# shanice-l/UNOPose

Measured on AMD Instinct MI355X. Metric: (query,ref) pairs/sec forward, higher is better.
Workload: dtype bf16; 1 GPU; UNOPose.forward, batch 32 pairs/GPU, 2048 query pts, 5000->2048 reference pts, 196 coarse pts, 518x518 crops, DINOv2 ViT-B/14 reg4, random-init (trained-like) weights

## Files before the change

### include/unopose_hip.h

```cpp
#ifndef UNOPOSE_HIP_H
#define UNOPOSE_HIP_H

#include <stdint.h>

#ifdef __cplusplus
extern "C" {
#endif

#define UNOPOSE_OK 0
#define UNOPOSE_EINVAL 1
#define UNOPOSE_ELAUNCH 2
#define UNOPOSE_ENOMEM 3

typedef void *unopose_stream_t;

int unopose_abi_version(void);
const char *unopose_last_error(void);


int unopose_furthest_point_sampling(const float *xyz, int B, int N, int M,
                                    int32_t *idx, unopose_stream_t stream);

int unopose_gather_points(const float *points, const int32_t *idx, int B, int C,
                          int N, int M, float *out, unopose_stream_t stream);

int unopose_gather_points_grad(const float *grad_out, const int32_t *idx, int B,
                               int C, int N, int M, float *grad_points,
                               unopose_stream_t stream);

int unopose_ball_query(const float *new_xyz, const float *xyz, int B, int N,
                       int M, float radius, int nsample, int32_t *idx,
                       unopose_stream_t stream);

int unopose_group_points(const float *points, const int32_t *idx, int B, int C,
                         int N, int M, int S, float *out,
                         unopose_stream_t stream);

int unopose_group_points_grad(const float *grad_out, const int32_t *idx, int B,
                              int C, int N, int M, int S, float *grad_points,
                              unopose_stream_t stream);

int unopose_three_nn(const float *unknown, const float *known, int B, int n,
                     int m, float *dist2, int32_t *idx, unopose_stream_t stream);

int unopose_three_interpolate(const float *points, const int32_t *idx,
                              const float *weight, int B, int c, int m, int n,
                              float *out, unopose_stream_t stream);

int unopose_three_interpolate_grad(const float *grad_out, const int32_t *idx,
                                   const float *weight, int B, int c, int n,
                                   int m, float *grad_points,
                                   unopose_stream_t stream);


int unopose_lrf_global(const float *pts, int B, int N, int use_ref_rad,
                       float *out, unopose_stream_t stream);

int unopose_query_lrf_group(const float *xyz, int B, int N, float radius,
                            int nsample, float *out, unopose_stream_t stream);

int unopose_lrf_group_idx(const float *xyz, const float *new_xyz, const int *idx,
                          int B, int N, float radius, int nsample, float *out,
                          unopose_stream_t stream);

int unopose_weighted_procrustes(const float *src, const float *ref,
                                const float *w, int M, int N, float thresh,
                                float eps, float *R, float *t,
                                unopose_stream_t stream);

int unopose_pe_image_bytes(void);
int unopose_pe_pack_weights(const float *w1, const float *b1, const float *w2, const float *b2,
                            const float *w3, const float *b3, void *image, unopose_stream_t stream);

int unopose_pe_geometry(const float *xyz, int B, int N, float radius, int nsample, float radius2, int nsample2,
                        const int *cand_in, const int *cand_cnt_in, int cand_stride, void *lists, int *counts,
                        float *frames, int *cand_out, void *lists2, int *counts2, float *frames2,
                        unopose_stream_t stream);
int unopose_pe_mlp_max_packed(const float *xyz, int B, int N, float radius, int nsample, const void *image,
                              const void *lists, const int *counts, const float *frames, void *out, int out_ld,
                              int out_split, unopose_stream_t stream);

int unopose_geo_embedding(const float *points, int B, int n, const void *wd_hi,
                          const void *wd_lo, const void *wa_hi, const void *wa_lo,
                          const float *bias_sum, const float *div_term,
                          float sigma_d, float factor_a, int reduce_mean, int split,
                          int out_bf16, int32_t *knn_ws, void *out,
                          unopose_stream_t stream);

int unopose_geo_embedding_table(const float *points, int B, int n, const float *tab_d, int rows_d, const float *tab_a, int rows_a,
                                const float *bias_sum, const float *w_d, const float *div_term, int hinv, int npoint, float sigma_d,
                                float factor_a, int reduce_mean, int out_bf16, int32_t *knn_ws, void *out,
                                unopose_stream_t stream);

int unopose_geo_embedding_train_workgroups(int B, int n);
int unopose_geo_embedding_train_forward(const float *points, int B, int n, const float *tab_d, int rows_d, const float *tab_a, int rows_a,
                                        const float *bias_sum, const float *w_d, const float *div_term, int hinv, float sigma_d, float factor_a,
                                        int reduce_mean, int32_t *knn, float *out, void *amax, unopose_stream_t stream);
int unopose_geo_embedding_train_backward(const float *points, const int32_t *knn, int B, int n, int rows_d, int rows_a, int hinv, float sigma_d,
                                         float factor_a, int reduce_mean, const float *dE, const void *amax, float *ws, float *full_d,
                                         int *past_table, unopose_stream_t stream);

int unopose_pe_group_mlp_max(const float *xyz, int B, int N, float radius, int nsample,
                             const float *w1, const float *b1, const float *w2,
                             const float *b2, const float *w3, const float *b3,
                             int bf16x3, float *out, unopose_stream_t stream);

int unopose_softmax_stats(const float *x, int B, int R, int C, float *stats_ws, unopose_stream_t stream);
int unopose_infonce_grad(const float *x, int B, int R, int C, const float *stats_ws, const long long *label1,
                         const long long *label2, const float *g, float *grad, unopose_stream_t stream);

int unopose_bn_train_chunk(void);
int unopose_bn_relu_train_forward(const float *x, int B, int C, long L, const float *gamma, const float *beta, float eps, float momentum,
                                  float *running_mean, float *running_var, float *workspace, float *mean, float *rstd, float *y,
                                  unopose_stream_t stream);
int unopose_bn_relu_train_backward(const float *x, const float *dy, int B, int C, long L, const float *gamma, const float *beta,
                                   const float *mean, const float *rstd, float *workspace, float *dgamma, float *dbeta, float *dx,
                                   unopose_stream_t stream);

int unopose_bn_relu_maxpool_train_forward(const float *x, int B, int C, int N, int S, const float *gamma, const float *beta, float eps,
                                          float momentum, float *running_mean, float *running_var, float *workspace, float *mean, float *rstd,
                                          float *out, int32_t *idx, unopose_stream_t stream);
int unopose_bn_relu_maxpool_train_backward(const float *x, const float *g, const int32_t *idx, int B, int C, int N, int S, const float *gamma,
                                           const float *beta, const float *mean, const float *rstd, float *workspace, float *dgamma, float *dbeta,
                                           float *dx, unopose_stream_t stream);

int unopose_saliency_train_forward(const float *atten, const float *s1, const float *s2, int B, int n1, int n2, float *m1, float *m2, float *rmax,
                                   float *rsum, float *cmax, float *csum, unopose_stream_t stream);
int unopose_saliency_train_backward(const float *atten, const float *s1, const float *s2, const float *m1, const float *m2, const float *rmax,
                                    const float *rsum, const float *cmax, const float *csum, const float *g1, const float *g2, int B, int n1, int n2,
                                    float *d_atten, float *ds1, float *ds2, unopose_stream_t stream);

int unopose_nearest_partner(const float *a, const float *b, int B, int n, int m, int over_b, float thr, float *dmin, int32_t *arg,
                            uint8_t *any_close, unopose_stream_t stream);

int unopose_conv1x1_train_wgrad_blocks(void);
int unopose_conv1x1_train_forward(const float *x, int B, int cin, long L, const float *w, int cout, float *y, unopose_stream_t stream);
int unopose_conv1x1_train_wgrad(const float *dy, const float *x, int B, int cout, int cin, long L, float *workspace, float *dw,
                                unopose_stream_t stream);

int unopose_linear_wgrad_f32_splits(long rows, int N, int K);
int unopose_linear_wgrad_f32(const float *g, const float *x, long rows, int N, int K, float *workspace, float *dw, unopose_stream_t stream);
int unopose_assign_labels(const float *atten, int B, int R, int C, const float *score1,
                          const float *score2, float *stats_ws, float *w1, float *w2,
                          unopose_stream_t stream);

int unopose_fine_correspondences(const float *atten, int B, int R, int C, const float *score1,
                                 const float *score2, const float *stats_ws, const float *w1,
                                 const float *w2, const float *pts2, float *weight, float *pred,
                                 unopose_stream_t stream);

int unopose_upproj_plan(const long long *choose, int B2, int Np, int H, int W, int side, int tok_offset, int tok_stride,
                        int cap_rows, int *ws, int *row_list, int *cellmap, int *tile_info, unopose_stream_t stream);

int unopose_linear_bf16_ld(const void *A, int lda, const void *W, int ldw, const float *bias, void *C, int ldc, long M, int N, int K,
                           int epilogue, unopose_stream_t stream);

int unopose_linear_add_layernorm_bf16(const void *A, const void *W, const float *bias, const void *resid, const float *ln_w,
                                      const float *ln_b, float eps, void *C, long M, int K, unopose_stream_t stream);

int unopose_linear_bf16_kv_vt(const void *A, const void *W, const float *bias, void *C, void *vt, long M, int N, int K, int tokens, int key_pad,
                              unopose_stream_t stream);

int unopose_linear_bf16_gather(const void *A, long M, int K, const void *W, int N, const float *bias, const int *row_list,
                               const int *tile_info, int max_tiles, void *C, unopose_stream_t stream);

int unopose_bilinear_sample_compact(const void *Cc, const int *cellmap, const long long *choose, int B2, int side, int Np,
                                    int H, int W, void *out, int out_bf16, unopose_stream_t stream);

int unopose_fine_assign(const void *f1, const void *f2, int B, int R, int C, int D, float shift, const float *score1,
                        const float *score2, const float *pts2, float *ws, float *w1, float *w2, float *weight,
                        float *pred, unopose_stream_t stream);

int unopose_min_dist(const float *p, const float *q, int B, int N, int M, const float *R,
                     const float *t, int cand_per_b, float *out, unopose_stream_t stream);

int unopose_coarse_hypotheses(const float *atten, int B, int R, int C, const float *score1,
                              const float *score2, const float *stats_ws, const float *w1,
                              const float *w2, const float *rand, int nprop, const float *pts1,
                              const float *pts2, float *cdf_ws, float *Rout, float *tout,
                              float *dis, unopose_stream_t stream);

int unopose_coarse_scores(const float *pts1, const float *pts2, int B, int n1, int n2,
                          const float *Rall, const float *tall, int nprop, const int64_t *top,
                          int ncand, const float *w1, float *score, unopose_stream_t stream);

int unopose_topk_smallest(const float *x, int B, int n, int k, int64_t *idx, unopose_stream_t stream);
int unopose_coarse_pick(const float *score, const int64_t *top, int B, int ncand, const float *Rall, const float *tall, int nprop,
                        float *R, float *t, float *best_score, unopose_stream_t stream);

int unopose_token_attention(const void *q, int ldq, const void *k, int ldk, const void *vt,
                            const void *qp, int ldqp, const void *E, int B, int n, int m,
                            float scale, void *out, unopose_stream_t stream);
int unopose_token_attention_key_pad(void);

int unopose_token_attention_f32(const float *q, int ldq, const float *k, int ldk, const float *vt,
                                const float *qp, int ldqp, const float *E, int B, int n, int m,
                                float scale, float *out, unopose_stream_t stream);
int unopose_vit_attention_f32(const float *qkv, int B, int T, int H, float *out, unopose_stream_t stream);
int unopose_token_attention_f32_train(const float *q, int ldq, const float *k, int ldk, const float *vt,
                                      const float *qp, int ldqp, const float *E, int B, int n, int m,
                                      float scale, float *out, float *P, unopose_stream_t stream);
int unopose_token_attention_f32_backward(const float *dout, const float *q, int ldq, const float *v, int ldv,
                                         const float *kt, const float *qp, int ldqp, const float *E, const float *P,
                                         int B, int n, int m, float scale, float *dS, float *dq, float *dk, float *dv,
                                         float *dqp, float *dE, unopose_stream_t stream);
int unopose_vit_attention_f32_split(const float *qkv, int B, int T, int H, void *out_split, unopose_stream_t stream);
int unopose_vit_attention_f32_ss(const void *qkv_split, int B, int T, int H, void *out_split, unopose_stream_t stream);

int unopose_vit_attention(const void *qkv, int B, int T, int H, void *out, unopose_stream_t stream);

int unopose_add_layernorm(const void *a, int a_bf16, const void *b, int b_bf16, const float *w,
                          const float *bias, long rows, int C, float eps, void *out, int out_bf16,
                          unopose_stream_t stream);

int unopose_add_layernorm_strided(const void *a, int a_bf16, const void *b, int b_bf16, const float *w,
                                  const float *bias, long rows, int C, float eps, void *out, int out_bf16,
                                  long ld_out, unopose_stream_t stream);

int unopose_bilinear_sample(const void *z, int z_bf16, const long long *choose, int B, int side, int Np,
                            int H, int W, float *out, unopose_stream_t stream);

int unopose_bilinear_sample_tokens(const void *z, int z_bf16, const long long *choose, int B, int side, int Np,
                                   int H, int W, int tok_offset, int tok_stride, float *out,
                                   unopose_stream_t stream);

int unopose_scale_residual_layernorm(float *x, const void *y_bf16, const float *gamma, const float *w,
                                     const float *bias, long rows, int C, float eps, void *out_bf16,
                                     unopose_stream_t stream);
int unopose_scale_residual_layernorm_f32(float *x, const float *y, const float *gamma, const float *w, const float *bias, long rows,
                                         int C, float eps, void *out_split, long out_ld_bytes, unopose_stream_t stream);

int unopose_scale_residual(float *x, const void *y_bf16, const float *gamma, long rows, int C,
                           unopose_stream_t stream);

int unopose_linear_attention(const void *x, const float *inv_softplus_scale, const void *kvt,
                             const float *ksum, int B, int N, int focus, int mode, void *out,
                             unopose_stream_t stream);
int unopose_linear_attention_kv_state(const void *ykv, const float *inv_softplus_scale, int B, int J, int rows_per_pair,
                                      int first_row, int focus, void *kvt, float *ksum, unopose_stream_t stream);
int unopose_linear_attention_f32(const float *x, const float *inv_softplus_scale, const float *kvt,
                                 const float *ksum, int B, int N, int focus, int mode, float *out,
                                 unopose_stream_t stream);

int unopose_render_depth(const float *verts, int V, const int *faces, int F, const float *Rt, const float *K4, int P, int H, int W,
                         float *depth, unopose_stream_t stream);

int unopose_patchify_bf16(const float *rgb_a, int na, const float *rgb_b, int nb, int S, int Kp, void *out,
                          unopose_stream_t stream);
int unopose_vit_tokens_layernorm(const void *patch, const float *pos, const float *prefix, int npre, int P, int nimg, int C,
                                 const float *ln_w, const float *ln_b, float eps, float *x, void *n1, float *row_mean, unopose_stream_t stream);
int unopose_patchify_split(const float *rgb_a, int na, const float *rgb_b, int nb, int S, int Kp, void *out, unopose_stream_t stream);
int unopose_vit_tokens_layernorm_f32(const float *patch, const float *pos, const float *prefix, int npre, int P, int nimg, int C,
                                     const float *ln_w, const float *ln_b, float eps, float *x, void *n1_split, unopose_stream_t stream);
int unopose_row_dot(const void *x, int x_bf16, const float *w, float b, long rows, int C, void *out, int out_bf16,
                    unopose_stream_t stream);
int unopose_normalize_rows_bf16(const void *x, int x_bf16, long rows, int C, float temp, void *out, int out_f32,
                                unopose_stream_t stream);
int unopose_gather_rows(const void *feats, int B, int N, int row_bytes, const void *idx, int idx_is_i64, int J, int off,
                        const void *alt, long alt_stride_bytes, int prepend, void *out, unopose_stream_t stream);
int unopose_transpose_pad_bf16(const void *v, long ld, int B, int m, int C, int pad, void *vt, unopose_stream_t stream);
int unopose_transpose_pad_f32(const float *v, long ld, int B, int m, int C, int pad, float *vt, unopose_stream_t stream);

int unopose_cloud_radius(const float *pts, int B, int N, float *radius, unopose_stream_t stream);
int unopose_scale_by_radius(const float *x, int B, int n, const float *radius, float eps, int multiply, float *out, unopose_stream_t stream);
int unopose_overlap_scores(const void *scores, int x_bf16, int B, int n_tot, int n1, int halves, float *out, unopose_stream_t stream);
int unopose_nan_to_num_multi(const void *ptrs_dev, const void *sizes_dev, int n_tensors, long max_size, float nan_value, float posinf_value,
                             float neginf_value, unopose_stream_t stream);
int unopose_copy_rows(const void *src, long src_stride_bytes, void *dst, long dst_stride_bytes, int rows, int row_bytes,
                      unopose_stream_t stream);
int unopose_rigid_rows_bf16(const float *p, int B, int N, const float *t, const float *R, void *out, unopose_stream_t stream);
int unopose_token_sum_bf16(const void *x, int B, int J, int C, float *out, unopose_stream_t stream);
int unopose_pose_score(const float *dis, const float *w, int B, int N, float thr, float *out, unopose_stream_t stream);

int unopose_linear_bf16(const void *A, const void *W, const float *bias, void *C, long M, int N, int K,
                        int epilogue, unopose_stream_t stream);
int unopose_gemm_bf16_tile(void);

int unopose_linear_bf16_residual(const void *A, const void *W, const float *bias, float *xres, void *xb, float *stats, const float *prev,
                                 int prev_nparts, long M, int N, int K, unopose_stream_t stream);
int unopose_linear_bf16_lnfold(const void *A, const void *W, const float *dvec, const float *cvec, const float *stats, int nparts, float eps,
                               void *C, long M, int N, int K, int gelu, unopose_stream_t stream);
int unopose_gemm_fold_stagger(int eighth_ticks_per_ktile);

int unopose_bmm_f32(const float *A, long sab, long sah, long sai, long sak, const float *Bm, long sbb, long sbh, long sbj, long sbk,
                    float *C, int bo, int bi, int n, int m, int K, float alpha, unopose_stream_t stream);

int unopose_split_bf16x2(const float *X, long M, int K, void *Xs, unopose_stream_t stream);
int unopose_linear_f32x3(const void *As, const void *Ws, const float *bias, float *C, void *Cs, long M, int N, int K,
                         int epilogue, unopose_stream_t stream);
int unopose_linear_f32x3_bf16(const void *As, const void *Ws, const float *bias, const void *resid, void *Cb, long M, int N, int K,
                              unopose_stream_t stream);

int unopose_prep_desc_ints(void);
int unopose_prep_crop_resize(const void *img, int H, int W, int C, const int *desc, const int *taps, const void *masks, const float *lut,
                             int D, int S, int bgr, int use_mask, float *out, unopose_stream_t stream);
int unopose_prep_compact_lift(const double *depth, int H, int W, const int *desc, const void *masks, const int *row_base, double fx,
                              double fy, double cx, double cy, int D, int max_h, int *pix, double *cloud, double *row_sums,
                              unopose_stream_t stream);
int unopose_prep_distances(const int *desc, const double *cloud, const double *row_sums, int D, int max_n, double *dist,
                           unopose_stream_t stream);
int unopose_prep_gather(const int *sel, const int *index, const int *pix, const double *cloud, int P, int n, int S, float *pts, void *choose,
                        unopose_stream_t stream);

int unopose_vsd_count_ints(void);
int unopose_vsd_counts(const float *test, int n_test, const float *gt, int n_gt, const float *est, int n_est, const int *index,
                       const double *pairs, const double *taus, int T, int P, int H, int W, int *counts, unopose_stream_t stream);
int unopose_pose_errors(const double *pts, int n, const double *syms, int S, const double *est, const double *gt, const double *K, int P,
                        double *mssd, double *mspd, unopose_stream_t stream);

int unopose_adi_tile_points(void);
int unopose_adi_slab_points(void);
int unopose_pose_metrics(const double *pts, int n, const double *syms, int S, const double *est, const double *gt, const double *K, int P,
                         int proj_sym, double *out, unopose_stream_t stream);
int unopose_adi(const double *pts, int n, const double *est, const double *gt, int P, double *workspace, double *adi,
                unopose_stream_t stream);

int unopose_gt_visibility_ints(void);
int unopose_gt_visibility(const float *canvas, int n_canvas, const float *test, int n_test, const int *index, const double *params, int G,
                          int H, int W, int *out, void *mask, void *mask_visib, unopose_stream_t stream);

int unopose_pts_extent_tile_points(void);
int unopose_pts_extent_doubles(void);
int unopose_pts_extent(const double *pts, const long long *offsets, const long long *offsets_dev, int M, int prune, double *kept,
                       long long *kept_count, double *out, unopose_stream_t stream);

#ifdef __cplusplus
}
#endif
#endif
```

### unopose_amd/_lib.py

```python
import ctypes
import os

import torch

_HERE = os.path.dirname(os.path.abspath(__file__))
SO_PATH = os.environ.get("UNOPOSE_LIB") or os.path.join(_HERE, "libunopose_hip.so")

_lib = None

_P = ctypes.c_void_p
_I = ctypes.c_int
_F = ctypes.c_float
_L = ctypes.c_long
_D = ctypes.c_double

SIGNATURES = {
    "unopose_furthest_point_sampling": [_P, _I, _I, _I, _P, _P],
    "unopose_gather_points": [_P, _P, _I, _I, _I, _I, _P, _P],
    "unopose_gather_points_grad": [_P, _P, _I, _I, _I, _I, _P, _P],
    "unopose_ball_query": [_P, _P, _I, _I, _I, _F, _I, _P, _P],
    "unopose_group_points": [_P, _P, _I, _I, _I, _I, _I, _P, _P],
    "unopose_group_points_grad": [_P, _P, _I, _I, _I, _I, _I, _P, _P],
    "unopose_three_nn": [_P, _P, _I, _I, _I, _P, _P, _P],
    "unopose_three_interpolate": [_P, _P, _P, _I, _I, _I, _I, _P, _P],
    "unopose_three_interpolate_grad": [_P, _P, _P, _I, _I, _I, _I, _P, _P],
    "unopose_lrf_global": [_P, _I, _I, _I, _P, _P],
    "unopose_query_lrf_group": [_P, _I, _I, _F, _I, _P, _P],
    "unopose_lrf_group_idx": [_P, _P, _P, _I, _I, _F, _I, _P, _P],
    "unopose_weighted_procrustes": [_P, _P, _P, _I, _I, _F, _F, _P, _P, _P],
    "unopose_assign_labels": [_P, _I, _I, _I, _P, _P, _P, _P, _P, _P],
    "unopose_linear_bf16_ld": [_P, _I, _P, _I, _P, _P, _I, ctypes.c_long, _I, _I, _I, _P],
    "unopose_scale_residual_layernorm_f32": [_P, _P, _P, _P, _P, ctypes.c_long, _I, _F, _P, _L, _P],
    "unopose_gather_rows": [_P, _I, _I, _I, _P, _I, _I, _I, _P, _L, _I, _P, _P],
    "unopose_softmax_stats": [_P, _I, _I, _I, _P, _P],
    "unopose_infonce_grad": [_P, _I, _I, _I, _P, _P, _P, _P, _P, _P],
    "unopose_fine_correspondences": [_P, _I, _I, _I, _P, _P, _P, _P, _P, _P, _P, _P, _P],
    "unopose_upproj_plan": [_P, _I, _I, _I, _I, _I, _I, _I, _I, _P, _P, _P, _P, _P],
    "unopose_linear_add_layernorm_bf16": [_P, _P, _P, _P, _P, _P, _F, _P, ctypes.c_long, _I, _P],
    "unopose_linear_bf16_kv_vt": [_P, _P, _P, _P, _P, ctypes.c_long, _I, _I, _I, _I, _P],
    "unopose_linear_bf16_gather": [_P, ctypes.c_long, _I, _P, _I, _P, _P, _P, _I, _P, _P],
    "unopose_bilinear_sample_compact": [_P, _P, _P, _I, _I, _I, _I, _I, _P, _I, _P],
    "unopose_fine_assign": [_P, _P, _I, _I, _I, _I, _F, _P, _P, _P, _P, _P, _P, _P, _P, _P],
    "unopose_min_dist": [_P, _P, _I, _I, _I, _P, _P, _I, _P, _P],
    "unopose_coarse_hypotheses": [_P, _I, _I, _I, _P, _P, _P, _P, _P, _P, _I, _P, _P, _P, _P, _P, _P, _P],
    "unopose_coarse_scores": [_P, _P, _I, _I, _I, _P, _P, _I, _P, _I, _P, _P, _P],
    "unopose_topk_smallest": [_P, _I, _I, _I, _P, _P],
    "unopose_coarse_pick": [_P, _P, _I, _I, _P, _P, _I, _P, _P, _P, _P],
    "unopose_token_attention": [_P, _I, _P, _I, _P, _P, _I, _P, _I, _I, _I, _F, _P, _P],
    "unopose_token_attention_key_pad": [],
    "unopose_token_attention_f32": [_P, _I, _P, _I, _P, _P, _I, _P, _I, _I, _I, _F, _P, _P],
    "unopose_token_attention_f32_train": [_P, _I, _P, _I, _P, _P, _I, _P, _I, _I, _I, _F, _P, _P, _P],
    "unopose_token_attention_f32_backward": [_P, _P, _I, _P, _I, _P, _P, _I, _P, _P, _I, _I, _I, _F, _P, _P, _P, _P, _P, _P, _P],
    "unopose_vit_attention_f32": [_P, _I, _I, _I, _P, _P],
    "unopose_vit_attention_f32_split": [_P, _I, _I, _I, _P, _P],
    "unopose_vit_attention_f32_ss": [_P, _I, _I, _I, _P, _P],
    "unopose_bn_train_chunk": [],
    "unopose_bn_relu_train_forward": [_P, _I, _I, ctypes.c_long, _P, _P, _F, _F, _P, _P, _P, _P, _P, _P, _P],
    "unopose_bn_relu_train_backward": [_P, _P, _I, _I, ctypes.c_long, _P, _P, _P, _P, _P, _P, _P, _P, _P],
    "unopose_bn_relu_maxpool_train_forward": [_P, _I, _I, _I, _I, _P, _P, _F, _F, _P, _P, _P, _P, _P, _P, _P, _P],
    "unopose_bn_relu_maxpool_train_backward": [_P, _P, _P, _I, _I, _I, _I, _P, _P, _P, _P, _P, _P, _P, _P, _P],
    "unopose_nearest_partner": [_P, _P, _I, _I, _I, _I, _F, _P, _P, _P, _P],
    "unopose_saliency_train_forward": [_P, _P, _P, _I, _I, _I, _P, _P, _P, _P, _P, _P, _P],
    "unopose_saliency_train_backward": [_P, _P, _P, _P, _P, _P, _P, _P, _P, _P, _P, _I, _I, _I, _P, _P, _P, _P],
    "unopose_conv1x1_train_wgrad_blocks": [],
    "unopose_conv1x1_train_forward": [_P, _I, _I, ctypes.c_long, _P, _I, _P, _P],
    "unopose_conv1x1_train_wgrad": [_P, _P, _I, _I, _I, ctypes.c_long, _P, _P, _P],
    "unopose_linear_wgrad_f32_splits": [ctypes.c_long, _I, _I],
    "unopose_linear_wgrad_f32": [_P, _P, ctypes.c_long, _I, _I, _P, _P, _P],
    "unopose_vit_attention": [_P, _I, _I, _I, _P, _P],
    "unopose_add_layernorm": [_P, _I, _P, _I, _P, _P, ctypes.c_long, _I, _F, _P, _I, _P],
    "unopose_add_layernorm_strided": [_P, _I, _P, _I, _P, _P, ctypes.c_long, _I, _F, _P, _I, ctypes.c_long, _P],
    "unopose_bilinear_sample": [_P, _I, _P, _I, _I, _I, _I, _I, _P, _P],
    "unopose_bilinear_sample_tokens": [_P, _I, _P, _I, _I, _I, _I, _I, _I, _I, _P, _P],
    "unopose_scale_residual_layernorm": [_P, _P, _P, _P, _P, ctypes.c_long, _I, _F, _P, _P],
    "unopose_scale_residual": [_P, _P, _P, ctypes.c_long, _I, _P],
    "unopose_linear_attention": [_P, _P, _P, _P, _I, _I, _I, _I, _P, _P],
    "unopose_linear_attention_f32": [_P, _P, _P, _P, _I, _I, _I, _I, _P, _P],
    "unopose_linear_attention_kv_state": [_P, _P, _I, _I, _I, _I, _I, _P, _P, _P],
    "unopose_linear_bf16": [_P, _P, _P, _P, ctypes.c_long, _I, _I, _I, _P],
    "unopose_gemm_bf16_tile": [],
    "unopose_gemm_fold_stagger": [_I],
    "unopose_linear_bf16_residual": [_P, _P, _P, _P, _P, _P, _P, _I, ctypes.c_long, _I, _I, _P],
    "unopose_linear_bf16_lnfold": [_P, _P, _P, _P, _P, _I, _F, _P, ctypes.c_long, _I, _I, _I, _P],
    "unopose_patchify_bf16": [_P, _I, _P, _I, _I, _I, _P, _P],
    "unopose_patchify_split": [_P, _I, _P, _I, _I, _I, _P, _P],
    "unopose_vit_tokens_layernorm": [_P, _P, _P, _I, _I, _I, _I, _P, _P, _F, _P, _P, _P, _P],
    "unopose_vit_tokens_layernorm_f32": [_P, _P, _P, _I, _I, _I, _I, _P, _P, _F, _P, _P, _P],
    "unopose_row_dot": [_P, _I, _P, _F, ctypes.c_long, _I, _P, _I, _P],
    "unopose_normalize_rows_bf16": [_P, _I, ctypes.c_long, _I, _F, _P, _I, _P],
    "unopose_transpose_pad_bf16": [_P, ctypes.c_long, _I, _I, _I, _I, _P, _P],
    "unopose_transpose_pad_f32": [_P, _L, _I, _I, _I, _I, _P, _P],
    "unopose_cloud_radius": [_P, _I, _I, _P, _P],
    "unopose_scale_by_radius": [_P, _I, _I, _P, _F, _I, _P, _P],
    "unopose_overlap_scores": [_P, _I, _I, _I, _I, _I, _P, _P],
    "unopose_copy_rows": [_P, _L, _P, _L, _I, _I, _P],
    "unopose_nan_to_num_multi": [_P, _P, _I, _L, _F, _F, _F, _P],
    "unopose_rigid_rows_bf16": [_P, _I, _I, _P, _P, _P, _P],
    "unopose_token_sum_bf16": [_P, _I, _I, _I, _P, _P],
    "unopose_pose_score": [_P, _P, _I, _I, _F, _P, _P],
    "unopose_render_depth": [_P, _I, _P, _I, _P, _P, _I, _I, _I, _P, _P],
    "unopose_bmm_f32": [_P, ctypes.c_long, ctypes.c_long, ctypes.c_long, ctypes.c_long, _P, ctypes.c_long, ctypes.c_long, ctypes.c_long, ctypes.c_long, _P, _I, _I, _I, _I, _I, _F, _P],
    "unopose_split_bf16x2": [_P, ctypes.c_long, _I, _P, _P],
    "unopose_linear_f32x3": [_P, _P, _P, _P, _P, ctypes.c_long, _I, _I, _I, _P],
    "unopose_pe_image_bytes": [],
    "unopose_pe_pack_weights": [_P, _P, _P, _P, _P, _P, _P, _P],
    "unopose_pe_geometry": [_P, _I, _I, _F, _I, _F, _I, _P, _P, _I, _P, _P, _P, _P, _P, _P, _P, _P],
    "unopose_pe_mlp_max_packed": [_P, _I, _I, _F, _I, _P, _P, _P, _P, _P, _I, _I, _P],
    "unopose_linear_f32x3_bf16": [_P, _P, _P, _P, _P, ctypes.c_long, _I, _I, _P],
    "unopose_pe_group_mlp_max": [_P, _I, _I, _F, _I, _P, _P, _P, _P, _P, _P, _I, _P, _P],
    "unopose_geo_embedding": [_P, _I, _I, _P, _P, _P, _P, _P, _P, _F, _F, _I, _I, _I, _P, _P, _P],
    "unopose_geo_embedding_train_workgroups": [_I, _I],
    "unopose_geo_embedding_train_forward": [_P, _I, _I, _P, _I, _P, _I, _P, _P, _P, _I, _F, _F, _I, _P, _P, _P, _P],
    "unopose_geo_embedding_train_backward": [_P, _P, _I, _I, _I, _I, _I, _F, _F, _I, _P, _P, _P, _P, _P, _P],
    "unopose_geo_embedding_table": [_P, _I, _I, _P, _I, _P, _I, _P, _P, _P, _I, _I, _F, _F, _I, _I, _P, _P, _P],
    "unopose_prep_desc_ints": [],
    "unopose_prep_crop_resize": [_P, _I, _I, _I, _P, _P, _P, _P, _I, _I, _I, _I, _P, _P],
    "unopose_prep_compact_lift": [_P, _I, _I, _P, _P, _P, _D, _D, _D, _D, _I, _I, _P, _P, _P, _P],
    "unopose_prep_distances": [_P, _P, _P, _I, _I, _P, _P],
    "unopose_prep_gather": [_P, _P, _P, _P, _I, _I, _I, _P, _P, _P],
    "unopose_vsd_count_ints": [],
    "unopose_vsd_counts": [_P, _I, _P, _I, _P, _I, _P, _P, _P, _I, _I, _I, _I, _P, _P],
    "unopose_pose_errors": [_P, _I, _P, _I, _P, _P, _P, _I, _P, _P, _P],
    "unopose_adi_tile_points": [],
    "unopose_adi_slab_points": [],
    "unopose_pose_metrics": [_P, _I, _P, _I, _P, _P, _P, _I, _I, _P, _P],
    "unopose_adi": [_P, _I, _P, _P, _I, _P, _P, _P],
    "unopose_gt_visibility_ints": [],
    "unopose_gt_visibility": [_P, _I, _P, _I, _P, _P, _I, _I, _I, _P, _P, _P, _P],
    "unopose_pts_extent_tile_points": [],
    "unopose_pts_extent_doubles": [],
    "unopose_pts_extent": [_P, _P, _P, _I, _I, _P, _P, _P, _P],
}


def lib():
    global _lib
    if _lib is None:
        if not os.path.exists(SO_PATH):
            raise RuntimeError(
                f"{SO_PATH} is missing: the HIP extension has not been built "
                "(run `python -m unopose_amd.build`). There is no CPU fallback."
            )
        L = ctypes.CDLL(SO_PATH)
        L.unopose_abi_version.restype = _I
        L.unopose_last_error.restype = ctypes.c_char_p
        for name, argtypes in SIGNATURES.items():
            fn = getattr(L, name)
            fn.argtypes = argtypes
            fn.restype = _I
        _lib = L
    return _lib


def stream_ptr(device=None):
    if device is None:
        idx = torch._C._cuda_getDevice()
    else:
        idx = device if isinstance(device, int) else torch.device(device).index
        if idx is None:
            idx = torch._C._cuda_getDevice()
    return ctypes.c_void_p(torch._C._cuda_getCurrentRawStream(idx))


class _NullContext:
    def __enter__(self):
        return None

    def __exit__(self, *a):
        return False


_NULL_CONTEXT = _NullContext()


def on_device(dev):
    idx = dev.index if isinstance(dev, torch.device) else dev
    if idx is None or idx == torch._C._cuda_getDevice():
        return _NULL_CONTEXT
    return torch.cuda.device(idx)


def call(name, *args):
    L = lib()
    rc = getattr(L, name)(*args)
    if rc != 0:
        raise RuntimeError(f"{name} failed (code {rc}): {L.unopose_last_error().decode()}")


def ptr(t):
    return ctypes.c_void_p(t.data_ptr())


def check_f32(x, name):
    if not x.is_cuda:
        raise RuntimeError(f"{name}: CPU not supported")
    if not x.is_contiguous():
        raise RuntimeError(f"{name} must be a contiguous tensor")
    if x.dtype != torch.float32:
        raise RuntimeError(f"{name} must be a float tensor")


def check_i32(x, name):
    if not x.is_cuda:
        raise RuntimeError(f"{name} must be a CUDA tensor")
    if not x.is_contiguous():
        raise RuntimeError(f"{name} must be a contiguous tensor")
    if x.dtype != torch.int32:
        raise RuntimeError(f"{name} must be an int tensor")
```

### unopose_amd/csrc/gemm.hip

```cpp
#include <mutex>

#include "gemm_kernel.h"

using namespace unopose;

static inline int use_nt_store(long M, int N) { return (size_t)M * N * 2 > (32u << 20) ? 1 : 0; }

namespace unopose {
int gemm_small_tiles_limit() {
  return gemm_cu_count() * 5 / 8;
}
}
static int small_tiles_limit() { return unopose::gemm_small_tiles_limit(); }

namespace unopose {
int *gemm_sched_slot(hipStream_t stream) {
  hipStreamCaptureStatus cap = hipStreamCaptureStatusNone;
  if (hipStreamIsCapturing(stream, &cap) != hipSuccess || cap != hipStreamCaptureStatusNone) return nullptr;
  static std::mutex mu;
  static int *ring[64] = {nullptr};
  static unsigned next_slot[64] = {0};
  int dev = 0;
  if (hipGetDevice(&dev) != hipSuccess || dev < 0 || dev >= 64) return nullptr;
  std::lock_guard<std::mutex> lock(mu);
  if (!ring[dev]) {
    int *p = nullptr;
    if (hipMalloc(&p, 1024 * 16 * sizeof(int)) != hipSuccess || hipMemset(p, 0, 1024 * 16 * sizeof(int)) != hipSuccess) return nullptr;
    ring[dev] = p;
  }
  return ring[dev] + (size_t)(next_slot[dev]++ & 1023u) * 16;
}
}

static int linear_bf16_dispatch(const void *A, int lda, const void *W, int ldw, const float *bias, void *C, int ldc, long M, int N, int K,
                                int epilogue, hipStream_t s, const char *what) {
  const int tiles_n = N / GEMM_BN;
  const int tiles = cdiv(M, GEMM_BM) * tiles_n;
  if (tiles < small_tiles_limit()) return gemm_small_linear(A, W, bias, C, M, N, K, lda, ldw, ldc, epilogue, s);
  const int n_cu = gemm_cu_count();
  const int grid = tiles >= n_cu ? n_cu : ((tiles + 7) & ~7);
  const int nt = use_nt_store(M, N);
#define UNOPOSE_LD_LAUNCH(E)                                                                                                                \
  hipLaunchKernelGGL(gemm256_kernel<E>, dim3(grid), dim3(512), 0, s, (const u16 *)A, (const u16 *)W, bias, (u16 *)C, (int)M, N, K, tiles_n, \
                     tiles, nt, (const int *)nullptr, (const int *)nullptr, (const u16 *)nullptr, (const float *)nullptr,                     \
                     (const float *)nullptr, 0.f, lda, ldw, ldc, sched)
  int *const sched = tiles > grid ? gemm_sched_slot(s) : nullptr;
  if (epilogue == 1)
    UNOPOSE_LD_LAUNCH(1);
  else if (epilogue == 2)
    UNOPOSE_LD_LAUNCH(2);
  else
    UNOPOSE_LD_LAUNCH(0);
#undef UNOPOSE_LD_LAUNCH
  return check_launch(what);
}

extern "C" {

int unopose_gemm_bf16_tile(void) { return GEMM_BM; }

int unopose_linear_bf16(const void *A, const void *W, const float *bias, void *C, long M, int N, int K, int epilogue,
                        unopose_stream_t stream) {
  UNOPOSE_REQUIRE(A && W && bias && C, "linear_bf16: null pointer");
  UNOPOSE_REQUIRE(M >= 1 && M < (1L << 31) && N >= GEMM_BN && N % GEMM_BN == 0 && K >= GEMM_BK && K % GEMM_BK == 0,
                  "linear_bf16: needs N %% 256 == 0 and K %% 64 == 0 (got M=%ld N=%d K=%d)", M, N, K);
  UNOPOSE_REQUIRE((size_t)M * K * 2 < (1UL << 32) && (size_t)N * K * 2 < (1UL << 32) && (size_t)M * N * 2 < (1UL << 32), "linear_bf16: operand larger than 4 GiB");
  UNOPOSE_REQUIRE(epilogue >= 0 && epilogue <= 2, "linear_bf16: epilogue must be 0 (bias), 1 (bias + GELU) or 2 (bias + ReLU)");
  return linear_bf16_dispatch(A, K, W, K, bias, C, N, M, N, K, epilogue, (hipStream_t)stream, "linear_bf16");
}

int unopose_linear_bf16_ld(const void *A, int lda, const void *W, int ldw, const float *bias, void *C, int ldc, long M, int N, int K,
                           int epilogue, unopose_stream_t stream) {
  UNOPOSE_REQUIRE(A && W && bias && C, "linear_bf16_ld: null pointer");
  UNOPOSE_REQUIRE(M >= 1 && M < (1L << 31) && N >= GEMM_BN && N % GEMM_BN == 0 && K >= GEMM_BK && K % GEMM_BK == 0,
                  "linear_bf16_ld: needs N %% 256 == 0 and K %% 64 == 0 (got M=%ld N=%d K=%d)", M, N, K);
  UNOPOSE_REQUIRE(lda >= K && ldw >= K && ldc >= N && lda % 8 == 0 && ldw % 8 == 0 && ldc % 8 == 0,
                  "linear_bf16_ld: row strides must cover the rows and be multiples of 8 elements (lda=%d ldw=%d ldc=%d)", lda, ldw, ldc);
  UNOPOSE_REQUIRE((size_t)M * lda * 2 < (1UL << 32) && (size_t)N * ldw * 2 < (1UL << 32) && (size_t)M * ldc * 2 < (1UL << 32), "linear_bf16_ld: operand larger than 4 GiB");
  UNOPOSE_REQUIRE(epilogue >= 0 && epilogue <= 2, "linear_bf16_ld: epilogue must be 0 (bias), 1 (bias + GELU) or 2 (bias + ReLU)");
  return linear_bf16_dispatch(A, lda, W, ldw, bias, C, ldc, M, N, K, epilogue, (hipStream_t)stream, "linear_bf16_ld");
}

int unopose_linear_add_layernorm_bf16(const void *A, const void *W, const float *bias, const void *resid, const float *ln_w,
                                      const float *ln_b, float eps, void *C, long M, int K, unopose_stream_t stream) {
  UNOPOSE_REQUIRE(A && W && bias && resid && ln_w && ln_b && C, "linear_add_layernorm_bf16: null pointer");
  UNOPOSE_REQUIRE(M >= 1 && M < (1L << 31) && K >= GEMM_BK && K % GEMM_BK == 0, "linear_add_layernorm_bf16: needs K %% 64 == 0 (got M=%ld K=%d)", M, K);
  UNOPOSE_REQUIRE((size_t)M * K * 2 < (1UL << 32), "linear_add_layernorm_bf16: operand larger than 4 GiB");
  const int tiles = cdiv(M, GEMM_BM);
  if (tiles < small_tiles_limit()) return gemm_small_linear_ln(A, W, bias, resid, ln_w, ln_b, eps, C, M, K, (hipStream_t)stream);
  const int n_cu = gemm_cu_count();
  const int grid = tiles >= n_cu ? n_cu : ((tiles + 7) & ~7);
  hipLaunchKernelGGL((gemm256_kernel<3, false>), dim3(grid), dim3(512), 0, (hipStream_t)stream, (const u16 *)A, (const u16 *)W, bias,
                     (u16 *)C, (int)M, GEMM_BN, K, 1, tiles, use_nt_store(M, GEMM_BN), (const int *)nullptr, (const int *)nullptr,
                     (const u16 *)resid, ln_w, ln_b, eps);
  return check_launch("linear_add_layernorm_bf16");
}

int unopose_linear_bf16_kv_vt(const void *A, const void *W, const float *bias, void *C, void *vt, long M, int N, int K, int tokens, int key_pad,
                               unopose_stream_t stream) {
  UNOPOSE_REQUIRE(A && W && bias && C && vt, "linear_bf16_kv_vt: null pointer");
  UNOPOSE_REQUIRE(M >= 1 && M < (1L << 31) && N >= 256 && N % 128 == 0 && K >= GEMM_BK && K % GEMM_BK == 0,
                  "linear_bf16_kv_vt: needs N %% 128 == 0 (>= 256) and K %% 64 == 0 (got M=%ld N=%d K=%d)", M, N, K);
  UNOPOSE_REQUIRE(tokens >= 1 && key_pad >= tokens && M % tokens == 0 && key_pad - tokens <= 64, "linear_bf16_kv_vt: M must be whole clouds of `tokens` rows, key_pad in [tokens, tokens + 64] (got %ld, %d, %d)", M, tokens, key_pad);
  UNOPOSE_REQUIRE((size_t)M * K * 2 < (1UL << 32) && (size_t)N * K * 2 < (1UL << 32) && (size_t)M * N * 2 < (1UL << 32), "linear_bf16_kv_vt: operand larger than 4 GiB");
  return gemm_small_linear_vt(A, W, bias, C, vt, M, N, K, tokens, key_pad, (hipStream_t)stream);
}

int unopose_linear_bf16_gather(const void *A, long M, int K, const void *W, int N, const float *bias, const int *row_list,
                               const int *tile_info, int max_tiles, void *C, unopose_stream_t stream) {
  UNOPOSE_REQUIRE(A && W && bias && C && row_list && tile_info, "linear_bf16_gather: null pointer");
  UNOPOSE_REQUIRE(M >= 1 && M < (1L << 31) && N >= GEMM_BN && N % GEMM_BN == 0 && N / GEMM_BN <= 64 && K >= GEMM_BK && K % GEMM_BK == 0,
                  "linear_bf16_gather: needs N %% 256 == 0 and K %% 64 == 0 (got M=%ld N=%d K=%d)", M, N, K);
  UNOPOSE_REQUIRE((size_t)M * K * 2 < (1UL << 32) && (size_t)N * K * 2 < (1UL << 32), "linear_bf16_gather: operand larger than 4 GiB");
  UNOPOSE_REQUIRE(max_tiles >= 0, "linear_bf16_gather: bad tile capacity");
  if (max_tiles == 0) return UNOPOSE_OK;
  const int n_cu = gemm_cu_count();
  const int grid = max_tiles >= n_cu ? n_cu : ((max_tiles + 7) & ~7);
  hipLaunchKernelGGL((gemm256_kernel<0, true>), dim3(grid), dim3(512), 0, (hipStream_t)stream, (const u16 *)A, (const u16 *)W, bias,
                     (u16 *)C, (int)M, N, K, 1, 0, 0, row_list, tile_info);
  return check_launch("linear_bf16_gather");
}

static int fold_launch_shape(long M, int N, int *grid, int *tiles, int *tiles_n) {
  *tiles_n = N / GEMM_BN;
  *tiles = cdiv(M, GEMM_BM) * *tiles_n;
  const int n_cu = gemm_cu_count();
  *grid = *tiles >= n_cu ? n_cu : ((*tiles + 7) & ~7);
  return use_nt_store(M, N);
}

static int g_fold_stagger = 8 * 105;
int unopose_gemm_fold_stagger(int eighth_ticks_per_ktile) {
  const int was = g_fold_stagger;
  if (eighth_ticks_per_ktile >= 0) g_fold_stagger = eighth_ticks_per_ktile;
  return was;
}

int unopose_linear_bf16_residual(const void *A, const void *W, const float *bias, float *xres, void *xb, float *stats, const float *prev,
                                 int prev_nparts, long M, int N, int K, unopose_stream_t stream) {
  UNOPOSE_REQUIRE(A && W && bias && xres && xb && stats, "linear_bf16_residual: null pointer");
  UNOPOSE_REQUIRE(prev != stats && (prev_nparts == 0 || (prev && prev_nparts * GEMM_BN == N && prev_nparts <= GEMM_LNF_MAXPARTS)),
                  "linear_bf16_residual: prev must be another buffer with 0 or N / 256 <= %d partials per row (got prev_nparts=%d N=%d)",
                  GEMM_LNF_MAXPARTS, prev_nparts, N);
  UNOPOSE_REQUIRE(M >= 1 && M < (1L << 31) && N >= GEMM_BN && N % GEMM_BN == 0 && K >= GEMM_BK && K % GEMM_BK == 0,
                  "linear_bf16_residual: needs N %% 256 == 0 and K %% 64 == 0 (got M=%ld N=%d K=%d)", M, N, K);
  UNOPOSE_REQUIRE((size_t)M * K * 2 < (1UL << 32) && (size_t)N * K * 2 < (1UL << 32) && (size_t)M * N * 4 < (1UL << 31), "linear_bf16_residual: operand too large for 32-bit buffer offsets");
  int grid, tiles, tiles_n;
  const int nt = fold_launch_shape(M, N, &grid, &tiles, &tiles_n);
  hipStream_t s = (hipStream_t)stream;
  int *const sched = tiles > grid ? gemm_sched_slot(s) : nullptr;
  hipLaunchKernelGGL((gemm256_kernel<5>), dim3(grid), dim3(512), 0, s, (const u16 *)A, (const u16 *)W, bias, (u16 *)xb, (int)M, N, K, tiles_n, tiles, nt,
                     (const int *)nullptr, (const int *)nullptr, (const u16 *)nullptr, (const float *)nullptr, (const float *)nullptr, 0.f, 0, 0, 0, sched,
                     (void *)xres, (const float *)nullptr, (float2 *)stats, prev_nparts, tiles > grid ? g_fold_stagger * (K / GEMM_BK) / 8 : 0, prev);
  return check_launch("linear_bf16_residual");
}

int unopose_linear_bf16_lnfold(const void *A, const void *W, const float *dvec, const float *cvec, const float *stats, int nparts, float eps, void *C,
                               long M, int N, int K, int gelu, unopose_stream_t stream) {
  UNOPOSE_REQUIRE(A && W && dvec && cvec && stats && C, "linear_bf16_lnfold: null pointer");
  UNOPOSE_REQUIRE(M >= 1 && M < (1L << 31) && N >= GEMM_BN && N % GEMM_BN == 0 && K >= GEMM_BK && K % GEMM_BK == 0,
                  "linear_bf16_lnfold: needs N %% 256 == 0 and K %% 64 == 0 (got M=%ld N=%d K=%d)", M, N, K);
  UNOPOSE_REQUIRE(nparts >= 1 && nparts <= GEMM_LNF_MAXPARTS && nparts * GEMM_BN == K, "linear_bf16_lnfold: needs nparts = K / 256 <= %d (got nparts=%d K=%d)", GEMM_LNF_MAXPARTS, nparts, K);
  UNOPOSE_REQUIRE((size_t)M * K * 2 < (1UL << 32) && (size_t)N * K * 2 < (1UL << 32) && (size_t)M * N * 2 < (1UL << 32), "linear_bf16_lnfold: operand larger than 4 GiB");
  int grid, tiles, tiles_n;
  const int nt = fold_launch_shape(M, N, &grid, &tiles, &tiles_n);
  hipStream_t s = (hipStream_t)stream;
  int *const sched = tiles > grid ? gemm_sched_slot(s) : nullptr;
#define UNOPOSE_LNF_LAUNCH(E)                                                                                                                      \
  hipLaunchKernelGGL((gemm256_kernel<E>), dim3(grid), dim3(512), 0, s, (const u16 *)A, (const u16 *)W, dvec, (u16 *)C, (int)M, N, K, tiles_n, tiles, nt, \
                     (const int *)nullptr, (const int *)nullptr, (const u16 *)nullptr, (const float *)nullptr, (const float *)nullptr, eps, 0, 0, 0, sched, \
                     (void *)nullptr, cvec, (float2 *)stats, nparts)
  if (gelu)
    UNOPOSE_LNF_LAUNCH(7);
  else
    UNOPOSE_LNF_LAUNCH(6);
#undef UNOPOSE_LNF_LAUNCH
  return check_launch("linear_bf16_lnfold");
}

}
```

### unopose_amd/csrc/gemm_kernel.h

```cpp
#pragma once
#include "gemm_common.h"

namespace unopose {

constexpr int GEMM_XPOL = 2;
#define GEMM_BK 64
constexpr int GEMM_ROTX = 5, GEMM_ROTS = 3;

#define GEMM_WAIT_VM(n) asm volatile("s_waitcnt vmcnt(" #n ")" ::: "memory")
#define GEMM_WAIT_VM_(n) GEMM_WAIT_VM(n)

#define GEMM_LDS_BIAS (2 * GEMM_BUFBYTES)
#define GEMM_LDS_MBOX (GEMM_LDS_BIAS + 2048)
#define GEMM_LDS_LNW (GEMM_LDS_MBOX + 16)
#define GEMM_LDS_LNB (GEMM_LDS_LNW + 1024)
#define GEMM_LDS_LNPART (GEMM_LDS_LNB + 1024)
#define GEMM_LDS_STATS GEMM_LDS_LNPART
#define GEMM_LNF_MAXPARTS 4
#define GEMM_LDS_SHIFT (GEMM_LDS_LNPART + 8192)

template <int EPI, bool GATHER = false, bool F32 = false>
__global__ __launch_bounds__(512, 1) __attribute__((amdgpu_num_vgpr(127))) void gemm256_kernel(const void *__restrict__ Av, const void *__restrict__ Wv,
                                                           const float *__restrict__ bias, void *__restrict__ Cv, int M,
                                                           int N, int K, int tiles_n, int tiles_arg, int nt_store,
                                                           const int *__restrict__ row_list = nullptr,
                                                           const int *__restrict__ tile_info = nullptr,
                                                           const u16 *__restrict__ resid = nullptr, const float *__restrict__ ln_w = nullptr,
                                                           const float *__restrict__ ln_b = nullptr, float ln_eps = 0.f, int lda = 0,
                                                           int ldw = 0, int ldc = 0, int *__restrict__ sched = nullptr,
                                                           void *__restrict__ C2v = nullptr, const float *__restrict__ aux_vec = nullptr,
                                                           float2 *__restrict__ stats = nullptr, int nparts = 0, int stagger = 0,
                                                           const float *__restrict__ fold_prev = nullptr) {
  static_assert(!(F32 && (EPI == 3 || GATHER)), "the fp32-class form has no LayerNorm epilogue / gathered rows");
  static_assert(!((F32 || GATHER) && EPI >= 5), "the residual / LayerNorm-fold epilogues belong to the dense bf16 form");
  constexpr bool LNF = EPI == 6 || EPI == 7;
  static_assert(F32 || EPI != 4, "EPI 4 (bf16 + residual out of fp32-class operands) is an F32 epilogue");
  constexpr int ESZ = F32 ? 4 : 2;
  constexpr int KT = F32 ? 32 : 64;
  const char *A = reinterpret_cast<const char *>(Av), *W = reinterpret_cast<const char *>(Wv);
  const int LDA = lda ? lda : K, LDW = ldw ? ldw : K, LDC = ldc ? ldc : N;
  const int tiles = GATHER ? __builtin_amdgcn_readfirstlane(tile_info[0]) : tiles_arg;
  __shared__ __attribute__((aligned(1024))) char smem[GEMM_LDS_BIAS + 2048 + 16 + (EPI == 3 ? 2048 + 8192 : EPI == 5 ? 2048 + 8192 + 4096 : LNF ? 2048 + 2 * 8192 : 0)];
  float *const lnw_lds = reinterpret_cast<float *>(smem + GEMM_LDS_LNW), *const lnb_lds = reinterpret_cast<float *>(smem + GEMM_LDS_LNB);
  float2 *const ln_part = reinterpret_cast<float2 *>(smem + GEMM_LDS_LNPART);
  if (EPI == 3 && threadIdx.x < GEMM_BN) {
    lnw_lds[threadIdx.x] = ln_w[threadIdx.x];
    lnb_lds[threadIdx.x] = ln_b[threadIdx.x];
  }
  const int tid = threadIdx.x, lane = tid & 63, wave = __builtin_amdgcn_readfirstlane(tid >> 6);
  const int wm = wave >> 2, wn = wave & 3;
  const int l31 = lane & 31, hi = lane >> 5;
  const int l31_ = l31, hi_ = hi, lane_ = lane;
  const int xcd = blockIdx.x & 7, slot = blockIdx.x >> 3, nslots = gridDim.x >> 3;
  const int tiles_m = tiles / tiles_n, per_group = GEMM_GM * tiles_n;
  int cw = (size_t)N * K * ESZ > (size_t)(4u << 20) ? (2400 * 1024) / (GEMM_BN * K * ESZ) : 0;
  if (cw < 3) cw = 0;
  const bool colwalk = cw > 0 && !GATHER && tiles_n > cw && ((tiles_m & 7) == 0 || tiles_m >= 512);
  const int rq = tiles_m >> 3, rr = tiles_m & 7;
  const int rows_x = rq + (xcd < rr ? 1 : 0), row_base = xcd < rr ? xcd * (rq + 1) : rr * (rq + 1) + (xcd - rr) * rq;
  const int cq = tiles >> 3, cr = tiles & 7;
  const int chunk_base = xcd < cr ? xcd * (cq + 1) : cr * (cq + 1) + (xcd - cr) * cq;
  const int chunk_len = colwalk ? rows_x * tiles_n : cq + (xcd < cr ? 1 : 0);
  const __amdgpu_buffer_rsrc_t a_rs = __builtin_amdgcn_make_buffer_rsrc((void *)A, 0, (int)((size_t)M * LDA * ESZ), 0x00020000);
  const __amdgpu_buffer_rsrc_t w_rs = __builtin_amdgcn_make_buffer_rsrc((void *)W, 0, (int)((size_t)N * LDW * ESZ), 0x00020000);
  const __amdgpu_buffer_rsrc_t c_rs = __builtin_amdgcn_make_buffer_rsrc(Cv, 0, GATHER ? 0x7fffffff : (int)((size_t)M * LDC * 2), 0x00020000);
  const __amdgpu_buffer_rsrc_t b_rs = __builtin_amdgcn_make_buffer_rsrc((void *)bias, 0, N * 4, 0x00020000);
  const int nk = K / KT;

  const int fx = (l31 >> 1) & 7;
  uint32_t fr_off[4];
#pragma unroll
  for (int ks = 0; ks < 4; ++ks) fr_off[ks] = (uint32_t)((l31 >> 3) * 1024 + (l31 & 7) * 128 + ((((ks << 1) | hi) ^ fx) << 4));
  const uint32_t a_base = (uint32_t)(wm * 16384);
  const uint32_t w_base = (uint32_t)(GEMM_OPBYTES + wn * 8192);
  const uint32_t a_dst = (uint32_t)((wave >> 2) * 16384 + (wave & 3) * 2048);
  const uint32_t w_dst = (uint32_t)(GEMM_OPBYTES + (wave >> 1) * 8192 + (wave & 1) * 2048);

  struct TileP {
    int m0, n0, rot;
    uint32_t a_off[4], w_off[2];
  };
  auto tile_params = [&](int ti, int step, TileP &p) {
    const int t = chunk_base + ti;
    int tn, tm;
    if (GATHER) {
      tm = t;
      tn = 0;
      const int ng = N / GEMM_BN;
      for (int g = 1; g < ng; ++g) tn += t >= tile_info[1 + g] ? 1 : 0;
      tn = __builtin_amdgcn_readfirstlane(tn);
    } else if (colwalk) {
      const int per_block = rows_x * cw;
      const int cb = ti / per_block, v = ti - cb * per_block;
      const int cwb = min(cw, tiles_n - cb * cw);
      const int g = v / (GEMM_GM * cwb), w = v - g * GEMM_GM * cwb;
      const int gm = min(GEMM_GM, rows_x - g * GEMM_GM);
      const int tl = w / gm;
      tn = cb * cw + tl;
      tm = row_base + g * GEMM_GM + (w - tl * gm);
    } else {
      const int mg = t / per_group, rr = t - mg * per_group;
      const int gm = min(GEMM_GM, tiles_m - mg * GEMM_GM);
      tn = rr / gm;
      tm = mg * GEMM_GM + (rr - tn * gm);
    }
    p.m0 = __builtin_amdgcn_readfirstlane(tm * GEMM_BM);
    p.n0 = __builtin_amdgcn_readfirstlane(tn * GEMM_BN);
#pragma unroll
    for (int j = 0; j < 4; ++j) {
      const int row = (wave >> 2) * 128 + (j >> 1) * 64 + (wave & 3) * 16 + (j & 1) * 8 + (lane >> 3);
      const int c = (lane & 7) ^ ((row >> 1) & 7);
      int arow = p.m0 + row;
      if (GATHER) arow = max(row_list[p.m0 + row], 0);
      p.a_off[j] = (uint32_t)((size_t)arow * LDA * ESZ + c * 16);
    }
#pragma unroll
    for (int i = 0; i < 2; ++i) {
      const int row = (wave >> 1) * 64 + (wave & 1) * 16 + i * 8 + (lane >> 3);
      const int c = (lane & 7) ^ ((row >> 1) & 7);
      p.w_off[i] = (uint32_t)((size_t)(p.n0 + row) * LDW * ESZ + c * 16);
    }
    const int skew = ((tm & 3) + tn) % GEMM_SKEW;
    p.rot = __builtin_amdgcn_readfirstlane((xcd * GEMM_ROTX + step * GEMM_ROTS + skew) % nk);
  };
  const uint32_t lds0 = (uint32_t)(uintptr_t)(__attribute__((address_space(3))) char *)smem;
  enum { H_A0 = 0, H_B0 = 1, H_B1 = 2, H_A1 = 3 };
  auto stage_half = [&](const TileP &p, int kind, int kt, uint32_t bufoff) {
    kt += __builtin_amdgcn_readfirstlane(p.rot);
    if (kt >= nk) kt -= nk;
    const int so = kt * GEMM_ROWB;
    if (kind == H_A0 || kind == H_A1) {
      const int ah = kind == H_A1 ? 1 : 0;
      const uint32_t la = lds0 + bufoff + a_dst + ah * 8192;
      gemm_dma16(la, p.a_off[2 * ah], a_rs, so);
      gemm_dma16(la + 1024, p.a_off[2 * ah + 1], a_rs, so);
    } else {
      const int bh = kind == H_B1 ? 1 : 0;
      const uint32_t lw = lds0 + bufoff + w_dst + bh * 4096;
      const int sob = so + bh * (32 * ESZ) * LDW;
      gemm_dma16(lw, p.w_off[0], w_rs, sob);
      gemm_dma16(lw + 1024, p.w_off[1], w_rs, sob);
    }
  };
  const __amdgpu_buffer_rsrc_t cv_rs = __builtin_amdgcn_make_buffer_rsrc((void *)(LNF ? aux_vec : bias), 0, N * 4, 0x00020000);
  const __amdgpu_buffer_rsrc_t st_rs = __builtin_amdgcn_make_buffer_rsrc((void *)stats, 0, LNF ? (int)((size_t)((M + GEMM_BM - 1) / GEMM_BM) * GEMM_BM * nparts * 8) : 0, 0x00020000);
  auto stage_bias = [&](const TileP &p, int bsel) {
    if (!LNF) {
      gemm_dma16(lds0 + GEMM_LDS_BIAS + bsel * 1024, (uint32_t)(lane * 16), b_rs, __builtin_amdgcn_readfirstlane(p.n0 * 4));
      return;
    }
    const int total = 2 + 2 * nparts;
#pragma unroll
    for (int rep = 0; rep < (2 + 2 * GEMM_LNF_MAXPARTS + 7) / 8; ++rep) {
      if (rep * 8 >= total) break;
      int pc = rep * 8 + wave;
      if (pc >= total) pc = 0;
      if (pc == 0)
        gemm_dma16(lds0 + GEMM_LDS_BIAS + bsel * 1024, (uint32_t)(lane * 16), b_rs, __builtin_amdgcn_readfirstlane(p.n0 * 4));
      else if (pc == 1)
        gemm_dma16(lds0 + GEMM_LDS_LNW + bsel * 1024, (uint32_t)(lane * 16), cv_rs, __builtin_amdgcn_readfirstlane(p.n0 * 4));
      else
        gemm_dma16(lds0 + GEMM_LDS_STATS + bsel * 8192 + (pc - 2) * 1024, (uint32_t)(lane * 16), st_rs,
                   __builtin_amdgcn_readfirstlane(p.m0 * nparts * 8 + (pc - 2) * 1024));
    }
  };
  const bool can_stream = EPI != 3 && nk >= 2;
  const bool dyn = sched != nullptr && !GATHER && can_stream && nk >= 5;
  int *const mbox = reinterpret_cast<int *>(smem + GEMM_LDS_MBOX);
  TileP cur;
  bool have = false;
  uint32_t par = 0;
  int bsel = 0;
  int ti = slot;
  if (dyn) {
    if (tid == 0) mbox[0] = atomicAdd(sched + xcd, 1);
    __syncthreads();
    ti = __builtin_amdgcn_readfirstlane(mbox[0]);
  }
  if (EPI == 5 && stagger > 0 && ((slot / tiles_n) & 1)) {
    const uint64_t t0 = __builtin_amdgcn_s_memrealtime();
    while ((int64_t)(__builtin_amdgcn_s_memrealtime() - t0) < (int64_t)stagger) __builtin_amdgcn_s_sleep(8);
  }
  for (; ti < chunk_len;) {
    const int step = dyn ? ti / nslots : (ti - slot) / nslots;
    if (!have) {
      tile_params(ti, step, cur);
      stage_bias(cur, bsel);
      stage_half(cur, H_A0, 0, par);
      stage_half(cur, H_B0, 0, par);
      stage_half(cur, H_B1, 0, par);
      stage_half(cur, H_A1, 0, par);
      if (nk >= 2) {
        stage_half(cur, H_A0, 1, par ^ GEMM_BUFBYTES);
        stage_half(cur, H_B0, 1, par ^ GEMM_BUFBYTES);
        GEMM_WAIT_VM(6);
      } else {
        GEMM_WAIT_VM(2);
      }
      asm volatile("s_waitcnt lgkmcnt(0)" ::: "memory");
      __builtin_amdgcn_s_barrier();
    }
    const int m0 = __builtin_amdgcn_readfirstlane(cur.m0), n0 = __builtin_amdgcn_readfirstlane(cur.n0);
    cur.rot = __builtin_amdgcn_readfirstlane(cur.rot);
    bool more = can_stream && ti + nslots < chunk_len;
    int ti_next = ti + nslots;
    TileP nxt;

    const float *bias_lds = reinterpret_cast<const float *>(smem + GEMM_LDS_BIAS + bsel * 1024);
    f32x16 acc[2][4];
#pragma unroll
    for (int nb = 0; nb < 2; ++nb)
#pragma unroll
      for (int g = 0; g < 4; ++g) {
        const float4 bv = EPI == 3 || LNF ? make_float4(0.f, 0.f, 0.f, 0.f) : *reinterpret_cast<const float4 *>(bias_lds + wn * 64 + nb * 32 + 8 * g + 4 * hi);
#pragma unroll
        for (int mb = 0; mb < 4; ++mb) {
          acc[nb][mb][4 * g + 0] = bv.x;
          acc[nb][mb][4 * g + 1] = bv.y;
          acc[nb][mb][4 * g + 2] = bv.z;
          acc[nb][mb][4 * g + 3] = bv.w;
        }
      }

    bf16x8 af[2][4], wf0[4], wf1[4];
    auto read_a = [&](const char *lb, int ah) {
#pragma unroll
      for (int mbl = 0; mbl < 2; ++mbl)
#pragma unroll
        for (int ks = 0; ks < 4; ++ks) af[mbl][ks] = *reinterpret_cast<const bf16x8 *>(lb + a_base + ah * 8192 + mbl * 4096 + fr_off[ks]);
    };
    auto read_b = [&](const char *lb, int bh, bf16x8(&wf)[4]) {
#pragma unroll
      for (int ks = 0; ks < 4; ++ks) wf[ks] = *reinterpret_cast<const bf16x8 *>(lb + w_base + bh * 4096 + fr_off[ks]);
    };
    auto mfma_q = [&](int ah, int bh, const bf16x8(&wf)[4]) {
      if (F32) {
#pragma unroll
        for (int b = 0; b < 2; ++b)
#pragma unroll
          for (int mbl = 0; mbl < 2; ++mbl) {
            f32x16 &a = acc[bh][2 * ah + mbl];
            a = __builtin_amdgcn_mfma_f32_32x32x16_bf16(wf[2 + b], af[mbl][b], a, 0, 0, 0);
            a = __builtin_amdgcn_mfma_f32_32x32x16_bf16(wf[b], af[mbl][2 + b], a, 0, 0, 0);
            a = __builtin_amdgcn_mfma_f32_32x32x16_bf16(wf[b], af[mbl][b], a, 0, 0, 0);
          }
        return;
      }
#pragma unroll
      for (int ks = 0; ks < 4; ++ks)
#pragma unroll
        for (int mbl = 0; mbl < 2; ++mbl)
          acc[bh][2 * ah + mbl] = __builtin_amdgcn_mfma_f32_32x32x16_bf16(wf[ks], af[mbl][ks], acc[bh][2 * ah + mbl], 0, 0, 0);
    };
    if (wm == 1) __builtin_amdgcn_s_barrier();
    auto phase = [&](auto compute) {
      asm volatile("s_waitcnt lgkmcnt(0)" ::: "memory");
      __builtin_amdgcn_sched_barrier(0);
      __builtin_amdgcn_s_barrier();
      __builtin_amdgcn_sched_barrier(0);
      compute();
      __builtin_amdgcn_sched_barrier(0);
      __builtin_amdgcn_s_barrier();
      asm volatile("" ::: "memory");
      __builtin_amdgcn_sched_barrier(0);
    };
    for (int t = 0; t < nk; ++t) {
      const bool last = t + 1 == nk, last2 = t + 2 >= nk;
      if (dyn) {
        if (t == 2 && wave == 0) {
          int tk;
          asm volatile("v_readfirstlane_b32 %0, v255" : "=s"(tk)::"memory");
          if (lane == 0) mbox[0] = tk;
        }
        if (t + 2 == nk) {
          ti_next = __builtin_amdgcn_readfirstlane(*reinterpret_cast<volatile int *>(mbox));
          more = ti_next < chunk_len;
        }
      }
      if (more && t + 2 == nk) tile_params(ti_next, dyn ? ti_next / nslots : step + 1, nxt);
      const char *lb = smem + par;
      const uint32_t bnext = par ^ GEMM_BUFBYTES;
      read_b(lb, 0, wf0);
      read_b(lb, 1, wf1);
      read_a(lb, 0);
      __builtin_amdgcn_sched_barrier(0);
      if (t == 0 && !last) stage_half(cur, H_B1, 1, bnext);
      if (!last)
        stage_half(cur, H_A1, t + 1, bnext);
      else if (more)
        stage_half(nxt, H_A1, 0, bnext);
      if (last && !more)
        GEMM_WAIT_VM(0);
      else
        GEMM_WAIT_VM(8);
      phase([&] {
        mfma_q(0, 0, wf0);
        mfma_q(0, 1, wf1);
      });
      read_a(lb, 1);
      __builtin_amdgcn_sched_barrier(0);
      if (dyn && t == 0 && wave == 0) {
        unsigned long long keep;
        const uint32_t zero = 0, one = 1;
#pragma clang diagnostic push
#pragma clang diagnostic ignored "-Winline-asm"
        asm volatile("s_mov_b64 %0, exec\n\ts_mov_b64 exec, 1\n\ts_nop 1\n\tglobal_atomic_add v255, %2, %3, %1 sc0\n\ts_mov_b64 exec, %0\n\ts_nop 1"
                     : "=&s"(keep)
                     : "s"(sched + xcd), "v"(zero), "v"(one)
                     : "memory", "v255");
#pragma clang diagnostic pop
      }
      if (!last2) {
        stage_half(cur, H_A0, t + 2, par);
        stage_half(cur, H_B0, t + 2, par);
        stage_half(cur, H_B1, t + 2, par);
        GEMM_WAIT_VM(8);
      } else if (more) {
        if (!last) {
          stage_bias(nxt, bsel ^ 1);
          stage_half(nxt, H_A0, 0, par);
          stage_half(nxt, H_B0, 0, par);
          stage_half(nxt, H_B1, 0, par);
          if (LNF) {
            if (nparts <= 3) GEMM_WAIT_VM(9);
            else GEMM_WAIT_VM(10);
          } else
            GEMM_WAIT_VM(8);
        } else if (F32) {
          GEMM_WAIT_VM(2);
        } else {
          stage_half(nxt, H_A0, 1, par);
          stage_half(nxt, H_B0, 1, par);
          GEMM_WAIT_VM(6);
        }
      } else if (!last) {
        GEMM_WAIT_VM(2);
      }
      phase([&] {
        mfma_q(1, 1, wf1);
        mfma_q(1, 0, wf0);
      });
      par ^= GEMM_BUFBYTES;
    }
    if (wm == 0) __builtin_amdgcn_s_barrier();
    par ^= GEMM_BUFBYTES;
    if (EPI == 3) {
#pragma unroll
      for (int mb = 0; mb < 4; ++mb) {
        const int m = min(m0 + wm * 128 + mb * 32 + l31, M - 1);
        const u16 *rp = resid + (size_t)m * GEMM_BN + wn * 64 + 4 * hi;
        float a1 = 0.f, a2 = 0.f;
#pragma unroll
        for (int nb = 0; nb < 2; ++nb)
#pragma unroll
          for (int g = 0; g < 4; ++g) {
            const int nl = nb * 32 + 8 * g + 4 * hi;
            const float4 bv = *reinterpret_cast<const float4 *>(bias_lds + wn * 64 + nl);
            const uint2 r = *reinterpret_cast<const uint2 *>(rp + nb * 32 + 8 * g);
            const float v0 = acc[nb][mb][4 * g + 0] + bv.x + __uint_as_float(r.x << 16);
            const float v1 = acc[nb][mb][4 * g + 1] + bv.y + __uint_as_float(r.x & 0xffff0000u);
            const float v2 = acc[nb][mb][4 * g + 2] + bv.z + __uint_as_float(r.y << 16);
            const float v3 = acc[nb][mb][4 * g + 3] + bv.w + __uint_as_float(r.y & 0xffff0000u);
            acc[nb][mb][4 * g + 0] = v0;
            acc[nb][mb][4 * g + 1] = v1;
            acc[nb][mb][4 * g + 2] = v2;
            acc[nb][mb][4 * g + 3] = v3;
            a1 += (v0 + v1) + (v2 + v3);
            a2 += (v0 * v0 + v1 * v1) + (v2 * v2 + v3 * v3);
          }
        a1 += __shfl_xor(a1, 32);
        a2 += __shfl_xor(a2, 32);
        if (hi == 0) ln_part[((wm * 4 + mb) * 32 + l31) * 4 + wn] = make_float2(a1, a2);
      }
      __syncthreads();
#pragma unroll
      for (int mb = 0; mb < 4; ++mb) {
        const float2 *pp = ln_part + ((wm * 4 + mb) * 32 + l31) * 4;
        const float t1 = (pp[0].x + pp[1].x) + (pp[2].x + pp[3].x), t2 = (pp[0].y + pp[1].y) + (pp[2].y + pp[3].y);
        const float mean = t1 * (1.f / GEMM_BN);
        const float rstd = rsqrtf(fmaxf(t2 * (1.f / GEMM_BN) - mean * mean, 0.f) + ln_eps);
#pragma unroll
        for (int nb = 0; nb < 2; ++nb)
#pragma unroll
          for (int g = 0; g < 4; ++g) {
            const int nl = wn * 64 + nb * 32 + 8 * g + 4 * hi;
            const float4 gw = *reinterpret_cast<const float4 *>(lnw_lds + nl), gb = *reinterpret_cast<const float4 *>(lnb_lds + nl);
            acc[nb][mb][4 * g + 0] = (acc[nb][mb][4 * g + 0] - mean) * rstd * gw.x + gb.x;
            acc[nb][mb][4 * g + 1] = (acc[nb][mb][4 * g + 1] - mean) * rstd * gw.y + gb.y;
            acc[nb][mb][4 * g + 2] = (acc[nb][mb][4 * g + 2] - mean) * rstd * gw.z + gb.z;
            acc[nb][mb][4 * g + 3] = (acc[nb][mb][4 * g + 3] - mean) * rstd * gw.w + gb.w;
          }
      }
    }
    if constexpr (LNF) {
      int l31 = l31_, hi = hi_;
      asm volatile("" : "+v"(l31), "+v"(hi));
      const float *c_lds = reinterpret_cast<const float *>(smem + GEMM_LDS_LNW + bsel * 1024);
      const float inv_k = 1.f / (float)K;
      float rs[4], nm[4];
#pragma unroll
      for (int mb = 0; mb < 4; ++mb) {
        const float2 *sp = reinterpret_cast<const float2 *>(smem + GEMM_LDS_STATS + bsel * 8192) + (wm * 128 + mb * 32 + l31) * nparts;
        float t1 = 0.f, t2 = 0.f;
#pragma unroll
        for (int i = 0; i < GEMM_LNF_MAXPARTS; ++i)
          if (i < nparts) {
            const float2 q = sp[i];
            t1 += q.x;
            t2 += q.y;
          }
        const float mean = t1 * inv_k;
        rs[mb] = rsqrtf(fmaxf(t2 * inv_k - mean * mean, 0.f) + ln_eps);
        nm[mb] = -mean * rs[mb];
      }
#pragma unroll
      for (int nb = 0; nb < 2; ++nb)
#pragma unroll
        for (int g = 0; g < 4; ++g) {
          const int nl = wn * 64 + nb * 32 + 8 * g + 4 * hi;
          const float4 cv = *reinterpret_cast<const float4 *>(c_lds + nl), dv = *reinterpret_cast<const float4 *>(bias_lds + nl);
#pragma unroll
          for (int mb = 0; mb < 4; ++mb) {
            acc[nb][mb][4 * g + 0] = fmaf(rs[mb], acc[nb][mb][4 * g + 0], fmaf(nm[mb], cv.x, dv.x));
            acc[nb][mb][4 * g + 1] = fmaf(rs[mb], acc[nb][mb][4 * g + 1], fmaf(nm[mb], cv.y, dv.y));
            acc[nb][mb][4 * g + 2] = fmaf(rs[mb], acc[nb][mb][4 * g + 2], fmaf(nm[mb], cv.z, dv.z));
            acc[nb][mb][4 * g + 3] = fmaf(rs[mb], acc[nb][mb][4 * g + 3], fmaf(nm[mb], cv.w, dv.w));
          }
        }
    }
    if constexpr (EPI == 5) {
      int l31 = l31_, hi = hi_, lane = lane_;
      asm volatile("" : "+v"(l31), "+v"(hi), "+v"(lane));
      char *cw = smem + par + (wave < 4 ? 8192 + (wave & 1) * 4096 + (wave >> 1) * 16384 : GEMM_OPBYTES + 4096 + (wave - 4) * 8192);
      const __amdgpu_buffer_rsrc_t x_rs = __builtin_amdgcn_make_buffer_rsrc(C2v, 0, (int)((size_t)M * N * 4), 0x00020000);
      const int r4 = lane >> 4, q = lane & 15;
      const uint32_t x_v0 = (uint32_t)((((size_t)m0 + wm * 128 + r4) * N + n0 + wn * 64 + q * 4) * 4);
      const uint32_t c_v0 = (uint32_t)((((size_t)m0 + wm * 128 + r4) * LDC + n0 + wn * 64 + q * 4) * 2);
      const uint32_t x_rowb = (uint32_t)(N * 4), c_rowb = (uint32_t)(LDC * 2);
      const int rows_p = tiles_m * GEMM_BM;
      float sv[2] = {0.f, 0.f};
      if (fold_prev != nullptr) {
        float pv[2][GEMM_LNF_MAXPARTS + 1];
#pragma unroll
        for (int j = 0; j < 2; ++j) {
          const size_t m = (size_t)m0 + wm * 128 + j * 64 + lane, sh_at = (size_t)rows_p * 2 * nparts + m;
#pragma unroll
          for (int i = 0; i < GEMM_LNF_MAXPARTS; ++i) pv[j][i] = fold_prev[i < nparts ? m * 2 * nparts + 2 * i : sh_at];
          pv[j][GEMM_LNF_MAXPARTS] = fold_prev[sh_at];
        }
#pragma unroll
        for (int j = 0; j < 2; ++j) {
          float t = 0.f;
#pragma unroll
          for (int i = 0; i < GEMM_LNF_MAXPARTS; ++i) t += i < nparts ? pv[j][i] : 0.f;
          sv[j] = m0 + wm * 128 + j * 64 + lane < M ? pv[j][GEMM_LNF_MAXPARTS] + t * (1.f / (float)N) : 0.f;
        }
      }
      constexpr int PF = 3;
      f32x4 rv[PF][4];
      auto load_round = [&](int r, f32x4(&dst)[4]) {
#pragma unroll
        for (int it = 0; it < 4; ++it) {
          dst[it] = __builtin_bit_cast(f32x4, __builtin_amdgcn_raw_buffer_load_b128(x_rs, x_v0 + (uint32_t)(r * 16 + it * 4) * x_rowb, 0, GEMM_XPOL));
        }
      };
#pragma unroll
      for (int r = 0; r < PF; ++r) load_round(r, rv[r]);
      float *const sh_lds = reinterpret_cast<float *>(smem + GEMM_LDS_SHIFT + wave * 512);
#pragma unroll
      for (int r = 0; r < 8; ++r) {
        const int mb = r >> 1, h = r & 1;
        if ((l31 >> 4) == h) {
#pragma unroll
          for (int nb = 0; nb < 2; ++nb)
#pragma unroll
            for (int g = 0; g < 4; ++g) {
              const int s16 = (nb * 8 + 2 * g + hi) ^ (l31 & 15);
              *reinterpret_cast<float4 *>(cw + (l31 & 15) * 256 + s16 * 16) =
                  make_float4(acc[nb][mb][4 * g + 0], acc[nb][mb][4 * g + 1], acc[nb][mb][4 * g + 2], acc[nb][mb][4 * g + 3]);
            }
        }
        if (r == 0) {
#pragma unroll
          for (int j = 0; j < 2; ++j) {
            sh_lds[j * 64 + lane] = sv[j];
            if (wn == 0) reinterpret_cast<float *>(stats)[(size_t)rows_p * 2 * tiles_n + m0 + wm * 128 + j * 64 + lane] = sv[j];
          }
        }
        __builtin_amdgcn_fence(__ATOMIC_RELEASE, "wavefront");
        __builtin_amdgcn_wave_barrier();
        __builtin_amdgcn_fence(__ATOMIC_ACQUIRE, "wavefront");
#pragma unroll
        for (int it = 0; it < 4; ++it) {
          const int row = it * 4 + r4;
          const f32x4 a = *reinterpret_cast<const f32x4 *>(cw + row * 256 + ((q ^ row) << 4));
          const f32x4 o = rv[r % PF][it];
          f32x4 v;
#pragma unroll
          for (int e = 0; e < 4; ++e) v[e] = a[e] + o[e];
          __builtin_amdgcn_raw_buffer_store_b128(__builtin_bit_cast(u32x4, v), x_rs, x_v0 + (uint32_t)(r * 16 + it * 4) * x_rowb, 0, GEMM_XPOL);
          const float s = sh_lds[row + r * 16];
#pragma unroll
          for (int e = 0; e < 4; ++e) v[e] = v[e] - s;
          typedef unsigned int u32x2 __attribute__((ext_vector_type(2)));
          const u32x2 pk = {cvt_pk_bf16_f32(v[0], v[1]), cvt_pk_bf16_f32(v[2], v[3])};
          if (nt_store)
            __builtin_amdgcn_raw_buffer_store_b64(pk, c_rs, c_v0 + (uint32_t)(r * 16 + it * 4) * c_rowb, 0, 2);
          else
            __builtin_amdgcn_raw_buffer_store_b64(pk, c_rs, c_v0 + (uint32_t)(r * 16 + it * 4) * c_rowb, 0, 0);
          float a1 = (v[0] + v[1]) + (v[2] + v[3]), a2 = (v[0] * v[0] + v[1] * v[1]) + (v[2] * v[2] + v[3] * v[3]);
          a1 += dpp_f32<0x111, 0xF>(a1, 0.f);
          a2 += dpp_f32<0x111, 0xF>(a2, 0.f);
          a1 += dpp_f32<0x112, 0xF>(a1, 0.f);
          a2 += dpp_f32<0x112, 0xF>(a2, 0.f);
          a1 += dpp_f32<0x114, 0xF>(a1, 0.f);
          a2 += dpp_f32<0x114, 0xF>(a2, 0.f);
          a1 += dpp_f32<0x118, 0xF>(a1, 0.f);
          a2 += dpp_f32<0x118, 0xF>(a2, 0.f);
          if (q == 15) ln_part[((wm * 4 + mb) * 32 + h * 16 + row) * 4 + wn] = make_float2(a1, a2);
        }
        __builtin_amdgcn_fence(__ATOMIC_RELEASE, "wavefront");
        __builtin_amdgcn_wave_barrier();
        __builtin_amdgcn_fence(__ATOMIC_ACQUIRE, "wavefront");
        if (r + PF < 8) load_round(r + PF, rv[r % PF]);
      }
      asm volatile("s_waitcnt lgkmcnt(0)" ::: "memory");
      __builtin_amdgcn_s_barrier();
      if (wn == 0 && hi == 0) {
#pragma unroll
        for (int mb = 0; mb < 4; ++mb) {
          const float2 *pp = ln_part + ((wm * 4 + mb) * 32 + l31) * 4;
          const float4 p01 = *reinterpret_cast<const float4 *>(pp), p23 = *reinterpret_cast<const float4 *>(pp + 2);
          stats[(size_t)(m0 + wm * 128 + mb * 32 + l31) * tiles_n + (n0 >> 8)] = make_float2((p01.x + p01.z) + (p23.x + p23.z), (p01.y + p01.w) + (p23.y + p23.w));
        }
      }
    } else if constexpr (!F32) {
    int l31 = l31_, hi = hi_, lane = lane_;
    asm volatile("" : "+v"(l31), "+v"(hi), "+v"(lane));
    char *cw = smem + par + (wave < 4 ? 8192 + (wave & 1) * 4096 + (wave >> 1) * 16384 : GEMM_OPBYTES + 4096 + (wave - 4) * 8192);
    const uint32_t c_v0 = GATHER ? (uint32_t)((((size_t)m0 + wm * 128 + (lane >> 3)) * GEMM_BN + wn * 64 + (lane & 7) * 8) * 2)
                                 : (uint32_t)((((size_t)m0 + wm * 128 + (lane >> 3)) * LDC + n0 + wn * 64 + (lane & 7) * 8) * 2);
    const uint32_t c_rowb = (uint32_t)((GATHER ? GEMM_BN : LDC) * 2);
#pragma unroll
    for (int mb = 0; mb < 4; ++mb) {
#pragma unroll
      for (int nb = 0; nb < 2; ++nb) {
#pragma unroll
        for (int g = 0; g < 4; ++g) {
          const int nl = nb * 32 + 8 * g + 4 * hi;
          float v0 = acc[nb][mb][4 * g + 0], v1 = acc[nb][mb][4 * g + 1], v2 = acc[nb][mb][4 * g + 2], v3 = acc[nb][mb][4 * g + 3];
          if (EPI == 1 || EPI == 7) {
            v0 = gelu_bf16_class(v0);
            v1 = gelu_bf16_class(v1);
            v2 = gelu_bf16_class(v2);
            v3 = gelu_bf16_class(v3);
          }
          if (EPI == 2) {
            v0 = fmaxf(v0, 0.f);
            v1 = fmaxf(v1, 0.f);
            v2 = fmaxf(v2, 0.f);
            v3 = fmaxf(v3, 0.f);
          }
          const int slot16 = (nl >> 3) ^ (l31 & 7);
          *reinterpret_cast<uint2 *>(cw + l31 * 128 + slot16 * 16 + (nl & 4) * 2) = make_uint2(cvt_pk_bf16_f32(v0, v1), cvt_pk_bf16_f32(v2, v3));
        }
      }
      __builtin_amdgcn_fence(__ATOMIC_RELEASE, "wavefront");
      __builtin_amdgcn_wave_barrier();
      __builtin_amdgcn_fence(__ATOMIC_ACQUIRE, "wavefront");
      u32x4 cv[4];
#pragma unroll
      for (int it = 0; it < 4; ++it) {
        const int row = it * 8 + (lane >> 3), q = lane & 7;
        cv[it] = *reinterpret_cast<const u32x4 *>(cw + row * 128 + ((q ^ (row & 7)) << 4));
      }
#pragma unroll
      for (int it = 0; it < 4; ++it) {
        const uint32_t off = c_v0 + (uint32_t)(mb * 32 + it * 8) * c_rowb;
        if (nt_store)
          __builtin_amdgcn_raw_buffer_store_b128(cv[it], c_rs, off, 0, 2);
        else
          __builtin_amdgcn_raw_buffer_store_b128(cv[it], c_rs, off, 0, 0);
      }
      __builtin_amdgcn_fence(__ATOMIC_RELEASE, "wavefront");
      __builtin_amdgcn_wave_barrier();
      __builtin_amdgcn_fence(__ATOMIC_ACQUIRE, "wavefront");
    }
    } else {
    int l31 = l31_, hi = hi_, lane = lane_;
    asm volatile("" : "+v"(l31), "+v"(hi), "+v"(lane));
    char *cw = smem + par + wave * 8192;
    const __amdgpu_buffer_rsrc_t cf_rs = __builtin_amdgcn_make_buffer_rsrc(Cv, 0, (int)((size_t)M * N * (EPI == 4 ? 2 : 4)), 0x00020000);
    const __amdgpu_buffer_rsrc_t cs_rs = __builtin_amdgcn_make_buffer_rsrc(C2v, 0, (int)((size_t)M * N * 4), 0x00020000);
    const __amdgpu_buffer_rsrc_t rs_rs = __builtin_amdgcn_make_buffer_rsrc((void *)resid, 0, (int)((size_t)M * N * 2), 0x00020000);
    const bool has_cf = Cv != nullptr, has_cs = C2v != nullptr;
    const uint32_t c32_v0 = (uint32_t)((((size_t)m0 + wm * 128 + (lane >> 4)) * N + n0 + wn * 64 + (lane & 15) * 4) * 4);
    const uint32_t c16_v0 = (uint32_t)((((size_t)m0 + wm * 128 + (lane >> 3)) * N + n0 + wn * 64 + (lane & 7) * 8) * 2);
#pragma unroll
    for (int mb = 0; mb < 4; ++mb) {
      auto vals = [&](int nb, int g, float (&x)[4]) {
#pragma unroll
        for (int e = 0; e < 4; ++e) {
          float t = acc[nb][mb][4 * g + e];
          if (EPI == 1) t = gelu_erf(t);
          if (EPI == 2) t = fmaxf(t, 0.f);
          x[e] = t;
        }
        __builtin_amdgcn_sched_barrier(0);
      };
      if (EPI == 4) {
#pragma unroll
        for (int nb = 0; nb < 2; ++nb)
#pragma unroll
          for (int g = 0; g < 4; ++g) {
            float x[4];
            vals(nb, g, x);
            *reinterpret_cast<uint2 *>(cw + l31 * 128 + (((nb * 4 + g) ^ (l31 & 7)) << 4) + hi * 8) =
                make_uint2(cvt_pk_bf16_f32(x[0], x[1]), cvt_pk_bf16_f32(x[2], x[3]));
          }
        __builtin_amdgcn_fence(__ATOMIC_RELEASE, "wavefront");
        __builtin_amdgcn_wave_barrier();
        __builtin_amdgcn_fence(__ATOMIC_ACQUIRE, "wavefront");
#pragma unroll
        for (int it = 0; it < 4; ++it) {
          const int row = it * 8 + (lane >> 3), q = lane & 7;
          u32x4 o = *reinterpret_cast<const u32x4 *>(cw + row * 128 + ((q ^ (row & 7)) << 4));
          const uint32_t off = c16_v0 + (uint32_t)(mb * 32 + it * 8) * (uint32_t)(N * 2);
          if (resid) {
            const u32x4 r = __builtin_amdgcn_raw_buffer_load_b128(rs_rs, off, 0, 0);
#pragma unroll
            for (int e = 0; e < 4; ++e)
              o[e] = cvt_pk_bf16_f32(__uint_as_float(o[e] << 16) + __uint_as_float(r[e] << 16),
                                     __uint_as_float(o[e] & 0xffff0000u) + __uint_as_float(r[e] & 0xffff0000u));
          }
          __builtin_amdgcn_raw_buffer_store_b128(o, cf_rs, off, 0, 0);
        }
        __builtin_amdgcn_fence(__ATOMIC_RELEASE, "wavefront");
        __builtin_amdgcn_wave_barrier();
        __builtin_amdgcn_fence(__ATOMIC_ACQUIRE, "wavefront");
        continue;
      }
      if (has_cf) {
#pragma unroll
        for (int nb = 0; nb < 2; ++nb)
#pragma unroll
          for (int g = 0; g < 4; ++g) {
            float x[4];
            vals(nb, g, x);
            const int s = (nb * 8 + 2 * g + hi) ^ (l31 & 15);
            *reinterpret_cast<float4 *>(cw + l31 * 256 + s * 16) = make_float4(x[0], x[1], x[2], x[3]);
          }
        __builtin_amdgcn_fence(__ATOMIC_RELEASE, "wavefront");
        __builtin_amdgcn_wave_barrier();
        __builtin_amdgcn_fence(__ATOMIC_ACQUIRE, "wavefront");
#pragma unroll
        for (int it = 0; it < 8; ++it) {
          const int row = it * 4 + (lane >> 4), q = lane & 15;
          const u32x4 o = *reinterpret_cast<const u32x4 *>(cw + row * 256 + ((q ^ (row & 15)) << 4));
          const uint32_t off = c32_v0 + (uint32_t)(mb * 32 + it * 4) * (uint32_t)(N * 4);
          if (nt_store)
            __builtin_amdgcn_raw_buffer_store_b128(o, cf_rs, off, 0, 2);
          else
            __builtin_amdgcn_raw_buffer_store_b128(o, cf_rs, off, 0, 0);
        }
        __builtin_amdgcn_fence(__ATOMIC_RELEASE, "wavefront");
        __builtin_amdgcn_wave_barrier();
        __builtin_amdgcn_fence(__ATOMIC_ACQUIRE, "wavefront");
      }
      if (has_cs) {
#pragma unroll
        for (int nb = 0; nb < 2; ++nb)
#pragma unroll
          for (int g = 0; g < 4; ++g) {
            float x[4];
            vals(nb, g, x);
            const uint32_t h0 = cvt_pk_bf16_f32(x[0], x[1]), h1 = cvt_pk_bf16_f32(x[2], x[3]);
            const float r0 = x[0] - __uint_as_float(h0 << 16), r1 = x[1] - __uint_as_float(h0 & 0xffff0000u);
            const float r2 = x[2] - __uint_as_float(h1 << 16), r3 = x[3] - __uint_as_float(h1 & 0xffff0000u);
            const uint32_t l0 = cvt_pk_bf16_f32(r0, r1), l1 = cvt_pk_bf16_f32(r2, r3);
            const int sh = (nb * 8 + g) ^ (l31 & 15), sl = (nb * 8 + 4 + g) ^ (l31 & 15);
            *reinterpret_cast<uint2 *>(cw + l31 * 256 + sh * 16 + hi * 8) = make_uint2(h0, h1);
            *reinterpret_cast<uint2 *>(cw + l31 * 256 + sl * 16 + hi * 8) = make_uint2(l0, l1);
          }
        __builtin_amdgcn_fence(__ATOMIC_RELEASE, "wavefront");
        __builtin_amdgcn_wave_barrier();
        __builtin_amdgcn_fence(__ATOMIC_ACQUIRE, "wavefront");
#pragma unroll
        for (int it = 0; it < 8; ++it) {
          const int row = it * 4 + (lane >> 4), q = lane & 15;
          const u32x4 o = *reinterpret_cast<const u32x4 *>(cw + row * 256 + ((q ^ (row & 15)) << 4));
          __builtin_amdgcn_raw_buffer_store_b128(o, cs_rs, c32_v0 + (uint32_t)(mb * 32 + it * 4) * (uint32_t)(N * 4), 0, 0);
        }
        __builtin_amdgcn_fence(__ATOMIC_RELEASE, "wavefront");
        __builtin_amdgcn_wave_barrier();
        __builtin_amdgcn_fence(__ATOMIC_ACQUIRE, "wavefront");
      }
    }
    }
    par ^= GEMM_BUFBYTES;
    asm volatile("s_waitcnt lgkmcnt(0)" ::: "memory");
    __builtin_amdgcn_s_barrier();
    if (F32 && more) {
      stage_half(nxt, H_A0, 1, par ^ GEMM_BUFBYTES);
      stage_half(nxt, H_B0, 1, par ^ GEMM_BUFBYTES);
    }
    have = more;
    if (more) {
      cur = nxt;
      bsel ^= 1;
    }
    ti = ti_next;
  }
  if (dyn && tid == 0) {
    if (atomicAdd(sched + 8, 1) == (int)gridDim.x - 1) {
#pragma unroll
      for (int i = 0; i < 9; ++i) __hip_atomic_store(sched + i, 0, __ATOMIC_RELAXED, __HIP_MEMORY_SCOPE_AGENT);
    }
  }
}

}
```

### unopose_amd/model/modules.py

```python
import math

import torch
import torch.nn as nn
import torch.nn.functional as F

from .. import ops


class _Attention(nn.Module):
    def __init__(self, dim, heads):
        super().__init__()
        self.heads = heads
        self.qkv = nn.Linear(dim, 3 * dim)
        self.proj = nn.Linear(dim, dim)

    def forward(self, x):
        B, T, C = x.shape
        qkv = ops.linear(x, self.qkv)
        o = ops.vit_attention(qkv, self.heads)
        return ops.linear(o, self.proj)


class _LayerScale(nn.Module):
    def __init__(self, dim):
        super().__init__()
        self.gamma = nn.Parameter(torch.full((dim,), 1e-5))


class _Mlp(nn.Module):
    def __init__(self, dim, ratio=4):
        super().__init__()
        self.fc1 = nn.Linear(dim, ratio * dim)
        self.fc2 = nn.Linear(ratio * dim, dim)

    def forward(self, x):
        return ops.mlp(x, self.fc1, self.fc2)


class _Block(nn.Module):
    def __init__(self, dim, heads):
        super().__init__()
        self.norm1 = nn.LayerNorm(dim, eps=1e-6)
        self.attn = _Attention(dim, heads)
        self.ls1 = _LayerScale(dim)
        self.norm2 = nn.LayerNorm(dim, eps=1e-6)
        self.mlp = _Mlp(dim)
        self.ls2 = _LayerScale(dim)

    def forward_fused(self, x, n1, next_norm):
        y = self.attn(n1)
        n2 = ops.scale_residual_layernorm_(x, y, self.ls1.gamma, self.norm2)
        y = self.mlp(n2)
        if next_norm is None:
            ops.scale_residual_(x, y, self.ls2.gamma)
            return x, None
        return x, ops.scale_residual_layernorm_(x, y, self.ls2.gamma, next_norm)

    def forward_folded(self, x, n1, xb, stats):
        a = self.attn
        qkv = ops.linear(n1, a.qkv) if n1 is not None else ops.linear_lnfold(xb, stats, a.qkv, self.norm1)
        xb, stats = ops.linear_residual_(x, ops.vit_attention(qkv, a.heads), a.proj, self.ls1.gamma, stats)
        h = ops.linear_lnfold(xb, stats, self.mlp.fc1, self.norm2, gelu=True)
        return ops.linear_residual_(x, h, self.mlp.fc2, self.ls2.gamma, stats)

    def forward_fused_f32(self, x, n1s, next_norm):
        B, T, C = x.shape
        rows = B * T
        a, m = self.attn, self.mlp
        cq = ops._f32x3_weights(a.qkv)
        qkv_s = ops.linear_f32x3(n1s, cq[1], cq[2], rows, 3 * C, C, out="split")
        cp = ops._f32x3_weights(a.proj)
        y = ops.linear_f32x3(ops.vit_attention_f32_ss(qkv_s, B, T, a.heads), cp[1], cp[2], rows, C, C).reshape(B, T, C)
        n2s = ops.scale_residual_layernorm_f32_(x, y, self.ls1.gamma, self.norm2)
        c1, c2 = ops._f32x3_weights(m.fc1), ops._f32x3_weights(m.fc2)
        hs = ops.linear_f32x3(n2s, c1[1], c1[2], rows, 4 * C, C, gelu=True, out="split")
        y = ops.linear_f32x3(hs, c2[1], c2[2], rows, C, 4 * C).reshape(B, T, C)
        if next_norm is None:
            return ops.scale_residual_layernorm_f32_(x, y, self.ls2.gamma, None), None
        return x, ops.scale_residual_layernorm_f32_(x, y, self.ls2.gamma, next_norm)

    def forward(self, x):
        if torch.is_autocast_enabled() and x.dtype == torch.float32 and x.is_cuda and not ops.is_differentiable():
            x = x.contiguous()
            y = self.attn(ops.add_layernorm(x, None, self.norm1, torch.bfloat16))
            ops.scale_residual_(x, y, self.ls1.gamma)
            y = self.mlp(ops.add_layernorm(x, None, self.norm2, torch.bfloat16))
            return ops.scale_residual_(x, y, self.ls2.gamma)
        x = x + self.attn(self.norm1(x)) * self.ls1.gamma
        return x + self.mlp(self.norm2(x)) * self.ls2.gamma


class _PatchEmbed(nn.Module):
    def __init__(self, dim, patch):
        super().__init__()
        self.proj = nn.Conv2d(3, dim, patch, patch)


SPARSE_SINGLE_CROP = True
F32_PROLOGUE = True
F32_TAPS_SPLIT = True


class SplitTaps:

    def __init__(self, split, B, T, K):
        self.split, self.B, self.T, self.K = split, B, T, K


class ViT(nn.Module):

    def __init__(self, embed_dim=768, depth=12, num_heads=12, patch_size=14, img_size=224, reg_tokens=4):
        super().__init__()
        self.patch_size, self.depth = patch_size, depth
        self.patch_embed = _PatchEmbed(embed_dim, patch_size)
        self.cls_token = nn.Parameter(torch.zeros(1, 1, embed_dim))
        self.reg_token = nn.Parameter(torch.zeros(1, reg_tokens, embed_dim))
        self.pos_embed = nn.Parameter(torch.zeros(1, (img_size // patch_size) ** 2, embed_dim))
        self.blocks = nn.ModuleList([_Block(embed_dim, num_heads) for _ in range(depth)])
        self.norm = nn.LayerNorm(embed_dim, eps=1e-6)
        self.head = nn.Linear(embed_dim, 1000)

    def forward(self, x, taps_side_by_side=False):
        xa, xb = x if isinstance(x, (tuple, list)) else (x, None)
        if ops.vit_prologue_ok(xa, self) and (xb is None or xb.shape[1:] == xa.shape[1:]):
            x, n1, mean = ops.vit_prologue(xa, xb, self, self.blocks[0].norm1, row_mean=True)
            return self._fused_blocks(x, n1, taps_side_by_side, mean)
        if F32_PROLOGUE and ops.vit_prologue_f32_ok(xa, self) and (xb is None or xb.shape[1:] == xa.shape[1:]):
            x, ns = ops.vit_prologue_f32(xa, xb, self, self.blocks[0].norm1)
            return self._fused_blocks_f32(x, ns, taps_side_by_side)
        x = xa if xb is None else torch.cat([xa, xb], 0)
        B = x.shape[0]
        p = self.patch_size
        gh, gw = x.shape[2] // p, x.shape[3] // p
        patches = x.reshape(B, 3, gh, p, gw, p).permute(0, 2, 4, 1, 3, 5).reshape(B, gh * gw, 3 * p * p)
        x = ops.patch_embed(patches, self.patch_embed.proj)
        x = x + self.pos_embed
        x = torch.cat([self.cls_token.expand(B, -1, -1).to(x.dtype), self.reg_token.expand(B, -1, -1).to(x.dtype), x], 1)
        n = self.depth // 4
        taps = {self.depth - 1, self.depth - n - 1, self.depth - 2 * n - 1, self.depth - 3 * n - 1}
        outs = []
        if x.is_cuda and torch.is_autocast_enabled() and x.dtype == torch.float32 and x.shape[-1] % 4 == 0 \
                and not ops.is_differentiable():
            x = x.contiguous()
            return self._fused_blocks(x, ops.add_layernorm(x, None, self.blocks[0].norm1, torch.bfloat16), taps_side_by_side)
        if ops.vit_f32_fused_ok(x, self):
            x = x.contiguous()
            return self._fused_blocks_f32(x, ops.scale_residual_layernorm_f32_(x, None, None, self.blocks[0].norm1), taps_side_by_side)
        for i, blk in enumerate(self.blocks):
            x = blk(x)
            if i in taps:
                outs.append(ops.add_layernorm(x, None, self.norm)
                            if x.is_cuda and torch.is_autocast_enabled() and not ops.is_differentiable() else self.norm(x))
        return outs

    def _fused_blocks_f32(self, x, ns, taps_side_by_side):
        n = self.depth // 4
        taps = {self.depth - 1, self.depth - n - 1, self.depth - 2 * n - 1, self.depth - 3 * n - 1}
        outs = []
        wide = torch.empty(x.shape[0] * x.shape[1], 2 * 4 * x.shape[2], dtype=torch.bfloat16, device=x.device) if taps_side_by_side and F32_TAPS_SPLIT else None
        for i, blk in enumerate(self.blocks):
            x, ns = blk.forward_fused_f32(x, ns, self.blocks[i + 1].norm1 if i + 1 < len(self.blocks) else None)
            if i in taps:
                if wide is not None:
                    ops.scale_residual_layernorm_f32_(x, None, None, self.norm, wide=wide, block=len(outs))
                    outs.append(None)
                else:
                    outs.append(self.norm(x))
        return SplitTaps(wide, x.shape[0], x.shape[1], 4 * x.shape[2]) if wide is not None else outs


def _vit_fused_blocks(self, x, n1, taps_side_by_side, row_mean=None):
    n = self.depth // 4
    taps = {self.depth - 1, self.depth - n - 1, self.depth - 2 * n - 1, self.depth - 3 * n - 1}
    outs = []
    B, _, D = x.shape
    wide = torch.empty(B, x.shape[1], len(taps) * D, dtype=torch.bfloat16, device=x.device) if taps_side_by_side else None
    fold = ops.ln_fold_ok(B * x.shape[1], D, x.device)
    if fold and row_mean is None:
        row_mean = ops.fold_row_means(x)
    xb, stats = None, row_mean
    for i, blk in enumerate(self.blocks):
        nxt = self.blocks[i + 1].norm1 if i + 1 < len(self.blocks) else None
        if fold:
            xb, stats = blk.forward_folded(x, n1, xb, stats)
            n1 = None
        else:
            x, n1 = blk.forward_fused(x, n1, nxt)
        if i in taps:
            k = len(outs)
            outs.append(ops.add_layernorm(x, None, self.norm, out=None if wide is None else wide[:, :, k * D:(k + 1) * D]))
    return outs if wide is None else wide


ViT._fused_blocks = _vit_fused_blocks


def interpolate_pos_embed(pos_embed_ckpt, new_side):
    P0, C = pos_embed_ckpt.shape[-2:]
    s0 = int(P0 ** 0.5)
    if s0 == new_side:
        return pos_embed_ckpt
    t = pos_embed_ckpt.reshape(-1, s0, s0, C).permute(0, 3, 1, 2)
    t = F.interpolate(t, size=(new_side, new_side), mode="bicubic", align_corners=False)
    return t.permute(0, 2, 3, 1).flatten(1, 2)


class ViT_AE(nn.Module):

    def __init__(self, cfg):
        super().__init__()
        assert cfg.up_type == "linear" and cfg.use_pyramid_feat, "only the configured variant is built"
        assert "reg4" in cfg.vit_type and "patch14" in cfg.vit_type
        dims = {"vit_small": (384, 12, 6), "vit_base": (768, 12, 12), "vit_large": (1024, 24, 16)}
        D, depth, heads = dims[cfg.vit_type[:cfg.vit_type.index("_patch")]]
        assert D == cfg.embed_dim
        self.out_dim = cfg.out_dim
        self.img_size = cfg.get("img_size", 224)
        self.vit = ViT(D, depth, heads, 14, self.img_size)
        self.output_upscaling = nn.Linear(4 * D, 16 * cfg.out_dim, bias=True)
        if cfg.get("pretrained", False):
            self.load_dinov2(cfg.vit_ckpt)

    def load_dinov2(self, path):
        ck = torch.load(path, map_location="cpu")["model"]
        sd = self.vit.state_dict()
        for k in ("head.weight", "head.bias"):
            if k in ck and ck[k].shape != sd[k].shape:
                del ck[k]
        if "pos_embed" in ck:
            ck["pos_embed"] = interpolate_pos_embed(ck["pos_embed"], self.img_size // 14)
        self.vit.load_state_dict(ck, strict=False)

    def lowres_map(self, x):
        B, _, H, W = x.shape
        side = H // 14
        outs = self.vit(x)
        z = torch.cat([o[:, 5:, :] for o in outs], dim=2)
        z = ops.linear(z, self.output_upscaling).reshape(B, side, side, 4, 4, self.out_dim)
        return z.permute(0, 1, 3, 2, 4, 5).reshape(B, 4 * side, 4 * side, self.out_dim), (H, W)

    def upprojected(self, x):
        B, _, H, W = x.shape
        side = H // 14
        outs = self.vit(x)
        z = torch.cat([o[:, 5:, :] for o in outs], dim=2)
        return ops.linear(z, self.output_upscaling).reshape(B, side, side, 4, 4, self.out_dim), (H, W)

    def upprojected_tokens(self, x):
        B, _, H, W = x.shape
        return self.upproject(self.vit(x, taps_side_by_side=True), H, W)

    def upproject(self, outs, H, W):
        if isinstance(outs, SplitTaps):
            lin = self.output_upscaling
            c = ops._f32x3_weights(lin)
            z = ops.linear_f32x3(outs.split, c[1], c[2], outs.B * outs.T, lin.weight.shape[0], outs.K)
            return z.reshape(outs.B, outs.T, 4, 4, self.out_dim), (H, W), outs.T - (H // 14) * (W // 14)
        B = outs.shape[0] if torch.is_tensor(outs) else outs[0].shape[0]
        if torch.is_tensor(outs):
            z = ops.linear(outs, self.output_upscaling)
            return z.reshape(B, outs.shape[1], 4, 4, self.out_dim), (H, W), outs.shape[1] - (H // 14) * (W // 14)
        z = ops.linear(torch.cat([o[:, 5:, :] for o in outs], dim=2), self.output_upscaling)
        return z.reshape(B, -1, 4, 4, self.out_dim), (H, W), 0

    def pixel_features(self, x, choose):
        if x.is_cuda and self.out_dim == 256 and not ops.is_differentiable():
            if SPARSE_SINGLE_CROP and ops.sparse_upproj_ok(x) and x.shape[-1] == x.shape[-2] and x.shape[-1] % 14 == 0:
                sd = x.shape[-1] // 14
                npre = self.vit.cls_token.shape[1] + self.vit.reg_token.shape[1]
                plan = ops.upproj_plan(choose, x.shape[-2], x.shape[-1], sd, npre, npre + sd * sd)
                acts = self.vit(x, taps_side_by_side=True)
                if torch.is_tensor(acts) and acts.shape[1] == plan["tok_stride"]:
                    return ops.sparse_pixel_features(acts, self.output_upscaling, plan)
                z, (H, W), off = self.upproject(acts, x.shape[-2], x.shape[-1])
                return ops.bilinear_sample_native(z, choose, H, W, tok_offset=off)
            z, (H, W), off = self.upprojected_tokens(x)
            return ops.bilinear_sample_native(z, choose, H, W, tok_offset=off)
        low, (H, W) = self.lowres_map(x)
        return ops.bilinear_sample_pixels(low, choose, H, W)


class ViTEncoderOneRef(nn.Module):
    def __init__(self, cfg, npoint=None):
        super().__init__()
        self.npoint = npoint
        self.rgb_net = ViT_AE(cfg)


class SinusoidalPositionalEmbedding(nn.Module):
    def __init__(self, d_model):
        super().__init__()
        self.d_model = d_model
        div = torch.exp(torch.arange(0, d_model, 2).float() * (-math.log(10000.0) / d_model))
        self.register_buffer("div_term", div)


class GeometricStructureEmbedding(nn.Module):

    def __init__(self, cfg):
        super().__init__()
        self.sigma_d, self.sigma_a, self.angle_k = cfg.sigma_d, cfg.sigma_a, cfg.angle_k
        self.factor_a = 180.0 / (self.sigma_a * math.pi)
        self.embedding = SinusoidalPositionalEmbedding(cfg.hidden_dim)
        self.proj_d = nn.Linear(cfg.hidden_dim, cfg.hidden_dim)
        self.proj_a = nn.Linear(cfg.hidden_dim, cfg.hidden_dim)
        self.reduction_a = cfg.reduction_a
        if self.reduction_a not in ("max", "mean"):
            raise ValueError(f"Unsupported reduction mode: {self.reduction_a}.")

    def forward(self, points):
        return ops.geo_embedding(points, self)


class _MHA(nn.Module):
    def __init__(self, d, rpe):
        super().__init__()
        self.proj_q = nn.Linear(d, d)
        self.proj_k = nn.Linear(d, d)
        self.proj_v = nn.Linear(d, d)
        if rpe:
            self.proj_p = nn.Linear(d, d)


class _AttentionLayer(nn.Module):
    def __init__(self, d, rpe):
        super().__init__()
        self.attention = _MHA(d, rpe)
        self.linear = nn.Linear(d, d)
        self.norm = nn.LayerNorm(d)


class _AttentionOutput(nn.Module):
    def __init__(self, d):
        super().__init__()
        self.expand = nn.Linear(d, 2 * d)
        self.squeeze = nn.Linear(2 * d, d)
        self.norm = nn.LayerNorm(d)

    def forward(self, x, out=None):
        if x.is_cuda and not ops.is_differentiable():
            return ops.ffn_add_layernorm(x, self.expand, self.squeeze, self.norm, out=out)
        assert out is None
        return self.norm(x + ops.linear(ops.linear(x, self.expand, relu=True), self.squeeze))


class TransformerLayer(nn.Module):

    def __init__(self, d, rpe, heads=4):
        super().__init__()
        self.heads = heads
        self.attention = _AttentionLayer(d, rpe)
        self.output = _AttentionOutput(d)

    def forward(self, x, mem, embed=None, out=None):
        a = self.attention
        if mem is None:
            mem = x
        h = ops.token_attention(x, mem, a.attention, self.heads, embed)
        if x.is_cuda and not ops.is_differentiable():
            x = ops.linear_add_layernorm(h, a.linear, x, a.norm)
        else:
            x = a.norm(ops.linear(h, a.linear) + x)
        return self.output(x, out=out)


class GeometricTransformer(nn.Module):

    def __init__(self, d, heads=4):
        super().__init__()
        self.layers = nn.ModuleList([TransformerLayer(d, True, heads), TransformerLayer(d, False, heads)])

    def forward(self, f0, e0, f1, e1):
        e_all = _adjacent(e0, e1)
        if e_all is not None and f0.shape == f1.shape:
            f = _adjacent(f0, f1)
            f = self.forward_stacked(torch.cat([f0, f1], 0) if f is None else f, e_all)
            B = f0.shape[0]
            return f[:B], f[B:]
        f0 = self.layers[0](f0, f0, e0)
        f1 = self.layers[0](f1, f1, e1)
        f0 = self.layers[1](f0, f1)
        f1 = self.layers[1](f1, f0)
        return f0, f1

    def forward_stacked(self, f, e_all):
        B = f.shape[0] // 2
        f = self.layers[0](f, None, e_all)
        if ops.USE_STACKED_OUT and f.is_cuda and not ops.is_differentiable():
            out = torch.empty_like(f, memory_format=torch.contiguous_format)
            f0 = self.layers[1](f[:B], f[B:], out=out[:B])
            self.layers[1](f[B:], f0, out=out[B:])
            return out
        f0 = self.layers[1](f[:B], f[B:])
        return torch.cat([f0, self.layers[1](f[B:], f0)], 0)


def _adjacent(e0, e1):
    if (e0.shape != e1.shape or e0.dtype != e1.dtype or not e0.is_contiguous() or not e1.is_contiguous()
            or e0.untyped_storage().data_ptr() != e1.untyped_storage().data_ptr()
            or e1.storage_offset() != e0.storage_offset() + e0.numel()):
        return None
    return e0.as_strided((2 * e0.shape[0],) + tuple(e0.shape[1:]), e0.stride())


class _LinearAttention(nn.Module):
    def __init__(self, d):
        super().__init__()
        self.proj_q = nn.Linear(d, d)
        self.proj_k = nn.Linear(d, d)
        self.proj_v = nn.Linear(d, d)
        self.scale = nn.Parameter(torch.zeros(1, 1, d))


class _LinearAttentionLayer(nn.Module):
    def __init__(self, d):
        super().__init__()
        self.attention = _LinearAttention(d)
        self.linear = nn.Linear(d, d)
        self.norm = nn.LayerNorm(d)


class LinearTransformerLayer(nn.Module):

    def __init__(self, d, heads=4, focusing_factor=3):
        super().__init__()
        self.heads, self.focusing_factor = heads, focusing_factor
        self.attention = _LinearAttentionLayer(d)
        self.output = _AttentionOutput(d)

    def forward(self, x, mem, kv_skip=0):
        a = self.attention
        h = ops.focused_linear_attention(x, mem, a.attention, self.heads, self.focusing_factor, kv_skip=kv_skip)
        if x.is_cuda and not ops.is_differentiable():
            x = ops.linear_add_layernorm(h, a.linear, x, a.norm)
        else:
            x = a.norm(ops.linear(h, a.linear) + x)
        return self.output(x)


class SparseToDenseTransformer(nn.Module):

    def __init__(self, d, heads=4, focusing_factor=3):
        super().__init__()
        self.sparse_layer = GeometricTransformer(d, heads)
        self.dense_layer = LinearTransformerLayer(d, heads, focusing_factor)

    @staticmethod
    def _sample(dense, fps_idx):
        return torch.cat([dense[:, 0:1], ops.gather_rows(dense, fps_idx)], dim=1)

    def forward(self, d0, e0, i0, d1, e1, i1):
        f0, f1 = self.sparse_layer(self._sample(d0, i0), e0, self._sample(d1, i1), e1)
        if d0.shape == d1.shape and f0.shape == f1.shape:
            B = d0.shape[0]
            nn_ = self.dense_layer(torch.cat([d0[:, 1:], d1[:, 1:]], 0), torch.cat([f0[:, 1:], f1[:, 1:]], 0))
            n0, n1 = nn_[:B], nn_[B:]
        else:
            n0 = self.dense_layer(d0[:, 1:], f0[:, 1:])
            n1 = self.dense_layer(d1[:, 1:], f1[:, 1:])
        return torch.cat([f0[:, 0:1], n0], 1), torch.cat([f1[:, 0:1], n1], 1)

    def forward_stacked(self, dense, bg, e_all, idx_all):
        f = self.sparse_layer.forward_stacked(ops.gather_rows(dense, idx_all, off=1, alt=bg, prepend=True), e_all)
        if not ops.USE_STACKED_OUT:
            return self.dense_layer(dense, f[:, 1:].contiguous()), f[:, 0:1].contiguous()
        return self.dense_layer(dense, f, kv_skip=1), f[:, 0:1]


class _BN(nn.Module):
    def __init__(self, c):
        super().__init__()
        self.bn = nn.BatchNorm2d(c)


class _ConvBN(nn.Module):
    def __init__(self, cin, cout):
        super().__init__()
        self.conv = nn.Conv2d(cin, cout, 1, bias=False)
        self.normlayer = _BN(cout)

    def folded(self):
        bn = self.normlayer.bn
        s = bn.weight / torch.sqrt(bn.running_var + bn.eps)
        return self.conv.weight.reshape(self.conv.weight.shape[0], -1) * s[:, None], bn.bias - bn.running_mean * s


class _SharedMLP(nn.Module):
    def __init__(self, chans):
        super().__init__()
        for i in range(len(chans) - 1):
            self.add_module(f"layer{i}", _ConvBN(chans[i], chans[i + 1]))
        self.n = len(chans) - 1

    def layers(self):
        return [getattr(self, f"layer{i}") for i in range(self.n)]

    def forward(self, x):
        for l in self.layers():
            x = ops.bn_relu(ops.conv1x1(x, l.conv), l.normlayer.bn)
        return x

    def forward_pooled(self, x):
        ls = self.layers()
        for l in ls[:-1]:
            x = ops.bn_relu(ops.conv1x1(x, l.conv), l.normlayer.bn)
        return ops.bn_relu_maxpool(ops.conv1x1(x, ls[-1].conv), ls[-1].normlayer.bn)


class _Conv1d(nn.Module):
    def __init__(self, cin, cout):
        super().__init__()
        self.conv = nn.Conv1d(cin, cout, 1, bias=True)


class PositionalEncoding(nn.Module):

    def __init__(self, out_dim, r1, r2, nsample1, nsample2):
        super().__init__()
        self.r1, self.r2, self.ns1, self.ns2 = r1, r2, nsample1, nsample2
        self.mlp1 = _SharedMLP([6, 32, 64, 128])
        self.mlp2 = _SharedMLP([6, 32, 64, 128])
        self.mlp3 = _Conv1d(256, out_dim)

    def groups(self, pts):
        pts = pts.float()
        if ops.is_differentiable():
            with torch.autocast("cuda", enabled=False):
                f1 = self.mlp1.forward_pooled(ops.query_lrf_group(pts, self.r1, self.ns1))
                f2 = self.mlp2.forward_pooled(ops.query_lrf_group(pts, self.r2, self.ns2))
            return torch.cat([f1, f2], dim=1).transpose(1, 2)
        if pts.is_cuda and (torch.is_autocast_enabled() or ops.USE_F32X3) and self.r2 >= self.r1 and self.ns1 % 32 == 0 and self.ns2 % 32 == 0:
            g2, g1, _ = ops.pe_geometry(pts, self.r2, self.ns2, self.r1, self.ns1)
            f2 = ops.pe_mlp_max(pts, self.r2, self.ns2, self.mlp2, g2)
            f1 = ops.pe_mlp_max(pts, self.r1, self.ns1, self.mlp1, g1)
        else:
            f1 = ops.pe_group_mlp_max(pts, self.r1, self.ns1, self.mlp1)
            f2 = ops.pe_group_mlp_max(pts, self.r2, self.ns2, self.mlp2)
        return torch.cat([f1, f2], dim=2).float()

    def split_ok(self, pts):
        return (pts.is_cuda and torch.is_autocast_enabled() and not ops.is_differentiable() and ops.USE_F32X3 and self.r2 >= self.r1
                and self.ns1 % 32 == 0 and self.ns2 % 32 == 0 and self.mlp3.conv.weight.shape[0] % 256 == 0)

    def groups_split(self, pts, buf, b0):
        pts = pts.float()
        g2, g1, _ = ops.pe_geometry(pts, self.r2, self.ns2, self.r1, self.ns1)
        ops.pe_mlp_max(pts, self.r2, self.ns2, self.mlp2, g2, out_split=(buf, b0, 128))
        ops.pe_mlp_max(pts, self.r1, self.ns1, self.mlp1, g1, out_split=(buf, b0, 0))
        return buf

    def _mlp3_split(self):
        conv = self.mlp3.conv
        key = (conv.weight._version, conv.weight.data_ptr(), conv.bias._version)
        cache = getattr(conv, "_f32x3_cache", None)
        if cache is None or cache[0] != key:
            with torch.no_grad():
                cache = (key, ops.split_f32(conv.weight.detach().float().reshape(conv.weight.shape[0], -1).contiguous()),
                         conv.bias.detach().float().contiguous())
            conv._f32x3_cache = cache
        return cache

    def project_add(self, buf, d):
        cache = self._mlp3_split()
        rows = buf.shape[0] * buf.shape[1]
        N, K = self.mlp3.conv.weight.shape[0], buf.shape[2] // 2
        return ops.linear_f32x3_bf16(buf, cache[1], cache[2], rows, N, K, resid=d.contiguous()).reshape(buf.shape[0], buf.shape[1], N)

    def project(self, feat):
        w = self.mlp3.conv.weight.reshape(self.mlp3.conv.weight.shape[0], -1)
        N, K = w.shape
        rows = feat.numel() // K
        with torch.autocast("cuda", enabled=False):
            if feat.is_cuda and not ops.is_differentiable() and ops.f32x3_ok(rows, N, K):
                cache = self._mlp3_split()
                return ops.linear_f32x3(ops.split_f32(feat.float().reshape(rows, K).contiguous()), cache[1], cache[2], rows, N, K).reshape(*feat.shape[:-1], N)
# ... 5 lines not shown
```

### unopose_amd/model/unopose.py

```python

import torch
import torch.nn as nn
import torch.nn.functional as F

from .. import ops
from ..losses import aug_pose_noise, overlap_losses
from .config import to_cfg
from .modules import (GeometricStructureEmbedding, GeometricTransformer, PositionalEncoding,
                      SparseToDenseTransformer, ViTEncoderOneRef, _adjacent)


STACKED_FINE = True
PE_UNDER_COARSE = True
GEOM_UNDER_VIT = 1
LRF_UNDER_VIT = True
_SIDE_STREAMS = {}
COARSE_SLOT = True
TRAIN_PE_UNDER_COARSE = True


def _scores(scores, n1, halves=False):
    return ops.overlap_scores(scores, n1, halves=halves)


def _bg_row(mod, dtype):
    p = mod.bg_token
    key = (p._version, p.data_ptr(), dtype)
    c = getattr(mod, "_bg_cache", None)
    if c is None or c[0] != key:
        with torch.no_grad():
            c = (key, p.detach().reshape(-1).to(dtype).contiguous())
        mod._bg_cache = c
    return c[1]


def _block_outputs(out_proj, score_head, f1, f2, n1, temp):
    scores = score_head(torch.cat((f1, f2), dim=1))
    atten = ops.feature_similarity(ops.linear(f1, out_proj), ops.linear(f2, out_proj), temp)
    s1, s2 = scores[:, 1:(n1 + 1)], scores[:, (n1 + 2):]
    m1, m2 = ops.saliency_pair(atten, s1, s2)
    score = torch.clamp(torch.sigmoid(torch.cat((s1, s2), dim=1).squeeze(-1)), min=0, max=1)
    saliency = torch.clamp(torch.sigmoid(torch.cat((m1, m2), dim=1).squeeze(-1)), min=0, max=1)
    return atten, score, saliency


class CoarsePointMatchingOneRef(nn.Module):
    def __init__(self, cfg):
        super().__init__()
        self.cfg = cfg
        self.nblock = cfg.nblock
        self.in_proj = nn.Linear(cfg.input_dim, cfg.hidden_dim)
        self.out_proj = nn.Linear(cfg.hidden_dim, cfg.out_dim)
        self.bg_token = nn.Parameter(torch.randn(1, 1, cfg.hidden_dim) * 0.02)
        self.score_heads = nn.ModuleList([nn.Linear(cfg.hidden_dim, 1) for _ in range(self.nblock)])
        self.transformers = nn.ModuleList([GeometricTransformer(cfg.hidden_dim, 4) for _ in range(self.nblock)])
        self.taps = None

    def forward_train(self, p1, f1, geo1, p2, f2, geo2, radius, end_points):
        B, n1 = f1.shape[:2]
        bg = self.bg_token.expand(B, -1, -1)
        f1 = torch.cat([bg, ops.linear(f1, self.in_proj)], dim=1)
        f2 = torch.cat([bg, ops.linear(f2, self.in_proj)], dim=1)
        attens, scores, sals = [], [], []
        for blk, head in zip(self.transformers, self.score_heads):
            f1, f2 = blk(f1, geo1, f2, geo2)
            a, sc, sa = _block_outputs(self.out_proj, head, f1, f2, n1, self.cfg.temp)
            attens.append(a)
            scores.append(sc)
            sals.append(sa)
        gt_R = end_points["rotation_label"]
        gt_t = end_points["translation_label"] / (radius.reshape(-1, 1) + 1e-6)
        init_R, init_t = end_points["aug_pose"] if "aug_pose" in end_points else aug_pose_noise(gt_R, gt_t)
        overlap_losses(end_points, attens, scores, sals, p1, p2, gt_R, gt_t, self.cfg.loss_predator_thres,
                       self.cfg.loss_dis_thres, "coarse_hard")
        end_points["init_R"], end_points["init_t"] = init_R, init_t
        return end_points

    def forward(self, p1, f1, geo1, p2, f2, geo2, radius, end_points, slot=None):
        if self.training:
            return self.forward_train(p1, f1, geo1, p2, f2, geo2, radius, end_points)
        B, n1 = f1.shape[:2]
        if slot is not None and f1.is_cuda and torch.is_autocast_enabled():
            f = ops.set_first_rows_(ops.linear(slot, self.in_proj), _bg_row(self, torch.bfloat16))
            f1, f2 = f[:B], f[B:]
        else:
            f1 = ops.linear(f1, self.in_proj)
            f2 = ops.linear(f2, self.in_proj)
            bg = self.bg_token.expand(B, -1, -1).to(f1.dtype)
            f1 = torch.cat([bg, f1], dim=1)
            f2 = torch.cat([bg, f2], dim=1)
        for blk in self.transformers:
            f1, f2 = blk(f1, geo1, f2, geo2)
        f = _adjacent(f1, f2)
        if f is not None and f1.is_cuda:
            score = _scores(ops.score_head(f, self.score_heads[self.nblock - 1]), n1, halves=True)
            o = ops.linear(f, self.out_proj)
            atten = ops.feature_similarity(o[:B], o[B:], self.cfg.temp)
        else:
            scores = ops.score_head(torch.cat((f1, f2), dim=1), self.score_heads[self.nblock - 1])
            atten = ops.feature_similarity(ops.linear(f1, self.out_proj), ops.linear(f2, self.out_proj), self.cfg.temp)
            score = _scores(scores, n1)
        if self.taps is not None:
            self.taps.update(f1=f1, f2=f2, atten=atten, score=score)
        n1p, n2p = self.cfg.nproposal1, self.cfg.nproposal2
        rand = end_points.get("coarse_rand")
        if rand is None:
            rand = torch.rand(B, n1p * 3, device=p1.device)
        init_R, init_t, init_score = ops.coarse_pose(atten, score, p1, p2, rand, n1p, n2p)
        end_points["init_pose_score"] = init_score
        end_points["init_R"] = init_R
        end_points["init_t"] = init_t
        return end_points


class FinePointMatchingOneRef(nn.Module):
    def __init__(self, cfg):
        super().__init__()
        self.cfg = cfg
        self.nblock = cfg.nblock
        d = cfg.hidden_dim
        self.in_proj = nn.Linear(cfg.input_dim, d)
        self.out_proj = nn.Linear(d, cfg.out_dim)
        self.dis_proj = nn.Linear(2 * d, 3)
        self.bg_token = nn.Parameter(torch.randn(1, 1, d) * 0.02)
        assert cfg.use_lrf and cfg.use_xyz and not cfg.get("use_feature", False), "only the configured PE variant"
        self.PE = PositionalEncoding(d, cfg.pe_radius1, cfg.pe_radius2, cfg.get("nsample1", 32), cfg.get("nsample2", 64))
        self.score_heads = nn.ModuleList([nn.Linear(d, 1) for _ in range(self.nblock)])
        self.transformers = nn.ModuleList(
            [SparseToDenseTransformer(d, 4, cfg.focusing_factor) for _ in range(self.nblock)])
        self.taps = None

    def forward_train(self, p1, f1, geo1, fps_idx1, p2, f2, geo2, fps_idx2, radius, end_points, pe_ahead=None):
        B, n1 = p1.shape[:2]
        bg = self.bg_token.expand(B, -1, -1)
        if pe_ahead is None:
            p1_ = (p1 - end_points["init_t"].unsqueeze(1)) @ end_points["init_R"] if "init_R" in end_points else p1
            pe1, pe2 = self.PE(p1_), self.PE(p2)
        else:
            g1, g2, side = pe_ahead
            torch.cuda.current_stream().wait_stream(side)
            pe1, pe2 = self.PE.project(g1), self.PE.project(g2)
        f1 = torch.cat([bg, ops.linear(f1, self.in_proj) + pe1], dim=1)
        f2 = torch.cat([bg, ops.linear(f2, self.in_proj) + pe2], dim=1)
        attens, scores, sals = [], [], []
        for blk, head in zip(self.transformers, self.score_heads):
            f1, f2 = blk(f1, geo1, fps_idx1, f2, geo2, fps_idx2)
            a, sc, sa = _block_outputs(self.out_proj, head, f1, f2, n1, self.cfg.temp)
            attens.append(a)
            scores.append(sc)
            sals.append(sa)
        gt_R = end_points["rotation_label"]
        gt_t = end_points["translation_label"] / (radius.reshape(-1, 1) + 1e-6)
        overlap_losses(end_points, attens, scores, sals, p1, p2, gt_R, gt_t, self.cfg.loss_predator_thres,
                       self.cfg.loss_dis_thres, "fine")
        return end_points

    def forward(self, p1, f1, geo1, fps_idx1, p2, f2, geo2, fps_idx2, radius, end_points, pe2_groups=None):
        if self.training:
            return self.forward_train(p1, f1, geo1, fps_idx1, p2, f2, geo2, fps_idx2, radius, end_points, pe_ahead=pe2_groups)
        B, n1 = p1.shape[:2]
        if "init_R" in end_points and "init_t" in end_points:
            p1_ = ops.rigid_rows(p1, end_points["init_t"], end_points["init_R"])
        else:
            p1_ = p1
        e_all, f_all = _adjacent(geo1, geo2), _adjacent(f1, f2)
        if (STACKED_FINE and p1_.shape == p2.shape and p1.is_cuda and e_all is not None
                and fps_idx1.shape == fps_idx2.shape):
            d = ops.linear(f_all if f_all is not None else torch.cat([f1, f2], 0), self.in_proj)
            if self.PE.split_ok(p1_) and d.dtype == torch.bfloat16 and (pe2_groups is None or isinstance(pe2_groups, tuple)):
                if pe2_groups is None:
                    buf = self.PE.groups_split(torch.cat([p1_, p2], 0), torch.empty(2 * B, p2.shape[1], 512, dtype=torch.bfloat16, device=p2.device), 0)
                else:
                    buf = self.PE.groups_split(p1_, pe2_groups[1], 0)
                d = self.PE.project_add(buf, d)
            else:
                pe = self.PE(torch.cat([p1_, p2], 0)) if pe2_groups is None else \
                    self.PE.project(torch.cat([self.PE.groups(p1_), pe2_groups], 0))
                d = d + pe.to(d.dtype)
            bg = _bg_row(self, d.dtype).reshape(1, 1, -1).expand(2 * B, -1, -1)
            idx_all = torch.cat([fps_idx1, fps_idx2], 0)
            for blk in self.transformers:
                d, bg = blk.forward_stacked(d, bg, e_all, idx_all)
            f = torch.cat([bg, d], dim=1)
            f1, f2 = f[:B], f[B:]
            sc = ops.score_head(f, self.score_heads[self.nblock - 1])
            o = ops.linear(f, self.out_proj)
            if self.taps is None and ops.fine_pose_fused_ok(o[:B], o[B:]):
                R, t, s = ops.fine_pose_from_features(o[:B], o[B:], self.cfg.temp, _scores(sc, n1, halves=True), p1, p2)
                return self._finish(end_points, R, t, s, radius)
            scores = torch.cat((sc[:B], sc[B:]), dim=1)
            atten = ops.feature_similarity(o[:B], o[B:], self.cfg.temp)
        else:
            if p1_.shape == p2.shape:
                pe = self.PE(torch.cat([p1_, p2], 0))
                pe1, pe2 = pe[:B], pe[B:]
            else:
                pe1, pe2 = self.PE(p1_), self.PE(p2)
            f1 = ops.linear(f1, self.in_proj) + pe1.to(f1.dtype)
            f2 = ops.linear(f2, self.in_proj) + pe2.to(f2.dtype)
            bg = self.bg_token.expand(B, -1, -1).to(f1.dtype)
            f1 = torch.cat([bg, f1], dim=1)
            f2 = torch.cat([bg, f2], dim=1)
            for blk in self.transformers:
                f1, f2 = blk(f1, geo1, fps_idx1, f2, geo2, fps_idx2)
            scores = ops.score_head(torch.cat((f1, f2), dim=1), self.score_heads[self.nblock - 1])
            o1, o2 = ops.linear(f1, self.out_proj), ops.linear(f2, self.out_proj)
            if self.taps is None and ops.fine_pose_fused_ok(o1, o2):
                R, t, s = ops.fine_pose_from_features(o1, o2, self.cfg.temp, _scores(scores, n1), p1, p2)
                return self._finish(end_points, R, t, s, radius)
            atten = ops.feature_similarity(o1, o2, self.cfg.temp)
        score = _scores(scores, n1)
        if self.taps is not None:
            self.taps.update(f1=f1, f2=f2, atten=atten, score=score)
        R, t, s = ops.fine_pose(atten, score, p1, p2)
        return self._finish(end_points, R, t, s, radius)

    @staticmethod
    def _finish(end_points, R, t, s, radius):
        end_points["pred_R"] = R
        end_points["pred_t"] = ops.scale_by_radius(t, radius, multiply=True)
        end_points["pred_pose_score"] = s
        return end_points


class UNOPose(nn.Module):
    def __init__(self, cfg):
        super().__init__()
        cfg = to_cfg(cfg)
        self.cfg = cfg
        self.coarse_npoint = cfg.coarse_npoint
        self.fine_npoint = cfg.fine_npoint
        self.use_ref_rad = cfg.get("use_ref_rad", False)
        self.test_coarse_only = cfg.get("test_coarse_only", False)
        self.feature_extraction = ViTEncoderOneRef(cfg.feature_extraction, self.fine_npoint)
        self.geo_embedding = GeometricStructureEmbedding(cfg.geo_embedding)
        self.coarse_point_matching = CoarsePointMatchingOneRef(cfg.coarse_point_matching)
        self.fine_point_matching = FinePointMatchingOneRef(cfg.fine_point_matching)
        self.taps = None
        self.fixed_init = None
        self._zero_rows = {}
        self.internal_overlap = True

    def _features(self, end_points):
        rgb, choose = end_points["rgb"], end_points["rgb_choose"]
        assert choose.size(1) == self.fine_npoint
        net = self.feature_extraction.rgb_net
        dense_pm = end_points["pts"]
        if "dense_po" in end_points and "dense_fo" in end_points:
            dense_fm = net.pixel_features(rgb, choose)
            dense_po, dense_fo = end_points["dense_po"].clone(), end_points["dense_fo"].clone()
            radius = ops.cloud_radius(dense_po)
            dense_pm = ops.scale_by_radius(dense_pm, radius)
            dense_po = ops.scale_by_radius(dense_po, radius)
            return dense_pm, dense_fm, dense_po, dense_fo, radius, None
        if "ref_dense_po" in end_points:
            radius = end_points["ref_radius"]
            dense_pm = ops.scale_by_radius(dense_pm, radius)
            return dense_pm, net.pixel_features(rgb, choose), end_points["ref_dense_po"], end_points["ref_dense_fo"], radius, None
        tem_rgb, tem_choose, tem_pts = end_points["tem1_rgb"], end_points["tem1_choose"], end_points["tem1_pts"]
        radius = ops.cloud_radius(tem_pts)
        dense_pm = ops.scale_by_radius(dense_pm, radius)
        tem_n = ops.scale_by_radius(tem_pts, radius)
        main = torch.cuda.current_stream()
        side = self._side_stream(tem_n.device)
        side.wait_stream(main)
        with torch.cuda.stream(side):
            idx_o = ops.furthest_point_sample(tem_n, self.fine_npoint)
            dense_po = ops.gather_rows(tem_n, idx_o)
            sparse_up = (ops.sparse_upproj_ok(rgb) and idx_o.shape == choose.shape and net.out_dim == 256 and rgb.shape == tem_rgb.shape
                         and tem_choose.dtype == choose.dtype and tem_choose.is_contiguous())
            if sparse_up:
                both_choose = torch.empty(2 * choose.shape[0], choose.shape[1], dtype=choose.dtype, device=choose.device)
                both_choose[:choose.shape[0]].copy_(choose)
                sel_choose = ops.gather_rows(tem_choose.unsqueeze(-1), idx_o, out=both_choose[choose.shape[0]:].unsqueeze(-1)).squeeze(-1)
            else:
                sel_choose = torch.gather(tem_choose, 1, idx_o.long())
            for t in (idx_o, dense_po, sel_choose):
                t.record_stream(main)
            plan = None
            if sparse_up:
                sd = rgb.shape[-1] // 14
                npre = net.vit.cls_token.shape[1] + net.vit.reg_token.shape[1]
                both_choose.record_stream(main)
                plan = ops.upproj_plan(both_choose, rgb.shape[-2], rgb.shape[-1], sd, npre, npre + sd * sd)
                for t in plan.values():
                    if torch.is_tensor(t):
                        t.record_stream(main)
            pre = None
            if GEOM_UNDER_VIT and self.internal_overlap:
                pre = {}
                pre["idx_m"] = ops.furthest_point_sample(dense_pm, self.coarse_npoint)
                pre["idx_o"] = ops.furthest_point_sample(dense_po, self.coarse_npoint)
                pre["sparse_pm"] = ops.gather_rows(dense_pm.float(), pre["idx_m"])
                pre["sparse_po"] = ops.gather_rows(dense_po.float(), pre["idx_o"])
                if GEOM_UNDER_VIT > 1 or LRF_UNDER_VIT:
                    pre["sparse_pm_lrf"] = ops.gather_rows(ops.lrf_global(end_points["pts"], self.use_ref_rad), pre["idx_m"])
                    pre["sparse_po_lrf"] = ops.gather_rows(ops.lrf_global(tem_pts, self.use_ref_rad), pre["idx_o"])
                if GEOM_UNDER_VIT > 1:
                    bg_point = torch.ones(dense_pm.size(0), 1, 3, device=dense_pm.device)
                    pre["geo"] = self.geo_embedding(torch.cat([torch.cat([bg_point, pre["sparse_pm_lrf"]], dim=1),
                                                               torch.cat([bg_point, pre["sparse_po_lrf"]], dim=1)], dim=0))
                for t in pre.values():
                    t.record_stream(main)
        B = rgb.shape[0]
        if plan is not None:
            acts = net.vit((rgb, tem_rgb), taps_side_by_side=True)
            if torch.is_tensor(acts) and acts.shape[1] == plan["tok_stride"]:
                main.wait_stream(side)
                both = ops.sparse_pixel_features(acts, net.output_upscaling, plan)
                return dense_pm, both[:B], dense_po, both[B:], radius, pre
            z, (H, W), off = net.upproject(acts, rgb.shape[-2], rgb.shape[-1])
        else:
            z, (H, W), off = net.upproject(net.vit((rgb, tem_rgb), taps_side_by_side=True), rgb.shape[-2], rgb.shape[-1])
        both = torch.empty(2 * B, choose.shape[1], 256, dtype=torch.float32, device=z.device) \
            if sel_choose.shape == choose.shape else None
        dense_fm = ops.bilinear_sample_native(z[:B], choose, H, W, out=None if both is None else both[:B], tok_offset=off)
        main.wait_stream(side)
        dense_fo = ops.bilinear_sample_native(z[B:], sel_choose, H, W, out=None if both is None else both[B:], tok_offset=off)
        return dense_pm, dense_fm, dense_po, dense_fo, radius, pre

    @torch.no_grad()
    def encode_reference(self, tem1_rgb, tem1_choose, tem1_pts):
        radius = ops.cloud_radius(tem1_pts)
        tem_n = ops.scale_by_radius(tem1_pts, radius)
        idx_o = ops.furthest_point_sample(tem_n, self.fine_npoint)
        sel_choose = torch.gather(tem1_choose, 1, idx_o.long())
        net = self.feature_extraction.rgb_net
        return dict(ref_dense_po=ops.gather_rows(tem_n, idx_o), ref_dense_fo=net.pixel_features(tem1_rgb, sel_choose),
                    ref_radius=radius, ref_lrf=ops.lrf_global(tem1_pts, self.use_ref_rad))

    def _side_stream(self, device):
        cur = torch.cuda.current_stream(device)
        key = (torch.device(device).index if torch.device(device).index is not None else torch.cuda.current_device(), cur.cuda_stream)
        if key not in _SIDE_STREAMS:
            _SIDE_STREAMS[key] = torch.cuda.Stream(device=device)
        return _SIDE_STREAMS[key]

    def _sample_wlrf(self, pts, pts_lrf, feats, npoint):
        idx = ops.furthest_point_sample(pts, npoint)
        return ops.gather_rows(pts.float(), idx), ops.gather_rows(pts_lrf, idx), ops.gather_rows(feats, idx), idx

    def _lowres_train(self, rgb):
        net = self.feature_extraction.rgb_net
        frozen = not any(p.requires_grad for p in net.vit.parameters())
        if frozen:
            with torch.no_grad(), ops.differentiable(False):
                taps = net.vit(rgb)
        else:
            taps = net.vit(rgb)
        B, _, H, W = rgb.shape
        side = H // 14
        z = torch.cat([o[:, 5:, :] for o in taps], dim=2).float()
        z = ops.linear(z, net.output_upscaling).reshape(B, side, side, 4, 4, net.out_dim)
        return z.permute(0, 1, 3, 2, 4, 5).reshape(B, 4 * side, 4 * side, net.out_dim)

    def _pixel_features_train(self, rgb, choose):
        return ops.bilinear_sample_pixels(self._lowres_train(rgb), choose, rgb.shape[-2], rgb.shape[-1])

    def forward_train(self, end_points):
        tem_pts = end_points["tem1_pts"]
        radius = torch.norm(tem_pts - tem_pts.mean(1, keepdim=True), dim=2).max(1)[0]
        scale = radius.reshape(-1, 1, 1) + 1e-6
        dense_pm, tem_n = end_points["pts"] / scale, tem_pts / scale
        main = torch.cuda.current_stream() if dense_pm.is_cuda else None
        side = self._side_stream(dense_pm.device) if main is not None and self.internal_overlap else None
        geo = {}

        def geometry():
            with torch.no_grad():
                geo["idx_o"] = ops.furthest_point_sample(tem_n, self.fine_npoint)
                geo["dense_po"] = ops.gather_rows(tem_n, geo["idx_o"])
                geo["sel_choose"] = torch.gather(end_points["tem1_choose"], 1, geo["idx_o"].long())
                geo["pm_lrf"] = ops.lrf_global(end_points["pts"], self.use_ref_rad)
                geo["po_lrf"] = ops.lrf_global(tem_pts, self.use_ref_rad)
                geo["fps_m"] = ops.furthest_point_sample(dense_pm, self.coarse_npoint)
                geo["fps_o"] = ops.furthest_point_sample(geo["dense_po"], self.coarse_npoint)

        if side is not None:
            side.wait_stream(main)
            with torch.cuda.stream(side):
                geometry()
                for t in geo.values():
                    t.record_stream(main)
            low_m = self._lowres_train(end_points["rgb"])
            low_o = self._lowres_train(end_points["tem1_rgb"])
            main.wait_stream(side)
        else:
            geometry()
            low_m = self._lowres_train(end_points["rgb"])
            low_o = self._lowres_train(end_points["tem1_rgb"])
        H, W = end_points["rgb"].shape[-2:]
        dense_po = geo["dense_po"]
        dense_fm = ops.bilinear_sample_pixels(low_m, end_points["rgb_choose"], H, W)
        dense_fo = ops.bilinear_sample_pixels(low_o, geo["sel_choose"], H, W)
        B = dense_pm.size(0)
        bg_point = torch.ones(B, 1, 3, device=dense_pm.device)
        fps_idx_m, fps_idx_o = geo["fps_m"], geo["fps_o"]
        sparse_pm, sparse_pm_lrf, sparse_fm = ops.gather_rows(dense_pm.float(), fps_idx_m), ops.gather_rows(geo["pm_lrf"], fps_idx_m), ops.gather_rows(dense_fm, fps_idx_m)
        sparse_po, sparse_po_lrf, sparse_fo = ops.gather_rows(dense_po.float(), fps_idx_o), ops.gather_rows(geo["po_lrf"], fps_idx_o), ops.gather_rows(dense_fo, fps_idx_o)
        pe_ahead = None
        if side is not None and TRAIN_PE_UNDER_COARSE:
            if "aug_pose" not in end_points:
                end_points["aug_pose"] = aug_pose_noise(end_points["rotation_label"], end_points["translation_label"] / (radius.reshape(-1, 1) + 1e-6))
            init_R, init_t = end_points["aug_pose"]
            side.wait_stream(main)
            with torch.cuda.stream(side):
                PE = self.fine_point_matching.PE
                g1 = PE.groups((dense_pm - init_t.unsqueeze(1)) @ init_R)
                g2 = PE.groups(dense_po)
            g1.record_stream(main)
            g2.record_stream(main)
            pe_ahead = (g1, g2, side)
        geo_m = self.geo_embedding(torch.cat([bg_point, sparse_pm_lrf], dim=1))
        geo_o = self.geo_embedding(torch.cat([bg_point, sparse_po_lrf], dim=1))
        end_points = self.coarse_point_matching(sparse_pm, sparse_fm, geo_m, sparse_po, sparse_fo, geo_o, radius, end_points)
        return self.fine_point_matching(dense_pm, dense_fm, geo_m, fps_idx_m, dense_po, dense_fo, geo_o, fps_idx_o, radius,
                                        end_points, pe2_groups=pe_ahead)

    def forward(self, end_points):
        if self.training:
            with ops.differentiable():
                return self.forward_train(end_points)
        return self.forward_matching(end_points, self.forward_features(end_points))

    def forward_features(self, end_points):
        try:
            return self._features(end_points)
        finally:
            ops.clear_split_memo()

    def forward_matching(self, end_points, feats):
        try:
            return self._matching_half(end_points, feats)
        finally:
            ops.clear_split_memo()

    def _matching_half(self, end_points, feats):
        dense_pm, dense_fm, dense_po, dense_fo, radius, pre = feats
        if pre is not None:
            return self._forward_from(pre, end_points, dense_pm, dense_fm, dense_po, dense_fo, radius)
        dense_pm_lrf = ops.lrf_global(end_points["pts"], self.use_ref_rad)
        if "ref_lrf" in end_points:
            dense_po_lrf = end_points["ref_lrf"]
        else:
            dense_po_lrf = ops.lrf_global(end_points["tem1_pts"], self.use_ref_rad) if "tem1_pts" in end_points \
                else ops.lrf_global(end_points["dense_po"], self.use_ref_rad)
        B = dense_pm.size(0)
        bg_point = torch.ones(B, 1, 3, device=dense_pm.device)
        sparse_pm, sparse_pm_lrf, sparse_fm, fps_idx_m = self._sample_wlrf(dense_pm, dense_pm_lrf, dense_fm,
                                                                         self.coarse_npoint)
        sparse_po, sparse_po_lrf, sparse_fo, fps_idx_o = self._sample_wlrf(dense_po, dense_po_lrf, dense_fo,
                                                                         self.coarse_npoint)
        pre = dict(idx_m=fps_idx_m, idx_o=fps_idx_o, sparse_pm=sparse_pm, sparse_po=sparse_po,
                   sparse_pm_lrf=sparse_pm_lrf, sparse_po_lrf=sparse_po_lrf, sparse_fm=sparse_fm, sparse_fo=sparse_fo)
        return self._forward_from(pre, end_points, dense_pm, dense_fm, dense_po, dense_fo, radius)

    def _forward_from(self, pre, end_points, dense_pm, dense_fm, dense_po, dense_fo, radius):
        B = dense_pm.size(0)
        bg_point = torch.ones(B, 1, 3, device=dense_pm.device)
        fps_idx_m, fps_idx_o = pre["idx_m"], pre["idx_o"]
        if self.taps is not None:
            self.taps.update(fps_idx_m=fps_idx_m, fps_idx_o=fps_idx_o, dense_pm=dense_pm, dense_fm=dense_fm,
                             dense_po=dense_po, dense_fo=dense_fo, radius=radius)
        if "sparse_pm_lrf" not in pre:
            po_lrf = end_points["ref_lrf"] if "ref_lrf" in end_points else ops.lrf_global(
                end_points["tem1_pts"] if "tem1_pts" in end_points else end_points["dense_po"], self.use_ref_rad)
            pre = dict(pre, sparse_pm_lrf=ops.gather_rows(ops.lrf_global(end_points["pts"], self.use_ref_rad), fps_idx_m),
                       sparse_po_lrf=ops.gather_rows(po_lrf, fps_idx_o))
        sparse_pm, sparse_po, sparse_pm_lrf, sparse_po_lrf = (pre[k] for k in ("sparse_pm", "sparse_po", "sparse_pm_lrf",
                                                                                  "sparse_po_lrf"))
        slot = None
        if ("sparse_fm" not in pre and "sparse_fo" not in pre and COARSE_SLOT and dense_fm.is_cuda and torch.is_autocast_enabled() and not ops.is_differentiable()
                and dense_fm.dtype == dense_fo.dtype and dense_fm.shape[2:] == dense_fo.shape[2:] and fps_idx_m.shape == fps_idx_o.shape
                and dense_fm.is_contiguous() and dense_fo.is_contiguous()):
            n, C = fps_idx_m.shape[1], dense_fm.shape[2]
            slot = torch.empty(2 * B, n + 1, C, dtype=dense_fm.dtype, device=dense_fm.device)
            zr = self._zero_row(C, dense_fm.dtype, dense_fm.device).expand(B, C)
            ops.gather_rows(dense_fm, fps_idx_m, alt=zr, prepend=True, out=slot[:B])
            ops.gather_rows(dense_fo, fps_idx_o, alt=zr, prepend=True, out=slot[B:])
            sparse_fm, sparse_fo = slot[:B, 1:], slot[B:, 1:]
        else:
            sparse_fm = pre["sparse_fm"] if "sparse_fm" in pre else ops.gather_rows(dense_fm, fps_idx_m)
            sparse_fo = pre["sparse_fo"] if "sparse_fo" in pre else ops.gather_rows(dense_fo, fps_idx_o)
        if "geo" in pre:
            geo = pre["geo"]
        else:
            geo = self._geo(bg_point, sparse_pm_lrf, sparse_po_lrf)
        return self._matching(end_points, geo, B, sparse_pm, sparse_fm, sparse_po, sparse_fo, fps_idx_m, fps_idx_o,
                              dense_pm, dense_fm, dense_po, dense_fo, radius, slot=slot)

    def _zero_row(self, C, dtype, device):
        key = (C, dtype, str(device))
        z = self._zero_rows.get(key)
        if z is None:
            z = self._zero_rows[key] = torch.zeros(C, dtype=dtype, device=device)
        return z

    def _geo(self, bg_point, sparse_pm_lrf, sparse_po_lrf):
        return self.geo_embedding(torch.cat([torch.cat([bg_point, sparse_pm_lrf], dim=1),
                                             torch.cat([bg_point, sparse_po_lrf], dim=1)], dim=0))

    def _matching(self, end_points, geo, B, sparse_pm, sparse_fm, sparse_po, sparse_fo, fps_idx_m, fps_idx_o, dense_pm,
                  dense_fm, dense_po, dense_fo, radius, slot=None):
        geo_m, geo_o = geo[:B], geo[B:]
        pe2 = None
        if (PE_UNDER_COARSE and self.internal_overlap and not self.test_coarse_only and dense_pm.is_cuda and torch.is_autocast_enabled()
                and dense_pm.shape == dense_po.shape):
            main = torch.cuda.current_stream()
            side = self._side_stream(dense_po.device)
            side.wait_stream(main)
            with torch.cuda.stream(side):
                PE = self.fine_point_matching.PE
                if PE.split_ok(dense_po) and STACKED_FINE:
                    buf = torch.empty(2 * B, dense_po.shape[1], 512, dtype=torch.bfloat16, device=dense_po.device)
                    pe2 = ("split", PE.groups_split(dense_po, buf, B))
                    buf.record_stream(main)
                else:
                    pe2 = PE.groups(dense_po)
                    pe2.record_stream(main)
        end_points = self.coarse_point_matching(sparse_pm, sparse_fm, geo_m, sparse_po, sparse_fo, geo_o, radius,
                                                end_points, slot=slot)
        if pe2 is not None:
            torch.cuda.current_stream().wait_stream(self._side_stream(dense_po.device))
        if self.fixed_init is not None:
            if self.taps is not None:
                self.taps.update(own_init_R=end_points["init_R"], own_init_t=end_points["init_t"])
            end_points["init_R"], end_points["init_t"] = self.fixed_init
        if self.test_coarse_only:
            end_points["pred_R"] = end_points["init_R"]
            end_points["pred_t"] = end_points["init_t"] * (radius.reshape(-1, 1) + 1e-6)
            end_points["pred_pose_score"] = end_points["init_pose_score"]
            return end_points
        return self.fine_point_matching(dense_pm, dense_fm, geo_m, fps_idx_m, dense_po, dense_fo, geo_o, fps_idx_o,
                                        radius, end_points, pe2_groups=pe2)
```

### unopose_amd/ops/__init__.py

```python
import sys
import types

from . import _state
from .common import (
    _c, differentiable, is_differentiable, _fallbacks_seen, note_fallback, _params_key, _SPLIT_MEMO, _MUTATION_EPOCH, note_mutation,
    clear_split_memo, _aligned16, _no_autograd, _f32_path, _own_f32, _own_glue,
)
from .dense import (
    linear_backend, _bf16_weights, linear_bf16_hip, own_gemm_ok, bf16_linear_2d, f32x3_ok, split_f32, _f32x3_weights, linear_f32x3,
    linear_f32x3_bf16, linear_f32_raw, _transposed_weights, _LinearFn, _ZERO_BIAS, _zero_bias, linear_train, _lin, mlp, linear,
    ffn_add_layernorm, linear_add_layernorm, patch_embed, vit_prologue_ok, vit_prologue, vit_prologue_f32_ok, vit_prologue_f32, bmm_nt_f32, score_head, add_layernorm,
    scale_residual_, scale_residual_layernorm_f32_, vit_f32_fused_ok, scale_residual_layernorm_, ln_fold_ok, _fold_producer_weights,
    _fold_consumer_weights, linear_residual_, linear_lnfold, fold_shift, fold_row_means, _into,
)
from .attention import (
    vit_attention, vit_attention_f32_split, vit_attention_f32_ss, vit_attention_torch, _KEY_PAD, token_attention,
    _token_attention_hip_f32, _attn_weights, _token_attention_hip, token_attention_torch, _key_pad, _transpose_pad_f32, _TokenAttnFn,
    token_attention_train_ok, _token_attention_train, focused_linear_attention,
    _focused_linear_attention_hip_f32, _focused_linear_attention_hip, focused_linear_attention_torch,
)
from .geometry import (
    lrf_global, query_lrf_group, lrf_group_idx, weighted_procrustes, cloud_radius, scale_by_radius, gather_rows, pairwise_distance,
    _bf16_split, _mfma_fragment_order, _GEO_HINV, _GEO_D_RANGE, _GEO_TABLE_UNAVAILABLE, _geo_tables, geo_embedding, geo_embedding_torch,
    pe_group_mlp_max, pe_group_mlp_max_unfused, pe_geometry, pe_mlp_max, _pe_image, furthest_point_sample, _geo_grid, _GeoEmbedFn, geo_embedding_train_ok,
)
from .sampling import (
    bilinear_sample_native, sparse_upproj_ok, upproj_plan, sparse_pixel_features, bilinear_sample_pixels,
)
from .pose import (
    overlap_scores, set_first_rows_, pose_score, rigid_rows, feature_similarity, soft_assignment, coarse_pose_torch, fine_pose_torch, _assign_labels, _check_score_width,
    coarse_pose, fine_pose, fine_pose_fused_ok, normalize_rows_bf16, normalize_rows_f32, fine_pose_from_features,
)
from .prep import (
    PrepPlan, _desc_ints, _tap_table, prep_norm_table, _require, _result, prep_crop_resize, prep_lift, prep_gather,
)
from .score import vsd_counts, pose_errors, pose_metrics, adi, gt_visibility, pts_extent
from .train import (
    _InfoNCEFn, infonce_two_way, _BNReLUTrain, bn_relu, _BNReLUMaxPoolTrain, bn_relu_maxpool, _SaliencyFn, saliency_pair,
    nearest_partner, _CONV_FWD_PAIRS, _CONV_WGRAD_PAIRS, _conv1x1_pair_ok, _conv1x1_wgrad_ok, _Conv1x1Fn, conv1x1,
)

_SWITCHES = frozenset(['FORBID_LIBRARY_BF16_GEMM', 'GEO_TABLE', 'GEO_TABLE_F32', 'HIP_GEMM_ALL', 'PIXEL_FEATS_BF16', 'TRAIN_FUSED_SALIENCY', 'TRAIN_OWN_ATTN', 'TRAIN_OWN_CONV', 'TRAIN_OWN_GEMM', 'TRAIN_OWN_GEMM_MIN_FLOP', 'TRAIN_OWN_GEO', 'TRAIN_OWN_WGRAD', 'TRAIN_OWN_WGRAD_MIN_ROWS', 'USE_F32X3', 'USE_FUSED_BN_RELU', 'USE_FUSED_FINE', 'USE_FUSED_INFONCE', 'USE_FUSED_LINEAR_LN', 'USE_HIP_GEMM', 'USE_KV_VT', 'USE_LA_KV_STATE', 'USE_LN_FOLD', 'USE_OWN_TOPK', 'USE_SPARSE_UPPROJ', 'USE_STACKED_OUT', '_DIFF'])


class _OpsModule(types.ModuleType):

    def __getattr__(self, name):
        if name in _SWITCHES:
            return getattr(_state, name)
        raise AttributeError(f"module {self.__name__!r} has no attribute {name!r}")

    def __setattr__(self, name, value):
        if name in _SWITCHES:
            setattr(_state, name, value)
        else:
            super().__setattr__(name, value)

    def __delattr__(self, name):
        if name in _SWITCHES:
            raise AttributeError(f"{name} is a switch of ops._state and cannot be deleted")
        super().__delattr__(name)


sys.modules[__name__].__class__ = _OpsModule
```

### unopose_amd/ops/dense.py

```python
import ctypes

import torch
import torch.nn.functional as F

from .._lib import call, lib, on_device, ptr, stream_ptr
from . import _state as st
from .common import _MUTATION_EPOCH, _SPLIT_MEMO, _aligned16, _c, _f32_path, _no_autograd, _params_key, note_fallback, note_mutation


def linear_backend():
    if st.USE_HIP_GEMM and st.HIP_GEMM_ALL:
        return "csrc/gemm.hip (256x256x64 LDS-DMA tiles, persistent; bias / bias + erf-GELU epilogue) for every ViT linear"
    if st.USE_HIP_GEMM:
        return "hipBLASLt (through torch); fc1 + GELU: csrc/gemm.hip (256x256x64 LDS-DMA tiles, fused bias + erf-GELU epilogue)"
    return "hipBLASLt (through torch)"


def _bf16_weights(lin):
    key = _params_key(lin)
    cache = getattr(lin, "_bf16_cache", None)
    if cache is None or cache[0] != key:
        with torch.no_grad():
            b32 = torch.zeros(lin.weight.shape[0], device=lin.weight.device) if lin.bias is None else lin.bias.detach().float().contiguous()
            cache = (key, lin.weight.detach().to(torch.bfloat16).contiguous(),
# ... 243 lines not shown
        y = linear_f32x3(hs, c2[1], c2[2], rows, N2, K2).reshape(*x.shape[:-1], N2)
        if out is not None and out.dtype == x.dtype and out.shape == x.shape and out.stride(-1) == 1 and out.is_contiguous():
            return add_layernorm(y, x, norm, out=out)
        return _into(out, add_layernorm(y, x, norm))
    return linear_add_layernorm(linear(x, expand, relu=True), squeeze, x, norm, out=out)


def _into(out, y):
    if out is None:
        return y
    note_mutation()
    out.copy_(y)
    return out


def linear_add_layernorm(h, lin, x, norm, out=None):
    N, K = lin.weight.shape
    rows = h.numel() // K
    if (st.USE_FUSED_LINEAR_LN and not st._DIFF and h.is_cuda and torch.is_autocast_enabled() and st.HIP_GEMM_ALL and N == 256
            and own_gemm_ok(rows, N, K) and tuple(norm.normalized_shape) == (256,) and norm.weight is not None and norm.bias is not None and lin.bias is not None):
        cache = _bf16_weights(lin)
        with torch.autocast("cuda", enabled=False):
            hb = _c(h if h.dtype == torch.bfloat16 else h.to(torch.bfloat16)).reshape(rows, K)
            xb = _c(x if x.dtype == torch.bfloat16 else x.to(torch.bfloat16)).reshape(rows, N)
            direct = out is not None and out.dtype == torch.bfloat16 and out.is_contiguous() and out.numel() == rows * N and out.device == h.device
            if direct:
                note_mutation()
            y = out if direct else torch.empty(rows, N, dtype=torch.bfloat16, device=h.device)
            with on_device(h.device):
                call("unopose_linear_add_layernorm_bf16", ptr(hb), ptr(cache[1]), ptr(cache[3]), ptr(xb), ptr(norm.weight.detach()),
                     ptr(norm.bias.detach()), float(norm.eps), ptr(y), rows, K, stream_ptr())
        return out if direct else _into(out, y.reshape(*h.shape[:-1], N))
    if out is not None and h.is_cuda and not st._DIFF and out.shape == x.shape and out.is_contiguous() and out.dtype in (torch.float32, torch.bfloat16):
        y = linear(h, lin)
        if y.dtype in (torch.float32, torch.bfloat16) and (out.dtype == (torch.bfloat16 if torch.is_autocast_enabled() else y.dtype)):
            return add_layernorm(y, x, norm, out=out)
        return _into(out, add_layernorm(y, x, norm))
    return _into(out, add_layernorm(linear(h, lin), x, norm))


def patch_embed(patches, conv):
    w = conv.weight.reshape(conv.weight.shape[0], -1)
    D, K = w.shape
    rows = patches.numel() // K
    if _f32_path(patches) and f32x3_ok(rows, D, 32):
        Kp = (K + 31) // 32 * 32
        key = _params_key(conv, Kp, "f32")
        cache = getattr(conv, "_f32x3_pad_cache", None)
        if cache is None or cache[0] != key:
            with torch.no_grad():
                wp = torch.zeros(D, Kp, dtype=torch.float32, device=w.device)
                wp[:, :K] = w.detach()
                b = torch.zeros(D, device=w.device) if conv.bias is None else conv.bias.detach().float().contiguous()
                cache = (key, split_f32(wp), b)
            conv._f32x3_pad_cache = cache
        a = torch.zeros(rows, Kp, dtype=torch.float32, device=patches.device)
        a[:, :K] = patches.reshape(rows, K)
        return linear_f32x3(split_f32(a), cache[1], cache[2], rows, D, Kp).reshape(*patches.shape[:-1], D)
    if st._DIFF or not (st.HIP_GEMM_ALL and patches.is_cuda and torch.is_autocast_enabled() and own_gemm_ok(rows, D, 64)):
        return F.linear(patches, w, conv.bias)
    Kp = (K + 63) // 64 * 64
    key = _params_key(conv, Kp)
    cache = getattr(conv, "_bf16_pad_cache", None)
    if cache is None or cache[0] != key:
        with torch.no_grad():
            wp = torch.zeros(D, Kp, dtype=torch.bfloat16, device=w.device)
            wp[:, :K] = w.detach()
            b = torch.zeros(D, device=w.device) if conv.bias is None else conv.bias.detach().float().contiguous()
        cache = (key, wp, b)
        conv._bf16_pad_cache = cache
    with torch.autocast("cuda", enabled=False):
        a = torch.zeros(rows, Kp, dtype=torch.bfloat16, device=patches.device)
        a[:, :K] = patches.reshape(rows, K)
        return linear_bf16_hip(a, cache[1], cache[2]).reshape(*patches.shape[:-1], D)


def vit_prologue_ok(xa, vit):
    return (not st._DIFF and xa.is_cuda and torch.is_autocast_enabled() and st.HIP_GEMM_ALL and st.USE_HIP_GEMM and xa.dtype == torch.float32
            and vit.pos_embed.shape[-1] == 768 and xa.shape[-1] == xa.shape[-2] and xa.shape[-1] % 14 == 0
            and vit.pos_embed.shape[1] == (xa.shape[-1] // 14) ** 2)


def vit_prologue(xa, xb, vit, norm1, row_mean=False):
    conv = vit.patch_embed.proj
    w = conv.weight.reshape(conv.weight.shape[0], -1)
    D, K = w.shape
    Kp = (K + 63) // 64 * 64
    key = _params_key(conv, Kp, vit.cls_token._version, vit.reg_token._version)
    cache = getattr(conv, "_prologue_cache", None)
    if cache is None or cache[0] != key:
        with torch.no_grad():
            wp = torch.zeros(D, Kp, dtype=torch.bfloat16, device=w.device)
            wp[:, :K] = w.detach()
            b = torch.zeros(D, device=w.device) if conv.bias is None else conv.bias.detach().float().contiguous()
            prefix = torch.cat([vit.cls_token.detach().float().reshape(-1, D), vit.reg_token.detach().float().reshape(-1, D)], 0).contiguous()
        cache = (key, wp, b, prefix)
        conv._prologue_cache = cache
    _, wp, b, prefix = cache
    na, nb = xa.shape[0], 0 if xb is None else xb.shape[0]
    S = xa.shape[-1]
    P = (S // 14) ** 2
    npre = prefix.shape[0]
    dev = xa.device
    with torch.autocast("cuda", enabled=False), on_device(dev):
        a = torch.empty((na + nb) * P, Kp, dtype=torch.bfloat16, device=dev)
        call("unopose_patchify_bf16", ptr(_c(xa)), na, None if xb is None else ptr(_c(xb)), nb, S, Kp, ptr(a), stream_ptr())
        y = linear_bf16_hip(a, wp, b)
        x = torch.empty(na + nb, npre + P, D, dtype=torch.float32, device=dev)
        n1 = torch.empty(na + nb, npre + P, D, dtype=torch.bfloat16, device=dev)
        rows = (na + nb) * (npre + P)
        mean = torch.zeros((rows + 255) // 256 * 256, dtype=torch.float32, device=dev) if row_mean else None
        call("unopose_vit_tokens_layernorm", ptr(y), ptr(vit.pos_embed.detach().float().contiguous()), ptr(prefix), npre, P, na + nb, D,
             ptr(norm1.weight.detach()), ptr(norm1.bias.detach()), float(norm1.eps), ptr(x), ptr(n1), None if mean is None else ptr(mean),
             stream_ptr())
    return (x, n1, mean) if row_mean else (x, n1)


def vit_prologue_f32_ok(xa, vit):
    if not (not st._DIFF and _no_autograd() and xa.is_cuda and not torch.is_autocast_enabled() and st.USE_F32X3 and xa.dtype == torch.float32
            and vit.pos_embed.shape[-1] == 768 and xa.shape[-1] == xa.shape[-2] and xa.shape[-1] % 14 == 0
            and vit.pos_embed.shape[1] == (xa.shape[-1] // 14) ** 2):
        return False
    rows = 2 * xa.shape[0] * (vit.pos_embed.shape[1] + 5)
    return f32x3_ok(rows, 768, 608) and f32x3_ok(rows, 3 * 768, 768) and f32x3_ok(rows, 768, 4 * 768)


def vit_prologue_f32(xa, xb, vit, norm1):
    conv = vit.patch_embed.proj
    w = conv.weight.reshape(conv.weight.shape[0], -1)
    D, K = w.shape
    Kp = (K + 31) // 32 * 32
    key = _params_key(conv, Kp, "f32", vit.cls_token._version, vit.reg_token._version, vit.pos_embed._version)
    cache = getattr(conv, "_prologue_cache_f32", None)
    if cache is None or cache[0] != key:
        with torch.no_grad():
            wp = torch.zeros(D, Kp, dtype=torch.float32, device=w.device)
            wp[:, :K] = w.detach()
            b = torch.zeros(D, device=w.device) if conv.bias is None else conv.bias.detach().float().contiguous()
            prefix = torch.cat([vit.cls_token.detach().float().reshape(-1, D), vit.reg_token.detach().float().reshape(-1, D)], 0).contiguous()
            cache = (key, split_f32(wp), b, prefix, vit.pos_embed.detach().float().contiguous())
        conv._prologue_cache_f32 = cache
    _, ws, b, prefix, pos = cache
    na, nb = xa.shape[0], 0 if xb is None else xb.shape[0]
    S = xa.shape[-1]
    P = (S // 14) ** 2
    npre = prefix.shape[0]
    dev = xa.device
    note_mutation()
    with on_device(dev):
        a = torch.empty((na + nb) * P, 2 * Kp, dtype=torch.bfloat16, device=dev)
        call("unopose_patchify_split", ptr(_c(xa)), na, None if xb is None else ptr(_c(xb)), nb, S, Kp, ptr(a), stream_ptr())
        y = linear_f32x3(a, ws, b, (na + nb) * P, D, Kp)
        x = torch.empty(na + nb, npre + P, D, dtype=torch.float32, device=dev)
        n1 = torch.empty((na + nb) * (npre + P), 2 * D, dtype=torch.bfloat16, device=dev)
        call("unopose_vit_tokens_layernorm_f32", ptr(y), ptr(pos), ptr(prefix), npre, P, na + nb, D, ptr(norm1.weight.detach()),
             ptr(norm1.bias.detach()), float(norm1.eps), ptr(x), ptr(n1), stream_ptr())
    return x, n1


def bmm_nt_f32(a, b, alpha=1.0):
    assert a.dtype == torch.float32 and b.dtype == torch.float32 and a.dim() == b.dim() and a.dim() in (3, 4)
    if a.dim() == 3:
        a4, b4 = a.unsqueeze(1), b.unsqueeze(1)
    else:
        a4, b4 = a, b
    Bo, Bi, n, K = a4.shape
    m = b4.shape[2]
    out = torch.empty(Bo, Bi, n, m, dtype=torch.float32, device=a.device)
    with on_device(a.device):
        call("unopose_bmm_f32", ptr(a4), a4.stride(0), a4.stride(1), a4.stride(2), a4.stride(3), ptr(b4), b4.stride(0), b4.stride(1),
             b4.stride(2), b4.stride(3), ptr(out), Bo, Bi, n, m, K, float(alpha), stream_ptr())
    return out if a.dim() == 4 else out[:, 0]


def score_head(x, lin):
    if _f32_path(x) and st.USE_F32X3 and x.shape[-1] == 256:
        key = (lin.weight._version, lin.weight.data_ptr(), None if lin.bias is None else lin.bias._version, "f32")
        cache = getattr(lin, "_rowdot_cache_f32", None)
        if cache is None or cache[0] != key:
            cache = (key, lin.weight.detach().float().reshape(-1).contiguous(), 0.0 if lin.bias is None else float(lin.bias.detach().float().item()))
            lin._rowdot_cache_f32 = cache
        xc = _c(x)
        out = torch.empty(*x.shape[:-1], 1, dtype=torch.float32, device=x.device)
        with on_device(x.device):
            call("unopose_row_dot", ptr(xc), 0, ptr(cache[1]), cache[2], xc.numel() // 256, 256, ptr(out), 0, stream_ptr())
        return out
    if st._DIFF or not (st.HIP_GEMM_ALL and x.is_cuda and torch.is_autocast_enabled()):
        return lin(x)
    with torch.autocast("cuda", enabled=False):
        key = (lin.weight._version, lin.weight.data_ptr(), None if lin.bias is None else lin.bias._version)
        cache = getattr(lin, "_rowdot_cache", None)
        if cache is None or cache[0] != key:
            cache = (key, lin.weight.detach().to(torch.bfloat16).float().reshape(-1).contiguous(),
                     0.0 if lin.bias is None else float(lin.bias.detach().float().item()))
            lin._rowdot_cache = cache
        if x.shape[-1] == 256 and x.dtype in (torch.bfloat16, torch.float32):
            xc = _c(x)
            out = torch.empty(*x.shape[:-1], 1, dtype=torch.bfloat16, device=x.device)
            with on_device(x.device):
                call("unopose_row_dot", ptr(xc), int(x.dtype == torch.bfloat16), ptr(cache[1]), cache[2], xc.numel() // 256, 256, ptr(out), 1,
                     stream_ptr())
            return out
        return ((x.float() * cache[1]).sum(-1, keepdim=True) + cache[2]).to(torch.bfloat16)


def add_layernorm(a, b, norm, out_dtype=None, out=None):
    a = _c(a)
    C = a.shape[-1]
    rows = a.numel() // C
    if b is not None:
        b = _c(b)
        assert b.shape == a.shape
    if out is not None:
        note_mutation()
    if out is None:
        if out_dtype is None:
            out_dtype = torch.bfloat16 if torch.is_autocast_enabled() else a.dtype
        out = torch.empty(a.shape, dtype=out_dtype, device=a.device)
        ld = C
    else:
        out_dtype = out.dtype
        ld = out.stride(-2)
        assert out.shape == a.shape and out.stride(-1) == 1 and ld >= C
        exp = ld
        for d in range(out.dim() - 2, -1, -1):
            assert out.stride(d) == exp or out.shape[d] == 1, "out rows must be uniformly strided"
            exp *= out.shape[d]
    ok = (torch.float32, torch.bfloat16)
    assert a.dtype in ok and out_dtype in ok and (b is None or b.dtype in ok) and a.is_cuda
    with on_device(a.device):
        call("unopose_add_layernorm_strided", ptr(a), int(a.dtype == torch.bfloat16), ptr(b) if b is not None else None,
             int(b is not None and b.dtype == torch.bfloat16), ptr(norm.weight), ptr(norm.bias), rows, C,
             float(norm.eps), ptr(out), int(out_dtype == torch.bfloat16), int(ld), stream_ptr())
    return out


def scale_residual_(x, y, gamma):
    note_mutation()
    assert x.dtype == torch.float32 and x.is_contiguous() and y.dtype == torch.bfloat16
    y = _c(y)
    C = x.shape[-1]
    with on_device(x.device):
        call("unopose_scale_residual", ptr(x), ptr(y), ptr(gamma), x.numel() // C, C, stream_ptr())
    return x


def scale_residual_layernorm_f32_(x, y, gamma, norm, wide=None, block=0):
    note_mutation()
    assert x.dtype == torch.float32 and x.is_contiguous() and (y is None or y.dtype == torch.float32)
    C = x.shape[-1]
    rows = x.numel() // C
    ld, dst = 0, None
    if wide is not None:
        assert norm is not None and wide.dtype == torch.bfloat16 and wide.is_contiguous() and wide.shape[0] == rows and wide.shape[1] % (2 * C) == 0
        ld = wide.shape[1] * 2
        assert 0 <= block < wide.shape[1] // (2 * C)
        dst = ctypes.c_void_p(wide.data_ptr() + block * C * 4)
    out = None if (norm is None or wide is not None) else torch.empty(rows, 2 * C, dtype=torch.bfloat16, device=x.device)
    with on_device(x.device):
        call("unopose_scale_residual_layernorm_f32", ptr(x), None if y is None else ptr(_c(y)), None if y is None else ptr(gamma),
             None if norm is None else ptr(norm.weight), None if norm is None else ptr(norm.bias), rows, C,
             0.0 if norm is None else float(norm.eps), dst if wide is not None else (None if out is None else ptr(out)), ld, stream_ptr())
    return x if norm is None else (wide if wide is not None else out)


def vit_f32_fused_ok(x, vit):
    C = x.shape[-1]
    return (x.is_cuda and x.dtype == torch.float32 and not st._DIFF and _no_autograd() and not torch.is_autocast_enabled() and st.USE_F32X3 and C % 32 == 0
            and C <= 1024 and C % 64 == 0 and f32x3_ok(x.numel() // C, 3 * C, C) and f32x3_ok(x.numel() // C, C, 4 * C))


def scale_residual_layernorm_(x, y, gamma, norm):
    note_mutation()
    assert x.dtype == torch.float32 and x.is_contiguous() and y.dtype == torch.bfloat16
    y = _c(y)
    C = x.shape[-1]
    out = torch.empty(x.shape, dtype=torch.bfloat16, device=x.device)
    with on_device(x.device):
        call("unopose_scale_residual_layernorm", ptr(x), ptr(y), ptr(gamma), ptr(norm.weight), ptr(norm.bias),
             x.numel() // C, C, float(norm.eps), ptr(out), stream_ptr())
    return out


def ln_fold_ok(rows, C, device=None):
    if not (st.USE_LN_FOLD and st.USE_HIP_GEMM and st.HIP_GEMM_ALL) or C % 256 != 0 or C // 256 > 4 or rows * C * 4 >= 2 ** 31:
        return False
    n_cu = torch.cuda.get_device_properties(torch.cuda.current_device() if device is None else device).multi_processor_count & ~7
    return ((rows + 255) // 256) * (C // 256) >= n_cu * 5 // 8


def _fold_producer_weights(lin, gamma):
    key = (lin.weight._version, lin.weight.data_ptr(), lin.weight.device, None if lin.bias is None else lin.bias._version, gamma._version, gamma.data_ptr())
    cache = getattr(lin, "_fold_prod_cache", None)
    if cache is None or cache[0] != key:
        with torch.no_grad():
            g = gamma.detach().float()
            w = (lin.weight.detach().float() * g[:, None]).to(torch.bfloat16).contiguous()
            b = (torch.zeros_like(g) if lin.bias is None else lin.bias.detach().float() * g).contiguous()
        cache = (key, w, b)
        lin._fold_prod_cache = cache
    return cache


def _fold_consumer_weights(lin, norm):
    key = (lin.weight._version, lin.weight.data_ptr(), lin.weight.device, None if lin.bias is None else lin.bias._version,
           norm.weight._version, norm.weight.data_ptr(), norm.bias._version)
    cache = getattr(lin, "_fold_cons_cache", None)
    if cache is None or cache[0] != key:
        with torch.no_grad():
            w32 = lin.weight.detach().float()
            w = (w32 * norm.weight.detach().float()[None, :]).to(torch.bfloat16).contiguous()
            c = w.float().sum(1).contiguous()
            d = (w32.double() @ norm.bias.detach().double()).float()
            if lin.bias is not None:
                d = d + lin.bias.detach().float()
            d = d.contiguous()
        cache = (key, w, c, d)
        lin._fold_cons_cache = cache
    return cache


def linear_residual_(x, a, lin, gamma, prev=None):
    note_mutation()
    _, w, b = _fold_producer_weights(lin, gamma)
    C, K = w.shape
    rows = x.numel() // C
    rows_p = (rows + 255) // 256 * 256
    assert x.dtype == torch.float32 and x.is_contiguous() and a.dtype == torch.bfloat16 and a.numel() == rows * K
    prev_parts = 0
    if prev is not None:
        assert prev.dtype == torch.float32 and prev.device == x.device and prev.shape[0] == rows_p and prev.is_contiguous()
        if prev.dim() == 3:
            prev_parts = prev.shape[1]
            assert prev_parts == C // 256 and prev.untyped_storage().nbytes() >= (prev.storage_offset() + prev.numel() + rows_p) * 4
        else:
            assert prev.dim() == 1
    a = _c(a)
    xb = torch.empty(x.shape, dtype=torch.bfloat16, device=x.device)
    buf = torch.empty(rows_p * (2 * (C // 256) + 1), dtype=torch.float32, device=x.device)
    stats = buf[:rows_p * 2 * (C // 256)].view(rows_p, C // 256, 2)
    with on_device(x.device):
        call("unopose_linear_bf16_residual", ptr(a), ptr(w), ptr(b), ptr(x), ptr(xb), ptr(stats), None if prev is None else ptr(prev), prev_parts,
             rows, C, K, stream_ptr())
    return xb, stats


def fold_shift(stats):
    return torch.as_strided(stats, (stats.shape[0],), (1,), stats.storage_offset() + stats.numel())


def fold_row_means(x):
    C = x.shape[-1]
    rows = x.numel() // C
    mean = torch.zeros((rows + 255) // 256 * 256, dtype=torch.float32, device=x.device)
    with torch.autocast(x.device.type, enabled=False):
        torch.mean(x.reshape(rows, C), 1, out=mean[:rows])
    return mean


def linear_lnfold(xb, stats, lin, norm, gelu=False):
    _, w, c, d = _fold_consumer_weights(lin, norm)
    N, K = w.shape
    rows = xb.numel() // K
    out = torch.empty(*xb.shape[:-1], N, dtype=torch.bfloat16, device=xb.device)
    with on_device(xb.device):
        call("unopose_linear_bf16_lnfold", ptr(xb), ptr(w), ptr(d), ptr(c), ptr(stats), K // 256, float(norm.eps), ptr(out), rows, N, K, int(gelu), stream_ptr())
    return out
```

### unopose_amd/ops/sampling.py

```python
import torch

from .._lib import call, on_device, ptr, stream_ptr
from . import _state as st
from .common import _c, note_mutation
from .dense import _bf16_weights


def bilinear_sample_native(z, choose, H, W, out=None, tok_offset=0):
    z = _c(z)
    assert z.shape[-1] == 256 and z.shape[-2] == 4 and z.shape[-3] == 4 and z.dtype in (torch.float32, torch.bfloat16)
    if out is not None:
        note_mutation()
    B = z.shape[0]
    if z.dim() == 5:
        tok_stride = z.shape[1]
        side = int(round((tok_stride - tok_offset) ** 0.5))
        assert side * side + tok_offset == tok_stride
    else:
        assert z.dim() == 6 and tok_offset == 0
        side = z.shape[1]
        tok_stride = side * side
    choose = _c(choose.long())
    Np = choose.shape[1]
    if out is None:
        out = torch.empty(B, Np, 256, dtype=torch.float32, device=z.device)
    assert out.shape == (B, Np, 256) and out.dtype == torch.float32 and out.is_contiguous()
    with on_device(z.device):
        call("unopose_bilinear_sample_tokens", ptr(z), int(z.dtype == torch.bfloat16), ptr(choose), B, side, Np, int(H),
             int(W), int(tok_offset), int(tok_stride), ptr(out), stream_ptr())
    return out


def sparse_upproj_ok(x):
    return st.USE_SPARSE_UPPROJ and x.is_cuda and torch.is_autocast_enabled() and not st._DIFF


def upproj_plan(choose, H, W, side, tok_offset, tok_stride):
    choose = _c(choose.long())
    B2, Np = choose.shape
    cells = 16 * side * side
    cap_rows = (B2 * min(4 * Np, cells) + 16 * 256 + 255) // 256 * 256
    dev = choose.device
    i32 = dict(dtype=torch.int32, device=dev)
    plan = dict(choose=choose, H=int(H), W=int(W), side=int(side), tok_offset=int(tok_offset), tok_stride=int(tok_stride),
                cap_rows=cap_rows, ws=torch.empty(B2 * (cells + 32), **i32), row_list=torch.empty(cap_rows, **i32),
                cellmap=torch.empty(B2 * cells, **i32), tile_info=torch.empty(18, **i32))
    with on_device(dev):
        call("unopose_upproj_plan", ptr(choose), B2, Np, int(H), int(W), int(side), int(tok_offset), int(tok_stride), cap_rows,
             ptr(plan["ws"]), ptr(plan["row_list"]), ptr(plan["cellmap"]), ptr(plan["tile_info"]), stream_ptr())
    return plan


def sparse_pixel_features(acts, lin, plan, out=None):
    acts = _c(acts)
    if out is not None:
        note_mutation()
    B2, ts, K = acts.shape
    assert acts.dtype == torch.bfloat16 and ts == plan["tok_stride"] and B2 == plan["choose"].shape[0]
    cache = _bf16_weights(lin)
    w, bias = cache[1], cache[3]
    N = w.shape[0]
    assert N == 16 * 256 and w.shape[1] == K
    Np = plan["choose"].shape[1]
    dev = acts.device
    if out is None:
        out = torch.empty(B2, Np, 256, dtype=torch.bfloat16 if st.PIXEL_FEATS_BF16 else torch.float32, device=dev)
    assert out.shape == (B2, Np, 256) and out.dtype in (torch.float32, torch.bfloat16) and out.is_contiguous()
    with on_device(dev):
        cells = torch.empty(plan["cap_rows"], 256, dtype=torch.bfloat16, device=dev)
        call("unopose_linear_bf16_gather", ptr(acts), B2 * ts, K, ptr(w), N, ptr(bias), ptr(plan["row_list"]),
             ptr(plan["tile_info"]), plan["cap_rows"] // 256, ptr(cells), stream_ptr())
        call("unopose_bilinear_sample_compact", ptr(cells), ptr(plan["cellmap"]), ptr(plan["choose"]), B2, plan["side"], Np,
             plan["H"], plan["W"], ptr(out), int(out.dtype == torch.bfloat16), stream_ptr())
    return out


def bilinear_sample_pixels(low, choose, H, W):
    B, h, w, C = low.shape
    ys = torch.div(choose, W, rounding_mode="floor")
    xs = choose - ys * W

    def src(dst, n_in, n_out):
        s = (dst.float() + 0.5) * (n_in / n_out) - 0.5
        s = s.clamp(min=0.0)
        i0 = s.floor().long().clamp(max=n_in - 1)
        i1 = torch.where(i0 < n_in - 1, i0 + 1, i0)
        l1 = s - i0.float()
        return i0, i1, l1

    y0, y1, ly = src(ys, h, H)
    x0, x1, lx = src(xs, w, W)
    flat = low.reshape(B, h * w, C)

    def g(yy, xx):
        return torch.gather(flat, 1, (yy * w + xx).unsqueeze(2).expand(-1, -1, C)).float()

    lx, ly = lx.unsqueeze(2), ly.unsqueeze(2)
    top = (1 - lx) * g(y0, x0) + lx * g(y0, x1)
    bot = (1 - lx) * g(y1, x0) + lx * g(y1, x1)
    return (1 - ly) * top + ly * bot
```

Before: 1111 pairs/s.

## Fold ViT tap LayerNorms into the gathered upscaling GEMM with segmented stats

The ViT residual GEMM now writes its bf16 output straight into a wide side-by-side tap buffer (strided ldxb) and keeps its per-row LayerNorm partial stats. The sparse upscaling projection then runs a new gathered GEMM epilogue that applies a per-segment LayerNorm fold, rescaling accumulators at each segment boundary. The separate per-tap LayerNorm and concat passes are no longer materialised. In exchange the kernel gets extra LDS, a per-segment division rescale inside the K loop, and new precision behaviour from folding the norm into bf16 weights.

After: 1121 pairs/s (median of 6 runs). Within noise of the previous version (+0.9%).

```diff
diff --git a/include/unopose_hip.h b/include/unopose_hip.h
--- a/include/unopose_hip.h
+++ b/include/unopose_hip.h
@@ -280,6 +280,13 @@
                                  int prev_nparts, long M, int N, int K, unopose_stream_t stream);
 int unopose_linear_bf16_lnfold(const void *A, const void *W, const float *dvec, const float *cvec, const float *stats, int nparts, float eps,
                                void *C, long M, int N, int K, int gelu, unopose_stream_t stream);
+int unopose_linear_bf16_residual_ld(const void *A, const void *W, const float *bias, float *xres, void *xb, int ldxb, float *stats,
+                                    const float *prev, int prev_nparts, long M, int N, int K, unopose_stream_t stream);
+int unopose_linear_bf16_lnfold_ld(const void *A, int lda, const void *W, const float *dvec, const float *cvec, const float *stats, int nparts,
+                                  float eps, void *C, long M, int N, int K, int gelu, unopose_stream_t stream);
+int unopose_linear_bf16_gather_lnfold(const void *A, long M, int K, int segments, const void *W, int N, const float *dvec, const float *cvec,
+                                      const float *stats, float eps, const int *row_list, const int *tile_info, int max_tiles, void *C,
+                                      unopose_stream_t stream);
 int unopose_gemm_fold_stagger(int eighth_ticks_per_ktile);
 
 int unopose_bmm_f32(const float *A, long sab, long sah, long sai, long sak, const float *Bm, long sbb, long sbh, long sbj, long sbk,
diff --git a/unopose_amd/_lib.py b/unopose_amd/_lib.py
--- a/unopose_amd/_lib.py
+++ b/unopose_amd/_lib.py
@@ -82,6 +82,9 @@
     "unopose_gemm_fold_stagger": [_I],
     "unopose_linear_bf16_residual": [_P, _P, _P, _P, _P, _P, _P, _I, ctypes.c_long, _I, _I, _P],
     "unopose_linear_bf16_lnfold": [_P, _P, _P, _P, _P, _I, _F, _P, ctypes.c_long, _I, _I, _I, _P],
+    "unopose_linear_bf16_residual_ld": [_P, _P, _P, _P, _P, _I, _P, _P, _I, ctypes.c_long, _I, _I, _P],
+    "unopose_linear_bf16_lnfold_ld": [_P, _I, _P, _P, _P, _P, _I, _F, _P, ctypes.c_long, _I, _I, _I, _P],
+    "unopose_linear_bf16_gather_lnfold": [_P, ctypes.c_long, _I, _I, _P, _I, _P, _P, _P, _F, _P, _P, _I, _P, _P],
     "unopose_patchify_bf16": [_P, _I, _P, _I, _I, _I, _P, _P],
     "unopose_patchify_split": [_P, _I, _P, _I, _I, _I, _P, _P],
     "unopose_vit_tokens_layernorm": [_P, _P, _P, _I, _I, _I, _I, _P, _P, _F, _P, _P, _P, _P],
diff --git a/unopose_amd/csrc/gemm.hip b/unopose_amd/csrc/gemm.hip
--- a/unopose_amd/csrc/gemm.hip
+++ b/unopose_amd/csrc/gemm.hip
@@ -138,7 +138,14 @@
 
 int unopose_linear_bf16_residual(const void *A, const void *W, const float *bias, float *xres, void *xb, float *stats, const float *prev,
                                  int prev_nparts, long M, int N, int K, unopose_stream_t stream) {
+  return unopose_linear_bf16_residual_ld(A, W, bias, xres, xb, N, stats, prev, prev_nparts, M, N, K, stream);
+}
+
+int unopose_linear_bf16_residual_ld(const void *A, const void *W, const float *bias, float *xres, void *xb, int ldxb, float *stats,
+                                    const float *prev, int prev_nparts, long M, int N, int K, unopose_stream_t stream) {
   UNOPOSE_REQUIRE(A && W && bias && xres && xb && stats, "linear_bf16_residual: null pointer");
+  UNOPOSE_REQUIRE(ldxb >= N && ldxb % 8 == 0 && (size_t)M * ldxb * 2 < (1UL << 32),
+                  "linear_bf16_residual: the row stride of xb must cover a row, be a multiple of 8 elements and keep xb below 4 GiB (ldxb=%d)", ldxb);
   UNOPOSE_REQUIRE(prev != stats && (prev_nparts == 0 || (prev && prev_nparts * GEMM_BN == N && prev_nparts <= GEMM_LNF_MAXPARTS)),
                   "linear_bf16_residual: prev must be another buffer with 0 or N / 256 <= %d partials per row (got prev_nparts=%d N=%d)",
                   GEMM_LNF_MAXPARTS, prev_nparts, N);
@@ -150,14 +157,21 @@
   hipStream_t s = (hipStream_t)stream;
   int *const sched = tiles > grid ? gemm_sched_slot(s) : nullptr;
   hipLaunchKernelGGL((gemm256_kernel<5>), dim3(grid), dim3(512), 0, s, (const u16 *)A, (const u16 *)W, bias, (u16 *)xb, (int)M, N, K, tiles_n, tiles, nt,
-                     (const int *)nullptr, (const int *)nullptr, (const u16 *)nullptr, (const float *)nullptr, (const float *)nullptr, 0.f, 0, 0, 0, sched,
+                     (const int *)nullptr, (const int *)nullptr, (const u16 *)nullptr, (const float *)nullptr, (const float *)nullptr, 0.f, 0, 0, ldxb, sched,
                      (void *)xres, (const float *)nullptr, (float2 *)stats, prev_nparts, tiles > grid ? g_fold_stagger * (K / GEMM_BK) / 8 : 0, prev);
   return check_launch("linear_bf16_residual");
 }
 
 int unopose_linear_bf16_lnfold(const void *A, const void *W, const float *dvec, const float *cvec, const float *stats, int nparts, float eps, void *C,
                                long M, int N, int K, int gelu, unopose_stream_t stream) {
+  return unopose_linear_bf16_lnfold_ld(A, K, W, dvec, cvec, stats, nparts, eps, C, M, N, K, gelu, stream);
+}
+
+int unopose_linear_bf16_lnfold_ld(const void *A, int lda, const void *W, const float *dvec, const float *cvec, const float *stats, int nparts,
+                                  float eps, void *C, long M, int N, int K, int gelu, unopose_stream_t stream) {
   UNOPOSE_REQUIRE(A && W && dvec && cvec && stats && C, "linear_bf16_lnfold: null pointer");
+  UNOPOSE_REQUIRE(lda >= K && lda % 8 == 0 && (size_t)M * lda * 2 < (1UL << 32),
+                  "linear_bf16_lnfold: the row stride of A must cover a row, be a multiple of 8 elements and keep A below 4 GiB (lda=%d)", lda);
   UNOPOSE_REQUIRE(M >= 1 && M < (1L << 31) && N >= GEMM_BN && N % GEMM_BN == 0 && K >= GEMM_BK && K % GEMM_BK == 0,
                   "linear_bf16_lnfold: needs N %% 256 == 0 and K %% 64 == 0 (got M=%ld N=%d K=%d)", M, N, K);
   UNOPOSE_REQUIRE(nparts >= 1 && nparts <= GEMM_LNF_MAXPARTS && nparts * GEMM_BN == K, "linear_bf16_lnfold: needs nparts = K / 256 <= %d (got nparts=%d K=%d)", GEMM_LNF_MAXPARTS, nparts, K);
@@ -168,7 +182,7 @@
   int *const sched = tiles > grid ? gemm_sched_slot(s) : nullptr;
 #define UNOPOSE_LNF_LAUNCH(E)                                                                                                                      \
   hipLaunchKernelGGL((gemm256_kernel<E>), dim3(grid), dim3(512), 0, s, (const u16 *)A, (const u16 *)W, dvec, (u16 *)C, (int)M, N, K, tiles_n, tiles, nt, \
-                     (const int *)nullptr, (const int *)nullptr, (const u16 *)nullptr, (const float *)nullptr, (const float *)nullptr, eps, 0, 0, 0, sched, \
+                     (const int *)nullptr, (const int *)nullptr, (const u16 *)nullptr, (const float *)nullptr, (const float *)nullptr, eps, lda, 0, 0, sched, \
                      (void *)nullptr, cvec, (float2 *)stats, nparts)
   if (gelu)
     UNOPOSE_LNF_LAUNCH(7);
@@ -178,4 +192,26 @@
   return check_launch("linear_bf16_lnfold");
 }
 
-}
+int unopose_linear_bf16_gather_lnfold(const void *A, long M, int K, int segments, const void *W, int N, const float *dvec, const float *cvec,
+                                      const float *stats, float eps, const int *row_list, const int *tile_info, int max_tiles, void *C,
+                                      unopose_stream_t stream) {
+  UNOPOSE_REQUIRE(A && W && dvec && cvec && stats && C && row_list && tile_info, "linear_bf16_gather_lnfold: null pointer");
+  UNOPOSE_REQUIRE(M >= 1 && M < (1L << 31) && N >= GEMM_BN && N % GEMM_BN == 0 && N / GEMM_BN <= 64 && K >= GEMM_BK && K % GEMM_BK == 0,
+                  "linear_bf16_gather_lnfold: needs N %% 256 == 0 and K %% 64 == 0 (got M=%ld N=%d K=%d)", M, N, K);
+  UNOPOSE_REQUIRE(segments >= 1 && segments <= GEMM_GLN_MAXSEGS && K % segments == 0 && (K / segments) % GEMM_BN == 0 &&
+                      K / segments / GEMM_BN <= GEMM_LNF_MAXPARTS,
+                  "linear_bf16_gather_lnfold: needs K = S * Kseg with 1 <= S <= %d, Kseg %% 256 == 0 and Kseg / 256 <= %d (got K=%d S=%d)",
+                  GEMM_GLN_MAXSEGS, GEMM_LNF_MAXPARTS, K, segments);
+  UNOPOSE_REQUIRE((size_t)M * K * 2 < (1UL << 32) && (size_t)N * K * 2 < (1UL << 32) && (size_t)segments * N * 4 < (1UL << 31),
+                  "linear_bf16_gather_lnfold: operand larger than 4 GiB");
+  UNOPOSE_REQUIRE(max_tiles >= 0, "linear_bf16_gather_lnfold: bad tile capacity");
+  if (max_tiles == 0) return UNOPOSE_OK;
+  const int n_cu = gemm_cu_count();
+  const int grid = max_tiles >= n_cu ? n_cu : ((max_tiles + 7) & ~7);
+  hipLaunchKernelGGL((gemm256_kernel<8, true>), dim3(grid), dim3(512), 0, (hipStream_t)stream, (const u16 *)A, (const u16 *)W, dvec, (u16 *)C, (int)M, N,
+                     K, 1, 0, 0, row_list, tile_info, (const u16 *)nullptr, (const float *)nullptr, (const float *)nullptr, eps, 0, 0, 0, (int *)nullptr,
+                     (void *)nullptr, cvec, (float2 *)stats, K / segments / GEMM_BN);
+  return check_launch("linear_bf16_gather_lnfold");
+}
+
+}
diff --git a/unopose_amd/csrc/gemm_kernel.h b/unopose_amd/csrc/gemm_kernel.h
--- a/unopose_amd/csrc/gemm_kernel.h
+++ b/unopose_amd/csrc/gemm_kernel.h
@@ -18,6 +18,9 @@
 #define GEMM_LDS_STATS GEMM_LDS_LNPART
 #define GEMM_LNF_MAXPARTS 4
 #define GEMM_LDS_SHIFT (GEMM_LDS_LNPART + 8192)
+#define GEMM_GLN_MAXSEGS 4
+#define GEMM_LDS_GC GEMM_LDS_LNW
+#define GEMM_LDS_GRS (GEMM_LDS_GC + 2 * 4096)
 
 template <int EPI, bool GATHER = false, bool F32 = false>
 __global__ __launch_bounds__(512, 1) __attribute__((amdgpu_num_vgpr(127))) void gemm256_kernel(const void *__restrict__ Av, const void *__restrict__ Wv,
@@ -32,15 +35,17 @@
                                                            float2 *__restrict__ stats = nullptr, int nparts = 0, int stagger = 0,
                                                            const float *__restrict__ fold_prev = nullptr) {
   static_assert(!(F32 && (EPI == 3 || GATHER)), "the fp32-class form has no LayerNorm epilogue / gathered rows");
-  static_assert(!((F32 || GATHER) && EPI >= 5), "the residual / LayerNorm-fold epilogues belong to the dense bf16 form");
+  static_assert(!((F32 || GATHER) && EPI >= 5 && EPI != 8), "the residual / LayerNorm-fold epilogues belong to the dense bf16 form");
+  static_assert(EPI != 8 || (GATHER && !F32), "EPI 8 (segmented LayerNorm fold) is a gathered bf16 form");
   constexpr bool LNF = EPI == 6 || EPI == 7;
+  constexpr bool GLN = EPI == 8;
   static_assert(F32 || EPI != 4, "EPI 4 (bf16 + residual out of fp32-class operands) is an F32 epilogue");
   constexpr int ESZ = F32 ? 4 : 2;
   constexpr int KT = F32 ? 32 : 64;
   const char *A = reinterpret_cast<const char *>(Av), *W = reinterpret_cast<const char *>(Wv);
   const int LDA = lda ? lda : K, LDW = ldw ? ldw : K, LDC = ldc ? ldc : N;
   const int tiles = GATHER ? __builtin_amdgcn_readfirstlane(tile_info[0]) : tiles_arg;
-  __shared__ __attribute__((aligned(1024))) char smem[GEMM_LDS_BIAS + 2048 + 16 + (EPI == 3 ? 2048 + 8192 : EPI == 5 ? 2048 + 8192 + 4096 : LNF ? 2048 + 2 * 8192 : 0)];
+  __shared__ __attribute__((aligned(1024))) char smem[GEMM_LDS_BIAS + 2048 + 16 + (EPI == 3 ? 2048 + 8192 : EPI == 5 ? 2048 + 8192 + 4096 : LNF ? 2048 + 2 * 8192 : GLN ? 2 * 4096 + 2 * 8192 : 0)];
   float *const lnw_lds = reinterpret_cast<float *>(smem + GEMM_LDS_LNW), *const lnb_lds = reinterpret_cast<float *>(smem + GEMM_LDS_LNB);
   float2 *const ln_part = reinterpret_cast<float2 *>(smem + GEMM_LDS_LNPART);
   if (EPI == 3 && threadIdx.x < GEMM_BN) {
@@ -66,6 +71,8 @@
   const __amdgpu_buffer_rsrc_t c_rs = __builtin_amdgcn_make_buffer_rsrc(Cv, 0, GATHER ? 0x7fffffff : (int)((size_t)M * LDC * 2), 0x00020000);
   const __amdgpu_buffer_rsrc_t b_rs = __builtin_amdgcn_make_buffer_rsrc((void *)bias, 0, N * 4, 0x00020000);
   const int nk = K / KT;
+  const int segs = GLN ? K / (nparts * GEMM_BN) : 1, seg_tiles = GLN ? nparts * (GEMM_BN / KT) : nk;
+  const size_t seg_f2 = GLN ? (size_t)((M + GEMM_BM - 1) / GEMM_BM) * (GEMM_BM / 2) * (2 * nparts + 1) : 0;
 
   const int fx = (l31 >> 1) & 7;
   uint32_t fr_off[4];
@@ -80,7 +87,7 @@
     int m0, n0, rot;
     uint32_t a_off[4], w_off[2];
   };
-  auto tile_params = [&](int ti, int step, TileP &p) {
+  auto tile_params = [&](int ti, int step, TileP &p, int gsel) {
     const int t = chunk_base + ti;
     int tn, tm;
     if (GATHER) {
@@ -113,6 +120,20 @@
       int arow = p.m0 + row;
       if (GATHER) arow = max(row_list[p.m0 + row], 0);
       p.a_off[j] = (uint32_t)((size_t)arow * LDA * ESZ + c * 16);
+      if constexpr (GLN) {
+        const int sg = (lane & 7) >> 1, i0 = (lane & 1) * 2, i1 = i0 + 1;
+        const float2 *sp = stats + (sg < segs ? sg : 0) * seg_f2 + (size_t)arow * nparts;
+        const float2 v0 = sp[i0 < nparts ? i0 : 0], v1 = sp[i1 < nparts ? i1 : 0];
+        float t1 = (i0 < nparts ? v0.x : 0.f) + (i1 < nparts ? v1.x : 0.f), t2 = (i0 < nparts ? v0.y : 0.f) + (i1 < nparts ? v1.y : 0.f);
+        t1 += __shfl_xor(t1, 1);
+        t2 += __shfl_xor(t2, 1);
+        const float inv_k = 1.f / (float)(nparts * GEMM_BN);
+        const float mean = t1 * inv_k;
+        const float rs = rsqrtf(fmaxf(t2 * inv_k - mean * mean, 0.f) + ln_eps);
+        if ((lane & 1) == 0)
+          reinterpret_cast<float2 *>(smem + GEMM_LDS_GRS + gsel * 8192)[row * GEMM_GLN_MAXSEGS + sg] =
+              sg < segs ? make_float2(rs, -mean * rs) : make_float2(0.f, 0.f);
+      }
     }
 #pragma unroll
     for (int i = 0; i < 2; ++i) {
@@ -142,9 +163,18 @@
       gemm_dma16(lw + 1024, p.w_off[1], w_rs, sob);
     }
   };
-  const __amdgpu_buffer_rsrc_t cv_rs = __builtin_amdgcn_make_buffer_rsrc((void *)(LNF ? aux_vec : bias), 0, N * 4, 0x00020000);
+  const __amdgpu_buffer_rsrc_t cv_rs = __builtin_amdgcn_make_buffer_rsrc((void *)(LNF || GLN ? aux_vec : bias), 0, (GLN ? segs : 1) * N * 4, 0x00020000);
   const __amdgpu_buffer_rsrc_t st_rs = __builtin_amdgcn_make_buffer_rsrc((void *)stats, 0, LNF ? (int)((size_t)((M + GEMM_BM - 1) / GEMM_BM) * GEMM_BM * nparts * 8) : 0, 0x00020000);
   auto stage_bias = [&](const TileP &p, int bsel) {
+    if constexpr (GLN) {
+      const int pc = wave <= segs ? wave : 0;
+      if (pc == 0)
+        gemm_dma16(lds0 + GEMM_LDS_BIAS + bsel * 1024, (uint32_t)(lane * 16), b_rs, __builtin_amdgcn_readfirstlane(p.n0 * 4));
+      else
+        gemm_dma16(lds0 + GEMM_LDS_GC + bsel * 4096 + (pc - 1) * 1024, (uint32_t)(lane * 16), cv_rs,
+                   __builtin_amdgcn_readfirstlane(((pc - 1) * N + p.n0) * 4));
+      return;
+    }
     if (!LNF) {
       gemm_dma16(lds0 + GEMM_LDS_BIAS + bsel * 1024, (uint32_t)(lane * 16), b_rs, __builtin_amdgcn_readfirstlane(p.n0 * 4));
       return;
@@ -184,7 +214,7 @@
   for (; ti < chunk_len;) {
     const int step = dyn ? ti / nslots : (ti - slot) / nslots;
     if (!have) {
-      tile_params(ti, step, cur);
+      tile_params(ti, step, cur, bsel);
       stage_bias(cur, bsel);
       stage_half(cur, H_A0, 0, par);
       stage_half(cur, H_B0, 0, par);
@@ -212,7 +242,7 @@
     for (int nb = 0; nb < 2; ++nb)
 #pragma unroll
       for (int g = 0; g < 4; ++g) {
-        const float4 bv = EPI == 3 || LNF ? make_float4(0.f, 0.f, 0.f, 0.f) : *reinterpret_cast<const float4 *>(bias_lds + wn * 64 + nb * 32 + 8 * g + 4 * hi);
+        const float4 bv = EPI == 3 || LNF || GLN ? make_float4(0.f, 0.f, 0.f, 0.f) : *reinterpret_cast<const float4 *>(bias_lds + wn * 64 + nb * 32 + 8 * g + 4 * hi);
 #pragma unroll
         for (int mb = 0; mb < 4; ++mb) {
           acc[nb][mb][4 * g + 0] = bv.x;
@@ -264,6 +294,7 @@
       asm volatile("" ::: "memory");
       __builtin_amdgcn_sched_barrier(0);
     };
+    int seg = GLN ? cur.rot / seg_tiles : 0, seg_left = GLN ? seg_tiles - (cur.rot - seg * seg_tiles) : 0;
     for (int t = 0; t < nk; ++t) {
       const bool last = t + 1 == nk, last2 = t + 2 >= nk;
       if (dyn) {
@@ -277,7 +308,7 @@
           more = ti_next < chunk_len;
         }
       }
-      if (more && t + 2 == nk) tile_params(ti_next, dyn ? ti_next / nslots : step + 1, nxt);
+      if (more && t + 2 == nk) tile_params(ti_next, dyn ? ti_next / nslots : step + 1, nxt, bsel ^ 1);
       const char *lb = smem + par;
       const uint32_t bnext = par ^ GEMM_BUFBYTES;
       read_b(lb, 0, wf0);
@@ -321,8 +352,8 @@
           stage_half(nxt, H_A0, 0, par);
           stage_half(nxt, H_B0, 0, par);
           stage_half(nxt, H_B1, 0, par);
-          if (LNF) {
-            if (nparts <= 3) GEMM_WAIT_VM(9);
+          if (LNF || GLN) {
+            if (GLN || nparts <= 3) GEMM_WAIT_VM(9);
             else GEMM_WAIT_VM(10);
           } else
             GEMM_WAIT_VM(8);
@@ -341,6 +372,24 @@
         mfma_q(1, 0, wf0);
       });
       par ^= GEMM_BUFBYTES;
+      if constexpr (GLN) {
+        if (--seg_left == 0 && !last) {
+          int l31 = l31_;
+          asm volatile("" : "+v"(l31));
+          const int seg_next = seg + 1 == segs ? 0 : seg + 1;
+          const float2 *gp = reinterpret_cast<const float2 *>(smem + GEMM_LDS_GRS + bsel * 8192) + (wm * 128 + l31) * GEMM_GLN_MAXSEGS;
+#pragma unroll
+          for (int mb = 0; mb < 4; ++mb) {
+            const float f = gp[mb * 32 * GEMM_GLN_MAXSEGS + seg].x / gp[mb * 32 * GEMM_GLN_MAXSEGS + seg_next].x;
+#pragma unroll
+            for (int nb = 0; nb < 2; ++nb)
+#pragma unroll
+              for (int i = 0; i < 16; ++i) acc[nb][mb][i] *= f;
+          }
+          seg = seg_next;
+          seg_left = seg_tiles;
+        }
+      }
     }
     if (wm == 0) __builtin_amdgcn_s_barrier();
     par ^= GEMM_BUFBYTES;
@@ -427,6 +476,50 @@
             acc[nb][mb][4 * g + 3] = fmaf(rs[mb], acc[nb][mb][4 * g + 3], fmaf(nm[mb], cv.w, dv.w));
           }
         }
+    }
+    if constexpr (GLN) {
+      int l31 = l31_, hi = hi_;
+      asm volatile("" : "+v"(l31), "+v"(hi));
+      const float *c_lds = reinterpret_cast<const float *>(smem + GEMM_LDS_GC + bsel * 4096);
+      const float2 *gp = reinterpret_cast<const float2 *>(smem + GEMM_LDS_GRS + bsel * 8192) + (wm * 128 + l31) * GEMM_GLN_MAXSEGS;
+      float rs[4];
+#pragma unroll
+      for (int mb = 0; mb < 4; ++mb) rs[mb] = gp[mb * 32 * GEMM_GLN_MAXSEGS + seg].x;
+#pragma unroll
+      for (int nb = 0; nb < 2; ++nb)
+#pragma unroll
+        for (int g = 0; g < 4; ++g) {
+          const float4 dv = *reinterpret_cast<const float4 *>(bias_lds + wn * 64 + nb * 32 + 8 * g + 4 * hi);
+#pragma unroll
+          for (int mb = 0; mb < 4; ++mb) {
+            acc[nb][mb][4 * g + 0] = fmaf(rs[mb], acc[nb][mb][4 * g + 0], dv.x);
+            acc[nb][mb][4 * g + 1] = fmaf(rs[mb], acc[nb][mb][4 * g + 1], dv.y);
+            acc[nb][mb][4 * g + 2] = fmaf(rs[mb], acc[nb][mb][4 * g + 2], dv.z);
+            acc[nb][mb][4 * g + 3] = fmaf(rs[mb], acc[nb][mb][4 * g + 3], dv.w);
+          }
+        }
+      __builtin_amdgcn_sched_barrier(0);
+#pragma unroll
+      for (int s = 0; s < GEMM_GLN_MAXSEGS; ++s) {
+        if (s >= segs) break;
+        float nm[4];
+#pragma unroll
+        for (int mb = 0; mb < 4; ++mb) nm[mb] = gp[mb * 32 * GEMM_GLN_MAXSEGS + s].y;
+#pragma unroll
+        for (int nb = 0; nb < 2; ++nb)
+#pragma unroll
+          for (int g = 0; g < 4; ++g) {
+            const float4 cv = *reinterpret_cast<const float4 *>(c_lds + s * GEMM_BN + wn * 64 + nb * 32 + 8 * g + 4 * hi);
+#pragma unroll
+            for (int mb = 0; mb < 4; ++mb) {
+              acc[nb][mb][4 * g + 0] = fmaf(nm[mb], cv.x, acc[nb][mb][4 * g + 0]);
+              acc[nb][mb][4 * g + 1] = fmaf(nm[mb], cv.y, acc[nb][mb][4 * g + 1]);
+              acc[nb][mb][4 * g + 2] = fmaf(nm[mb], cv.z, acc[nb][mb][4 * g + 2]);
+              acc[nb][mb][4 * g + 3] = fmaf(nm[mb], cv.w, acc[nb][mb][4 * g + 3]);
+            }
+          }
+        __builtin_amdgcn_sched_barrier(0);
+      }
     }
     if constexpr (EPI == 5) {
       int l31 = l31_, hi = hi_, lane = lane_;
diff --git a/unopose_amd/model/modules.py b/unopose_amd/model/modules.py
--- a/unopose_amd/model/modules.py
+++ b/unopose_amd/model/modules.py
@@ -56,11 +56,13 @@
             return x, None
         return x, ops.scale_residual_layernorm_(x, y, self.ls2.gamma, next_norm)
 
-    def forward_folded(self, x, n1, xb, stats):
+    def forward_folded(self, x, n1, xb, stats, tap=None):
         a = self.attn
         qkv = ops.linear(n1, a.qkv) if n1 is not None else ops.linear_lnfold(xb, stats, a.qkv, self.norm1)
         xb, stats = ops.linear_residual_(x, ops.vit_attention(qkv, a.heads), a.proj, self.ls1.gamma, stats)
         h = ops.linear_lnfold(xb, stats, self.mlp.fc1, self.norm2, gelu=True)
+        if tap is not None:
+            return ops.linear_residual_(x, h, self.mlp.fc2, self.ls2.gamma, stats, xb_out=tap[0], stats_out=tap[1])
         return ops.linear_residual_(x, h, self.mlp.fc2, self.ls2.gamma, stats)
 
     def forward_fused_f32(self, x, n1s, next_norm):
@@ -120,11 +122,11 @@
         self.norm = nn.LayerNorm(embed_dim, eps=1e-6)
         self.head = nn.Linear(embed_dim, 1000)
 
-    def forward(self, x, taps_side_by_side=False):
+    def forward(self, x, taps_side_by_side=False, fold_taps=0):
         xa, xb = x if isinstance(x, (tuple, list)) else (x, None)
         if ops.vit_prologue_ok(xa, self) and (xb is None or xb.shape[1:] == xa.shape[1:]):
             x, n1, mean = ops.vit_prologue(xa, xb, self, self.blocks[0].norm1, row_mean=True)
-            return self._fused_blocks(x, n1, taps_side_by_side, mean)
+            return self._fused_blocks(x, n1, taps_side_by_side, mean, fold_taps)
         if F32_PROLOGUE and ops.vit_prologue_f32_ok(xa, self) and (xb is None or xb.shape[1:] == xa.shape[1:]):
             x, ns = ops.vit_prologue_f32(xa, xb, self, self.blocks[0].norm1)
             return self._fused_blocks_f32(x, ns, taps_side_by_side)
@@ -142,7 +144,7 @@
         if x.is_cuda and torch.is_autocast_enabled() and x.dtype == torch.float32 and x.shape[-1] % 4 == 0 \
                 and not ops.is_differentiable():
             x = x.contiguous()
-            return self._fused_blocks(x, ops.add_layernorm(x, None, self.blocks[0].norm1, torch.bfloat16), taps_side_by_side)
+            return self._fused_blocks(x, ops.add_layernorm(x, None, self.blocks[0].norm1, torch.bfloat16), taps_side_by_side, None, fold_taps)
         if ops.vit_f32_fused_ok(x, self):
             x = x.contiguous()
             return self._fused_blocks_f32(x, ops.scale_residual_layernorm_f32_(x, None, None, self.blocks[0].norm1), taps_side_by_side)
@@ -169,26 +171,32 @@
         return SplitTaps(wide, x.shape[0], x.shape[1], 4 * x.shape[2]) if wide is not None else outs
 
 
-def _vit_fused_blocks(self, x, n1, taps_side_by_side, row_mean=None):
+def _vit_fused_blocks(self, x, n1, taps_side_by_side, row_mean=None, fold_taps=0):
     n = self.depth // 4
     taps = {self.depth - 1, self.depth - n - 1, self.depth - 2 * n - 1, self.depth - 3 * n - 1}
     outs = []
-    B, _, D = x.shape
-    wide = torch.empty(B, x.shape[1], len(taps) * D, dtype=torch.bfloat16, device=x.device) if taps_side_by_side else None
-    fold = ops.ln_fold_ok(B * x.shape[1], D, x.device)
+    B, T, D = x.shape
+    fold = ops.ln_fold_ok(B * T, D, x.device)
+    tap_fold = fold and taps_side_by_side and fold_taps == T and len(taps) == 4 and 0 not in taps
+    if tap_fold:
+        wide, tap_stats = ops.fold_tap_buffers(B, T, D, len(taps), x.device)
+    else:
+        wide = torch.empty(B, T, len(taps) * D, dtype=torch.bfloat16, device=x.device) if taps_side_by_side else None
     if fold and row_mean is None:
         row_mean = ops.fold_row_means(x)
     xb, stats = None, row_mean
     for i, blk in enumerate(self.blocks):
         nxt = self.blocks[i + 1].norm1 if i + 1 < len(self.blocks) else None
+        k = len(outs)
         if fold:
-            xb, stats = blk.forward_folded(x, n1, xb, stats)
+            xb, stats = blk.forward_folded(x, n1, xb, stats, (wide[:, :, k * D:(k + 1) * D], tap_stats[k]) if tap_fold and i in taps else None)
             n1 = None
         else:
             x, n1 = blk.forward_fused(x, n1, nxt)
         if i in taps:
-            k = len(outs)
-            outs.append(ops.add_layernorm(x, None, self.norm, out=None if wide is None else wide[:, :, k * D:(k + 1) * D]))
+            outs.append(None if tap_fold else ops.add_layernorm(x, None, self.norm, out=None if wide is None else wide[:, :, k * D:(k + 1) * D]))
+    if tap_fold:
+        return ops.FoldedTaps(wide, tap_stats, self.norm)
     return outs if wide is None else wide
 
 
@@ -269,8 +277,8 @@
                 sd = x.shape[-1] // 14
                 npre = self.vit.cls_token.shape[1] + self.vit.reg_token.shape[1]
                 plan = ops.upproj_plan(choose, x.shape[-2], x.shape[-1], sd, npre, npre + sd * sd)
-                acts = self.vit(x, taps_side_by_side=True)
-                if torch.is_tensor(acts) and acts.shape[1] == plan["tok_stride"]:
+                acts = self.vit(x, taps_side_by_side=True, fold_taps=plan["tok_stride"])
+                if (torch.is_tensor(acts) or isinstance(acts, ops.FoldedTaps)) and acts.shape[1] == plan["tok_stride"]:
                     return ops.sparse_pixel_features(acts, self.output_upscaling, plan)
                 z, (H, W), off = self.upproject(acts, x.shape[-2], x.shape[-1])
                 return ops.bilinear_sample_native(z, choose, H, W, tok_offset=off)
diff --git a/unopose_amd/model/unopose.py b/unopose_amd/model/unopose.py
--- a/unopose_amd/model/unopose.py
+++ b/unopose_amd/model/unopose.py
@@ -304,8 +304,8 @@
                     t.record_stream(main)
         B = rgb.shape[0]
         if plan is not None:
-            acts = net.vit((rgb, tem_rgb), taps_side_by_side=True)
-            if torch.is_tensor(acts) and acts.shape[1] == plan["tok_stride"]:
+            acts = net.vit((rgb, tem_rgb), taps_side_by_side=True, fold_taps=plan["tok_stride"])
+            if (torch.is_tensor(acts) or isinstance(acts, ops.FoldedTaps)) and acts.shape[1] == plan["tok_stride"]:
                 main.wait_stream(side)
                 both = ops.sparse_pixel_features(acts, net.output_upscaling, plan)
                 return dense_pm, both[:B], dense_po, both[B:], radius, pre
diff --git a/unopose_amd/ops/__init__.py b/unopose_amd/ops/__init__.py
--- a/unopose_amd/ops/__init__.py
+++ b/unopose_amd/ops/__init__.py
@@ -11,7 +11,7 @@
     linear_f32x3_bf16, linear_f32_raw, _transposed_weights, _LinearFn, _ZERO_BIAS, _zero_bias, linear_train, _lin, mlp, linear,
     ffn_add_layernorm, linear_add_layernorm, patch_embed, vit_prologue_ok, vit_prologue, vit_prologue_f32_ok, vit_prologue_f32, bmm_nt_f32, score_head, add_layernorm,
     scale_residual_, scale_residual_layernorm_f32_, vit_f32_fused_ok, scale_residual_layernorm_, ln_fold_ok, _fold_producer_weights,
-    _fold_consumer_weights, linear_residual_, linear_lnfold, fold_shift, fold_row_means, _into,
+    _fold_consumer_weights, linear_residual_, linear_lnfold, fold_shift, fold_row_means, _into, FoldedTaps, fold_tap_buffers, _row_stride,
 )
 from .attention import (
     vit_attention, vit_attention_f32_split, vit_attention_f32_ss, vit_attention_torch, _KEY_PAD, token_attention,
diff --git a/unopose_amd/ops/dense.py b/unopose_amd/ops/dense.py
--- a/unopose_amd/ops/dense.py
+++ b/unopose_amd/ops/dense.py
@@ -569,16 +569,16 @@
     return cache
 
 
-def _fold_consumer_weights(lin, norm):
+def _fold_consumer_weights(lin, norm, segments=1):
     key = (lin.weight._version, lin.weight.data_ptr(), lin.weight.device, None if lin.bias is None else lin.bias._version,
-           norm.weight._version, norm.weight.data_ptr(), norm.bias._version)
+           norm.weight._version, norm.weight.data_ptr(), norm.bias._version, segments)
     cache = getattr(lin, "_fold_cons_cache", None)
     if cache is None or cache[0] != key:
         with torch.no_grad():
             w32 = lin.weight.detach().float()
-            w = (w32 * norm.weight.detach().float()[None, :]).to(torch.bfloat16).contiguous()
-            c = w.float().sum(1).contiguous()
-            d = (w32.double() @ norm.bias.detach().double()).float()
+            w = (w32 * norm.weight.detach().float().repeat(segments)[None, :]).to(torch.bfloat16).contiguous()
+            c = w.float().sum(1).contiguous() if segments == 1 else w.float().reshape(w.shape[0], segments, -1).sum(2).t().contiguous()
+            d = (w32.double() @ norm.bias.detach().double().repeat(segments)).float()
             if lin.bias is not None:
                 d = d + lin.bias.detach().float()
             d = d.contiguous()
@@ -587,7 +587,30 @@
     return cache
 
 
-def linear_residual_(x, a, lin, gamma, prev=None):
+class FoldedTaps:
+
+    def __init__(self, wide, stats, norm):
+        self.wide, self.stats, self.norm = wide, stats, norm
+        self.shape = wide.shape
+
+
+def fold_tap_buffers(B, T, C, taps, device):
+    rows_p = (B * T + 255) // 256 * 256
+    return (torch.empty(B, T, taps * C, dtype=torch.bfloat16, device=device),
+            torch.empty(taps, rows_p * (2 * (C // 256) + 1), dtype=torch.float32, device=device))
+
+
+def _row_stride(t, width):
+    ld = t.stride(-2) if t.dim() >= 2 else width
+    assert t.shape[-1] == width and t.stride(-1) == 1 and ld >= width and ld % 8 == 0
+    exp = ld
+    for d in range(t.dim() - 2, -1, -1):
+        assert t.stride(d) == exp or t.shape[d] == 1, "rows must be uniformly strided"
+        exp *= t.shape[d]
+    return ld
+
+
+def linear_residual_(x, a, lin, gamma, prev=None, xb_out=None, stats_out=None):
     note_mutation()
     _, w, b = _fold_producer_weights(lin, gamma)
     C, K = w.shape
@@ -603,12 +626,21 @@
         else:
             assert prev.dim() == 1
     a = _c(a)
-    xb = torch.empty(x.shape, dtype=torch.bfloat16, device=x.device)
-    buf = torch.empty(rows_p * (2 * (C // 256) + 1), dtype=torch.float32, device=x.device)
+    if xb_out is None:
+        xb = torch.empty(x.shape, dtype=torch.bfloat16, device=x.device)
+    else:
+        xb = xb_out
+        assert xb.dtype == torch.bfloat16 and xb.shape == x.shape and xb.device == x.device
+    ldxb = _row_stride(xb, C)
+    if stats_out is None:
+        buf = torch.empty(rows_p * (2 * (C // 256) + 1), dtype=torch.float32, device=x.device)
+    else:
+        buf = stats_out
+        assert buf.dtype == torch.float32 and buf.dim() == 1 and buf.is_contiguous() and buf.numel() == rows_p * (2 * (C // 256) + 1) and buf.device == x.device
     stats = buf[:rows_p * 2 * (C // 256)].view(rows_p, C // 256, 2)
     with on_device(x.device):
-        call("unopose_linear_bf16_residual", ptr(a), ptr(w), ptr(b), ptr(x), ptr(xb), ptr(stats), None if prev is None else ptr(prev), prev_parts,
-             rows, C, K, stream_ptr())
+        call("unopose_linear_bf16_residual_ld", ptr(a), ptr(w), ptr(b), ptr(x), ptr(xb), ldxb, ptr(stats), None if prev is None else ptr(prev),
+             prev_parts, rows, C, K, stream_ptr())
     return xb, stats
 
 
@@ -631,5 +663,6 @@
     rows = xb.numel() // K
     out = torch.empty(*xb.shape[:-1], N, dtype=torch.bfloat16, device=xb.device)
     with on_device(xb.device):
-        call("unopose_linear_bf16_lnfold", ptr(xb), ptr(w), ptr(d), ptr(c), ptr(stats), K // 256, float(norm.eps), ptr(out), rows, N, K, int(gelu), stream_ptr())
+        call("unopose_linear_bf16_lnfold_ld", ptr(xb), _row_stride(xb, K), ptr(w), ptr(d), ptr(c), ptr(stats), K // 256, float(norm.eps), ptr(out), rows, N, K,
+             int(gelu), stream_ptr())
     return out
diff --git a/unopose_amd/ops/sampling.py b/unopose_amd/ops/sampling.py
--- a/unopose_amd/ops/sampling.py
+++ b/unopose_amd/ops/sampling.py
@@ -3,7 +3,7 @@
 from .._lib import call, on_device, ptr, stream_ptr
 from . import _state as st
 from .common import _c, note_mutation
-from .dense import _bf16_weights
+from .dense import FoldedTaps, _bf16_weights, _fold_consumer_weights
 
 
 def bilinear_sample_native(z, choose, H, W, out=None, tok_offset=0):
@@ -52,13 +52,19 @@
 
 
 def sparse_pixel_features(acts, lin, plan, out=None):
-    acts = _c(acts)
+    folded = acts if isinstance(acts, FoldedTaps) else None
+    acts = folded.wide if folded is not None else _c(acts)
     if out is not None:
         note_mutation()
     B2, ts, K = acts.shape
-    assert acts.dtype == torch.bfloat16 and ts == plan["tok_stride"] and B2 == plan["choose"].shape[0]
-    cache = _bf16_weights(lin)
-    w, bias = cache[1], cache[3]
+    assert acts.dtype == torch.bfloat16 and acts.is_contiguous() and ts == plan["tok_stride"] and B2 == plan["choose"].shape[0]
+    if folded is not None:
+        segs = folded.stats.shape[0]
+        _, w, cvec, bias = _fold_consumer_weights(lin, folded.norm, segs)
+        assert folded.stats.is_contiguous() and folded.stats.shape[1] == (B2 * ts + 255) // 256 * 256 * (2 * (K // segs // 256) + 1)
+    else:
+        cache = _bf16_weights(lin)
+        w, bias = cache[1], cache[3]
     N = w.shape[0]
     assert N == 16 * 256 and w.shape[1] == K
     Np = plan["choose"].shape[1]
@@ -68,8 +74,12 @@
     assert out.shape == (B2, Np, 256) and out.dtype in (torch.float32, torch.bfloat16) and out.is_contiguous()
     with on_device(dev):
         cells = torch.empty(plan["cap_rows"], 256, dtype=torch.bfloat16, device=dev)
-        call("unopose_linear_bf16_gather", ptr(acts), B2 * ts, K, ptr(w), N, ptr(bias), ptr(plan["row_list"]),
-             ptr(plan["tile_info"]), plan["cap_rows"] // 256, ptr(cells), stream_ptr())
+        if folded is not None:
+            call("unopose_linear_bf16_gather_lnfold", ptr(acts), B2 * ts, K, segs, ptr(w), N, ptr(bias), ptr(cvec), ptr(folded.stats),
+                 float(folded.norm.eps), ptr(plan["row_list"]), ptr(plan["tile_info"]), plan["cap_rows"] // 256, ptr(cells), stream_ptr())
+        else:
+            call("unopose_linear_bf16_gather", ptr(acts), B2 * ts, K, ptr(w), N, ptr(bias), ptr(plan["row_list"]),
+                 ptr(plan["tile_info"]), plan["cap_rows"] // 256, ptr(cells), stream_ptr())
         call("unopose_bilinear_sample_compact", ptr(cells), ptr(plan["cellmap"]), ptr(plan["choose"]), B2, plan["side"], Np,
              plan["H"], plan["W"], ptr(out), int(out.dtype == torch.bfloat16), stream_ptr())
     return out
```
